# treangenlab/bronko

Hardware: AMD Instinct MI355X
Metric: reads/sec through call k-mer->pileup, SARS-CoV-2 k=21 (higher is better)
Workload: dtype u64

## Files before the change

bronko_amd/csrc/bk_engine.cpp:

```cpp
#include <hip/hip_runtime.h>

#include <algorithm>
#include <cstdarg>
#include <cstdio>
#include <cstdlib>
#include <cstring>
#include <memory>
#include <string>
#include <vector>

#include "bk_engine.h"

thread_local std::string g_err;

int fail(int code, const char* fmt, ...) {
    char buf[1024];
    va_list ap;
    va_start(ap, fmt);
    vsnprintf(buf, sizeof buf, fmt, ap);
    va_end(ap);
    g_err = buf;
    return code;
}

static int alloc_sample_state(bk_engine* e) {
    const bk_params* prm = &e->params;
    const IndexTables& ix = *e->ix;
    for (MatePlane& p : e->mate) BK_HIP(p.counters.alloc(ix.plane_len));
    e->sparse = ix.W > 0 && (ix.plane_len >= (16ull << 20) || test_env("BK_SPARSE_FINALIZE") != nullptr);
    if (e->sparse) {
        const uint64_t n_rows = bk::v_real_rows(ix.n_full, ix.v_span);
        for (MatePlane& p : e->mate) {
            BK_HIP(hipMemset(p.counters.p, 0, p.counters.n * sizeof(unsigned long long)));
            BK_HIP(p.touch_v.alloc(n_rows / 32 + 1)); BK_HIP(p.touch_p.alloc(ix.n_prows / 32 + 1)); BK_HIP(p.touch_e.alloc((size_t)ix.n_u / 32 + 1));
            BK_HIP(hipMemset(p.touch_v.p, 0, p.touch_v.n * 4)); BK_HIP(hipMemset(p.touch_p.p, 0, p.touch_p.n * 4));
            BK_HIP(hipMemset(p.touch_e.p, 0, p.touch_e.n * 4));
            BK_HIP(p.touch_b.alloc((size_t)ix.total_cells / 64 / 32 + 2)); BK_HIP(hipMemset(p.touch_b.p, 0, p.touch_b.n * 4));
            BK_HIP(p.v_list.alloc(n_rows)); BK_HIP(p.p_list.alloc(ix.n_prows)); BK_HIP(p.e_list.alloc(ix.n_u));
            BK_HIP(p.n_list.alloc(8));
        }
    }
    BK_HIP(e->shard_sums.alloc((size_t)2 * ix.n_files * 5 + 9));
    BK_HIP(e->xport_flag.alloc(4));
    BK_HIP(hipMemset(e->xport_flag.p, 0, 4 * sizeof(unsigned long long)));
    if (prm->full_kmer_stats) {
        if (prm->kmer_table_log2 < 10 || prm->kmer_table_log2 > 31) return fail(BK_ERR_INVALID, "kmer_table_log2 out of range");
        BK_HIP(e->ktab.keys.alloc((size_t)1 << prm->kmer_table_log2));
        BK_HIP(e->ktab.cnt.alloc((size_t)1 << prm->kmer_table_log2));
        e->ktab.log2 = prm->kmer_table_log2;
        BK_HIP(e->ktab.h_fill.grow(bk::ktab_fill_words())); BK_HIP(e->ktab.fill_ev.create());
    }
    BK_HIP(e->ktab_out.alloc(8 + bk::ktab_fill_words()));
    if (ix.n_files <= 2048) BK_HIP(e->fin_partials.alloc(bk::finalize_partial_rows() * ((size_t)ix.n_files * 3 + 2)));
    BK_HIP(e->deferred.alloc(bk::v_plane_len(ix.n_full, ix.v_span, ix.n_prows) * (prm->pileup_selected_only ? 2 : 1)));
    BK_HIP(e->n_deferred.alloc(2));
    if (prm->pileup_selected_only && ix.ent_files.p) BK_HIP(e->deferred_mask.alloc(e->deferred.n));
    if (!e->sparse) {
        BK_HIP(e->deferred_n.alloc(e->deferred.n));
        for (MatePlane& p : e->mate) BK_HIP(hipMemset(p.counters.p, 0, std::max<size_t>(p.counters.n, 1) * sizeof(unsigned long long)));
    }
    if (ix.n_files == 1 && !e->sparse && ix.n_full > 0) { BK_HIP(e->lean_e_list.alloc((size_t)ix.n_full)); BK_HIP(e->lean_n_list.alloc(8)); BK_HIP(hipMemset(e->lean_n_list.p, 0, 8 * sizeof(unsigned int))); }
    BK_HIP(e->pileup.alloc(ix.total_cells * 4 * 4));
    e->gather_mode = ix.gather_ok && e->sparse && ix.cell_file.p && ix.dirty_ans.p && ix.W > 1 && ix.file_cell_lo_d.p && !test_env("BK_NO_GATHER");
    if (e->gather_mode) {
        for (MatePlane& p : e->mate) BK_HIP(p.alias_hits.alloc((size_t)bk_engine::kAliasCap * 3));
        BK_HIP(e->n_alias_hits.alloc(2));
        BK_HIP(e->last_sel.upload(std::vector<int>(1, -1)));
        BK_HIP(hipMemset(e->pileup.p, 0, std::max<size_t>(e->pileup.n, 1) * sizeof(unsigned long long)));
        const bool two_pass = prm->pileup_selected_only != 0 && ix.n_files > 1;
        if (!two_pass && prm->cs < (1ull << 28) && ix.total_cells >= 2 * (uint64_t)ix.n_full && !test_env("BK_NO_VOTE_TABLE")) {
            BK_HIP(e->row_bits.alloc((size_t)((bk::v_real_rows(ix.n_full, ix.v_span) + 31) / 32) + 1));
            BK_HIP(e->vote_tab.alloc(bk::vote_table_words(ix.view())));
        }
    }
    BK_HIP(e->stats.alloc((size_t)2 * ix.n_files * 3));
    BK_HIP(e->present.alloc((size_t)2 * ix.n_files));
    if (prm->pileup_selected_only != 0 && ix.n_files > 1) BK_HIP(e->sel_out.alloc(1));
    BK_HIP(e->l2_plan.alloc(4));
    BK_HIP(e->kstats.alloc(8));
    e->use_items = !e->sparse && ix.ref_in_lds && ix.W > 0 && ix.n_lds_bins > 0 && !test_env("BK_NO_ITEMS") && ix.seed_tab2.p && ix.rc_words.p &&
                   bk::item_geometry(std::min<uint32_t>(ix.n_lds_bins, (uint32_t)ix.total_cells), ix.n_full, ix.v_span, &e->ig) &&
                   bk::items_lds_bytes(e->ig, std::min<uint32_t>(ix.n_lds_bins, (uint32_t)ix.total_cells)) <= 128u * 1024u;
    if (e->use_items) {
        if (const char* cp = test_env("BK_ITEM_CAPS")) {
            unsigned ce = 0, cv = 0;
            if (sscanf(cp, "%u,%u", &ce, &cv) == 2 && ce >= 8 && cv >= 8 && ce <= 64 && cv <= 64 && ce % 8 == 0 && cv % 8 == 0) {
                bk::ItemGeom g2 = e->ig;
                g2.cap_e = ce; g2.cap_v = cv; g2.wg_items = g2.n_ebins * ce + g2.n_vbins * cv; g2.wg_stride = g2.wg_items;
                if (bk::items_lds_bytes(g2, std::min<uint32_t>(ix.n_lds_bins, (uint32_t)ix.total_cells)) <= 118u * 1024u) e->ig = g2;
            }
        }
        const size_t g = bk::items_max_grid(ix.n_cus);
        e->ig.grid_max = (uint32_t)g;
        BK_HIP(e->items.alloc(g * e->ig.wg_stride + 64));
        BK_HIP(e->item_tab.alloc(g * ((size_t)e->ig.n_ebins + e->ig.n_vbins)));
        BK_HIP(e->item_gext.alloc(g * ((size_t)e->ig.n_ebins + e->ig.n_vbins) * bk::kItemGCap));
        BK_HIP(e->ov.alloc((size_t)1 << 20));
        BK_HIP(e->ov_n.alloc(4));
        BK_HIP(hipMemset(e->ov_n.p, 0, 4 * sizeof(unsigned long long)));
    } else {
        BK_HIP(e->slabs.alloc((size_t)ix.n_cus * std::max<uint32_t>(ix.n_lds_bins, 1)));
    }
    if (ix.n_files > 1) { BK_HIP(e->win_votes.alloc((size_t)ix.n_files)); BK_HIP(e->win_sel.upload(std::vector<uint32_t>(2, 0u))); }
    e->fuse_ok = e->use_items && ix.n_files == 1 && ix.max_seqs_per_file == 1 && (uint64_t)ix.n_lds_bins >= ix.total_cells && !e->ktab.keys.p && ix.n_prows == 0 &&
                 ix.n_u == ix.n_full && ix.n_full > 0 && ix.dirty_ans.p && ix.W > 1 && ix.v_span > 0 && ix.v_span <= 32 && e->fin_partials.p && e->lean_e_list.p &&
                 prm->cs < (1ull << 32) && e->ig.vq_log2 == 6 && !test_env("BK_NO_LEAN_FINALIZE") && !test_env("BK_NO_FUSE") && !test_env("BK_NO_N_DIRECT");
    if (e->fuse_ok)
        for (MatePlane& p : e->mate) { BK_HIP(p.fuse_touch.alloc(((size_t)ix.n_full + (size_t)ix.v_span + 63) / 64 * 12 + 16)); BK_HIP(hipMemset(p.fuse_touch.p, 0, p.fuse_touch.n * sizeof(unsigned int))); }
    BK_HIP(hipStreamCreateWithFlags(&e->own_stream, hipStreamNonBlocking));
    e->stream = e->own_stream;
    return BK_OK;
}

extern "C" {

int bk_abi_version(void) { return BK_ABI_VERSION; }
int bk_device_count(void) {
    int n = 0;
    return hipGetDeviceCount(&n) == hipSuccess && n > 0 ? n : 0;
}
int bk_device_memory(int device, uint64_t* free_bytes, uint64_t* total_bytes) {
    if (!free_bytes || !total_bytes) return fail(BK_ERR_INVALID, "null argument");
    BK_HIP(hipSetDevice(device));
    size_t f = 0, t = 0;
    BK_HIP(hipMemGetInfo(&f, &t));
    *free_bytes = f; *total_bytes = t;
    return BK_OK;
}
const char* bk_last_error(void) { return g_err.c_str(); }

void bk_params_default(bk_params* p) {
    if (!p) return;
    p->n_fixed = 2;
    p->use_full_kmer = 0;
    p->ci = 3;
    p->cs = 1000000;
    p->cx = 1000000000ull;
    p->device = 0;
    p->full_kmer_stats = 0;
    p->kmer_table_log2 = 26;
    p->pileup_selected_only = 0;
}


int bk_engine_create(const bk_index_desc* ix, const bk_params* prm, bk_engine** out) {
    if (!ix || !prm || !out) return fail(BK_ERR_INVALID, "null argument");
    *out = nullptr;
    const int k = ix->k;
    if (k < 3 || k > bk::kMaxK || (k & 1) == 0) return fail(BK_ERR_INVALID, "Invalid kmer size %d, must be odd and <= %d", k, bk::kMaxK);
    if (prm->n_fixed < 0) return fail(BK_ERR_INVALID, "n_fixed must be >= 0");
    if (ix->n_files <= 0 || ix->n_files > 65536) return fail(BK_ERR_INVALID, "n_files out of range");
    if (ix->n_buckets && (!ix->bucket_ids || !ix->bucket_off || !ix->entries)) return fail(BK_ERR_INVALID, "null index arrays");

    int ndev = 0;
    if (hipGetDeviceCount(&ndev) != hipSuccess || ndev <= 0) return fail(BK_ERR_NO_DEVICE, "no HIP device visible (this library has no CPU fallback)");
    if (prm->device < 0 || prm->device >= ndev) return fail(BK_ERR_NO_DEVICE, "device %d not present (%d visible)", prm->device, ndev);
    BK_HIP(hipSetDevice(prm->device));
    {
        hipDeviceProp_t prop;
        BK_HIP(hipGetDeviceProperties(&prop, prm->device));
        if (std::strncmp(prop.gcnArchName, "gfx950", 6) != 0)
            return fail(BK_ERR_NO_DEVICE, "device %d is %s, not gfx950 (MI355X); this library has no other code path", prm->device, prop.gcnArchName);
    }

    auto tab = std::make_shared<IndexTables>();
    PhaseClock pc;
    if (int rc = build_index_tables(ix, prm, *tab, pc)) return rc;
    std::unique_ptr<bk_engine> e(new bk_engine());
    e->params = *prm;
    e->device = prm->device;
    e->ix = tab;
    if (int rc = alloc_sample_state(e.get())) return rc;
    BK_HIP(tab->d_view.upload(std::vector<bk::IndexView>(1, tab->view())));
    pc.lap("uploads + buffers");
    *out = e.release();
    return BK_OK;
}

int bk_engine_fork(const bk_engine* parent, bk_engine** out) { return bk_engine_fork_params(parent, nullptr, out); }

int bk_engine_fork_params(const bk_engine* parent, const bk_params* prm, bk_engine** out) {
    if (!parent || !out) return fail(BK_ERR_INVALID, "null argument");
    if (prm && (prm->n_fixed != parent->params.n_fixed || (prm->use_full_kmer != 0) != (parent->params.use_full_kmer != 0) ||
                prm->device != parent->params.device || (prm->full_kmer_stats != 0) != (parent->params.full_kmer_stats != 0)))
        return fail(BK_ERR_INVALID, "bk_engine_fork_params: n_fixed, use_full_kmer, full_kmer_stats and device shape the shared tables and must equal the parent's");
    if (prm && prm->cs == 0) return fail(BK_ERR_INVALID, "cs must be >= 1");
    BK_HIP(hipSetDevice(parent->device));
    std::unique_ptr<bk_engine> e(new bk_engine());
    e->params = prm ? *prm : parent->params;
    e->device = parent->device;
    e->ix = parent->ix;
    e->ix->family.fetch_add(1);
    if (int rc = alloc_sample_state(e.get())) return rc;
    *out = e.release();
    return BK_OK;
}

void bk_engine_destroy(bk_engine* e) {
    if (!e) return;
    e->ix->family.fetch_sub(1);
    (void)hipSetDevice(e->device);
    (void)hipStreamSynchronize(e->stream);
    for (auto& s : e->spans) { (void)hipEventDestroy(s.a); (void)hipEventDestroy(s.b); }
    for (auto ev : e->free_events) (void)hipEventDestroy(ev);
    if (e->copy_stream) (void)hipStreamDestroy(e->copy_stream);
    if (e->own_stream) (void)hipStreamDestroy(e->own_stream);
    delete e;
}

int bk_engine_set_stream(bk_engine* e, void* hip_stream) {
    if (!e) return fail(BK_ERR_INVALID, "null engine");
    BK_HIP(hipStreamSynchronize(e->stream));
    e->stream = hip_stream ? reinterpret_cast<hipStream_t>(hip_stream) : e->own_stream;
    return BK_OK;
}

void* bk_engine_get_stream(const bk_engine* e) { return e ? reinterpret_cast<void*>(e->stream) : nullptr; }

uint64_t bk_total_cells(const bk_engine* e) { return e ? e->ix->total_cells : 0; }
int32_t bk_n_files(const bk_engine* e) { return e ? e->ix->n_files : 0; }
uint64_t bk_n_slots(const bk_engine* e) { return e ? e->ix->n_slots : 0; }
uint64_t bk_counter_len(const bk_engine* e) { return e ? e->ix->plane_len : 0; }
int bk_can_shard(const bk_engine* e) { return e && !e->sparse ? 1 : 0; }

int GrowTable::clear(bk_engine* e) {
    if (!old.empty()) {
        BK_HIP(hipStreamSynchronize(e->stream));
        for (auto& o : old) { (void)hipFree(o.first); (void)hipFree(o.second); }
        old.clear();
    }
    BK_HIP(hipMemsetAsync(keys.p, 0xff, keys.n * sizeof(unsigned long long), e->stream));
    BK_HIP(hipMemsetAsync(cnt.p, 0, cnt.n * sizeof(unsigned int), e->stream));
    fill_known = 0; fill_unknown_upper = 0; fill_pending = false;
    return BK_OK;
}

int bk_sample_begin(bk_engine* e) {
    if (!e) return fail(BK_ERR_INVALID, "null engine");
    BK_HIP(hipSetDevice(e->device));
    bk_engine::Span sp(e, 2);
    e->win_chosen = false;
    const bool sel_rows = e->gather_mode && e->params.pileup_selected_only != 0 && e->ix->n_files > 1;
    bk::launch_zero_small(e->stats.p, e->stats.n, e->kstats.p, e->kstats.n, e->ktab_out.p, e->ktab_out.n, e->present.p, e->present.n,
                          e->n_deferred.p, e->n_deferred.n, e->pileup.p, e->gather_mode ? 0 : e->pileup.n, e->stream);
    if (sel_rows) bk::launch_zero_genome_rows(e->pileup.p, (size_t)e->ix->total_cells * 4, e->ix->file_cell_lo_d.p, e->ix->n_files, (uint32_t)e->ix->total_cells, e->last_sel.p, e->stream);
    if (e->ktab.keys.p) { if (int rc = e->ktab.clear(e)) return rc; }
    if (e->dump) { if (int rc = e->dump->begin_sample(e)) return rc; }
    for (EventPass* p : e->event_passes()) if (p) { if (int rc = p->begin_sample(e)) return rc; }
    if (e->linkage) { if (int rc = e->linkage->begin_sample(e)) return rc; }
    if (e->primers) { if (int rc = e->primers->begin_sample(e)) return rc; }
    if (e->adapters) { if (int rc = e->adapters->begin_sample(e)) return rc; }
    e->ktab_exchanged = false; e->in_sample = true; e->finalized_mates = 0; e->called = false; e->cons_made = false; e->ci_made = false; e->regions_made = false;
    e->pending.on = false;
    for (MatePlane& p : e->mate) { if (int rc = p.begin_sample(e)) return rc; }
    return BK_OK;
}

int MatePlane::begin_sample(bk_engine* e) {
    stale = true; fuse_off = false; reduced_shards = 0; pushed_records = 0;
    if (touch_used) { BK_HIP(hipMemsetAsync(fuse_touch.p, 0, fuse_touch.n * sizeof(unsigned int), e->stream)); touch_used = false; }
    return BK_OK;
}

static int flush_pending_items(bk_engine* e) {
    if (!e->pending.on) return BK_OK;
    bk_engine::Span sp(e, 3);
    bk::BinArgs b = e->pending.b;
    b.part = 2; b.v_mode = e->ix->item_v_mode >= 0 && e->ix->item_v_mode != 2 ? e->ix->item_v_mode : 1;
    e->pending.on = false; e->mate[e->pending.mate].no_more_waiting();
    BK_HIP(bk::launch_bin_count(b, e->stream));
    return BK_OK;
}

int MatePlane::zero_if_stale(bk_engine* e) {
    if (!stale) return BK_OK;
    if (used) {
        bk_engine::Span sp(e, 2);
        BK_HIP(hipMemsetAsync(counters.p, 0, std::max<size_t>(counters.n, 1) * sizeof(unsigned long long), e->stream));
        if (e->sparse) for (DevBuf<unsigned int>* t : {&touch_v, &touch_p, &touch_b, &touch_e}) BK_HIP(hipMemsetAsync(t->p, 0, t->n * 4, e->stream));
        used = false;
    }
    stale = false;
    v_clean = true;
    return BK_OK;
}

int GrowTable::ensure_room(bk_engine* e, unsigned long long* out, uint64_t upper) {
    if (!keys.p) return BK_OK;
    const uint64_t cap = 1ull << log2;
    if (fill_known + fill_unknown_upper + upper > cap / 2) {
        if (fill_pending) { BK_HIP(hipEventSynchronize(fill_ev)); read_fill(); }
        uint32_t nl = log2;
        while (nl < 31 && fill_known + fill_unknown_upper + upper > (1ull << nl) / 2) nl += 2;
        if (nl > 31) nl = 31;
        if (nl != log2) {
            unsigned long long* nk = nullptr; unsigned int* nc = nullptr;
            BK_HIP(hipMalloc(reinterpret_cast<void**>(&nk), ((size_t)1 << nl) * sizeof(unsigned long long)));
            BK_HIP(hipMalloc(reinterpret_cast<void**>(&nc), ((size_t)1 << nl) * sizeof(unsigned int)));
            BK_HIP(hipMemsetAsync(nk, 0xff, ((size_t)1 << nl) * sizeof(unsigned long long), e->stream));
            BK_HIP(hipMemsetAsync(nc, 0, ((size_t)1 << nl) * sizeof(unsigned int), e->stream));
            bk::launch_ktab_rehash(keys.p, cnt.p, log2, nk, nc, nl, out + 4, e->stream);
            old.emplace_back(keys.p, cnt.p);
            keys.p = nk; keys.n = (size_t)1 << nl;
            cnt.p = nc; cnt.n = (size_t)1 << nl;
            log2 = nl;
        }
    }
    fill_unknown_upper += upper;
    return BK_OK;
}
int GrowTable::note_fill(bk_engine* e, const unsigned long long* out) {
    if (!keys.p) return BK_OK;
    BK_HIP(hipMemcpyAsync(h_fill.p, out + 8, bk::ktab_fill_words() * sizeof(unsigned long long), hipMemcpyDeviceToHost, e->stream));
    BK_HIP(hipEventRecord(fill_ev, e->stream));
    fill_pending = true;
    return BK_OK;
}

#ifdef BK_TESTING
static int l2_count_report(bk_engine* e, const bk::ScanArgs& a) {
    if (!test_env("BK_L2_COUNT")) return BK_OK;
    const uint64_t take = a.n_records;
    std::vector<unsigned int> hb((size_t)take * a.l2_words), ha((size_t)(take + 31) / 32);
    BK_HIP(hipMemcpyAsync(hb.data(), e->n_bits.p, hb.size() * sizeof(unsigned int), hipMemcpyDeviceToHost, e->stream));
    BK_HIP(hipMemcpyAsync(ha.data(), e->n_any.p, ha.size() * sizeof(unsigned int), hipMemcpyDeviceToHost, e->stream));
    BK_HIP(hipStreamSynchronize(e->stream));
    uint64_t nk = 0, nr = 0, runs = 0;
    for (size_t i = 0; i < hb.size(); i++) { nk += (uint64_t)__builtin_popcount(hb[i]); runs += (uint64_t)__builtin_popcount(hb[i] & ~(hb[i] << 1)); }
    for (unsigned int w : ha) nr += (uint64_t)__builtin_popcount(w);
    fprintf(stderr, "[bk] left to level 2 by the scan: %llu of %llu records marked, %llu k-mers in %llu N runs (per 32-bit word)\n", (unsigned long long)nr,
            (unsigned long long)take, (unsigned long long)nk, (unsigned long long)runs);
    return BK_OK;
}
static int l2_stats_arm(bk_engine* e) {
    if (test_env("BK_L2_STATS") && !e->dbg.p) { BK_HIP(e->dbg.alloc(32 + 4 * 1024)); BK_HIP(hipMemsetAsync(e->dbg.p, 0, (32 + 4 * 1024) * sizeof(unsigned long long), e->stream)); }
    return BK_OK;
}
static int l2_stats_report(bk_engine* e) {
    if (!e->dbg.p) return BK_OK;
    const IndexTables& ix = *e->ix;
    unsigned long long h[32]; unsigned int nd[2] = {0, 0};
    BK_HIP(hipMemcpyAsync(nd, e->n_deferred.p, sizeof nd, hipMemcpyDeviceToHost, e->stream));
    std::vector<unsigned long long> clk(4 * 1024);
    BK_HIP(hipMemcpyAsync(h, e->dbg.p, sizeof h, hipMemcpyDeviceToHost, e->stream));
    BK_HIP(hipMemcpyAsync(clk.data(), e->dbg.p + 32, clk.size() * sizeof(unsigned long long), hipMemcpyDeviceToHost, e->stream));
    BK_HIP(hipMemsetAsync(e->dbg.p, 0, (32 + 4 * 1024) * sizeof(unsigned long long), e->stream));
    BK_HIP(hipStreamSynchronize(e->stream));
    unsigned long long t0 = ~0ull;
    int n_wg = 0;
    for (int b = 0; b < 512; b++) if (clk[4 * b]) { t0 = std::min(t0, clk[4 * b]); n_wg = b + 1; }
    if (n_wg) {
        double mx[4] = {0, 0, 0, 0}, mean[4] = {0, 0, 0, 0}, mn[4] = {1e30, 1e30, 1e30, 1e30};
        for (int b = 0; b < n_wg; b++)
            for (int j = 0; j < 4; j++) {
                const double us = (double)(clk[4 * b + j] - t0) * 0.01;
                mx[j] = std::max(mx[j], us); mn[j] = std::min(mn[j], us); mean[j] += us / n_wg;
            }
        fprintf(stderr, "[bk] scan workgroups (%d), us after the first start, min / mean / max: start %.1f / %.1f / %.1f, reference staged %.1f / %.1f / %.1f, "
                "tiles done %.1f / %.1f / %.1f, end %.1f / %.1f / %.1f\n", n_wg, mn[0], mean[0], mx[0], mn[1], mean[1], mx[1], mn[2], mean[2], mx[2], mn[3], mean[3], mx[3]);
        double m2[4] = {0, 0, 0, 0};
        int n2 = 0;
        for (int b = 0; b < std::min(n_wg, 512); b++) if (clk[2048 + 4 * b]) { n2++; for (int j = 0; j < 4; j++) m2[j] += (double)(clk[2048 + 4 * b + j] - t0) * 0.01; }
        if (n2) fprintf(stderr, "[bk]   ... mean: first tile's copy sent %.1f, window's loads stored %.1f, wave 0 has its first tile %.1f, buckets written out %.1f\n",
                        m2[0] / n2, m2[1] / n2, m2[2] / n2, m2[3] / n2);
        if (test_env("BK_L2_STATS")[0] == '2')
            for (int b = 0; b < n_wg; b++) fprintf(stderr, "[bk]   wg %d: %.1f %.1f %.1f %.1f\n", b, (clk[4 * b] - t0) * 0.01, (clk[4 * b + 1] - t0) * 0.01, (clk[4 * b + 2] - t0) * 0.01, (clk[4 * b + 3] - t0) * 0.01);
    }
    fprintf(stderr, "[bk] finalize: %u + %u k-mers deferred to the general kernel\n", nd[0], nd[1]);
    if (e->gather_mode) {
        unsigned int ah[2] = {0u, 0u};
        BK_HIP(hipMemcpy(ah, e->n_alias_hits.p, sizeof ah, hipMemcpyDeviceToHost));
        fprintf(stderr, "[bk] votes gathered cell by cell (bk_gather.hip); alias hits among the deferred k-mers: %u + %u\n", ah[0], ah[1]);
    }
    if (e->sparse) {
        unsigned int nl[8];
        BK_HIP(hipMemcpy(nl, e->mate[0].n_list.p, sizeof nl, hipMemcpyDeviceToHost));
        fprintf(stderr, "[bk] sparse finalize (mate file 0): %u V rows of %llu, %u pseudo rows of %llu, %u reference k-mers of %u and %u pseudo k-mers of %u touched\n",
                nl[0], (unsigned long long)bk::v_real_rows(ix.n_full, ix.v_span), nl[4], (unsigned long long)ix.n_prows, nl[2], ix.n_full, nl[3], ix.n_u - ix.n_full);
    }
    fprintf(stderr, "[bk] scan: %llu mismatches counted, %llu items processed, %llu E gaps before a mismatch, %llu behind the last\n", h[23], h[24], h[25], h[26]);
    fprintf(stderr, "[bk] scan N batches: %llu with %llu pieces (%.1f per batch), %llu of them forced by a tile's end\n", h[20], h[21], h[20] ? (double)h[21] / (double)h[20] : 0.0, h[22]);
    fprintf(stderr, "[bk] level 2 discovery: %llu records newly marked by the scan, %llu records queued, g_work %llu\n", h[27], h[28], h[29]);
    fprintf(stderr, "[bk] scan marked: no-diagonal %llu, dirty-head %llu, clean-head %llu, pairs %llu | level 2: k-mers %llu in %llu chunks, simple %llu, dead %llu, "
            "dirty answers %llu (one difference but id unknown: %llu), neither half present %llu, slow %llu (diffs 0/1/2/3+ with a diagonal: %llu/%llu/%llu/%llu) -> member %llu, neighbour %llu, nothing %llu\n",
            h[0], h[1], h[2], h[3], h[4], h[11], h[5], h[6], h[16], h[17], h[18], h[7], h[12], h[13], h[14], h[15], h[8], h[9], h[10]);
    return BK_OK;
}
#else
static int l2_count_report(bk_engine*, const bk::ScanArgs&) { return BK_OK; }
static int l2_stats_arm(bk_engine*) { return BK_OK; }
static int l2_stats_report(bk_engine*) { return BK_OK; }
#endif

static bk::ScanArgs scan_args(const bk_engine* e, int mate, const Records& r) {
    const IndexTables& ix = *e->ix;
    const MatePlane& pl = e->mate[mate];
    bk::ScanArgs a{};
    a.n_records_dev = r.n_dev; a.ixp = ix.d_view.p;
    a.k = ix.k; a.wstart = ix.wstart; a.W = ix.W; a.v_omin = ix.v_omin; a.v_span = ix.v_span; a.v_off = ix.v_off; a.total_cells = (uint32_t)ix.total_cells; a.n_u = ix.n_u;
    a.ref_words = ix.ref_words.p; a.cell_codes = ix.cell_codes.p; a.cell_has = ix.cell_has.p; a.cell_clean = ix.cell_clean.p; a.cell_clean3 = ix.cell_clean3.p; a.cell_yf = ix.cell_yf.p; a.cell_yr = ix.cell_yr.p; a.id_at = ix.id_at.p; a.cell_fast = ix.cell_fast.p; a.cell_nat = ix.cell_nat.p; a.cell_natrow = ix.cell_natrow.p; a.cell_blk = ix.cell_blk.p; a.seed_tab = ix.seed_tab.p; a.seed_log2 = ix.seed_log2;
    a.seed_tab2 = ix.seed_tab2.p; a.seed2_log2 = ix.seed2_log2; a.rc_words = ix.rc_words.p;
    a.n_direct = e->use_items && ix.n_files == 1 && ix.max_seqs_per_file == 1 && (uint64_t)ix.n_lds_bins >= ix.total_cells && !test_env("BK_NO_N_DIRECT");
    a.words = r.words; a.lens = r.lens; a.n_records = r.n; a.stride_words = r.stride_words;
    a.counters = pl.counters.p; a.kmer_total = e->kstats.p + mate * 4 + 1;
    a.ablate = ix.ablate; a.slabs = e->slabs.p; a.n_lds_bins = ix.n_lds_bins; a.ref_in_lds = ix.ref_in_lds ? 1 : 0;
    a.ktab_keys = e->ktab.keys.p; a.ktab_cnt = e->ktab.cnt.p; a.ktab_log2 = e->ktab.log2;
    a.ktab_overflow = e->ktab_out.p + 4; a.mate = (uint32_t)mate;
    a.occ = ix.occ.p; a.n_files = ix.n_files;
    if (e->sparse) {
        a.touch_v = pl.touch_v.p; a.touch_b = pl.touch_b.p; a.touch_p = pl.touch_p.p; a.touch_e = pl.touch_e.p;
        a.rl_recip = ~0ull / (unsigned long long)(ix.v_span + 1) + 1ull;
    }
    a.dbg = e->dbg.p; a.l2_words = bk::scan_l2_words(r.stride_words, ix.k); a.l2_min_grid = (uint32_t)std::max(1, ix.n_cus / 2);
    if (const char* mg = test_env("BK_L2_MIN_GRID")) a.l2_min_grid = (uint32_t)std::max(1, atoi(mg));
    if (e->use_items) { a.ig = e->ig; a.items = e->items.p; a.tab = e->item_tab.p; a.gext = e->item_gext.p; a.ov = e->ov.p; a.ov_n = e->ov_n.p; a.ov_cap = (uint32_t)e->ov.n; }
    return a;
}
static int choose_window(bk_engine* e, bk::ScanArgs& a, uint64_t n) {
    const IndexTables& ix = *e->ix;
    if (ix.occ.p && !e->win_chosen && n > 0) {
        BK_HIP(hipMemsetAsync(e->win_votes.p, 0, e->win_votes.n * sizeof(unsigned int), e->stream));
        const char* wf = test_env("BK_WINDOW_FILE");
        const int forced = wf ? std::max(0, atoi(wf)) : -1;
        bk::launch_pick_window(a, 16384, e->win_votes.p, ix.file_cell_lo_d.p, forced, e->win_sel.p, e->stream);
        e->win_chosen = true;
    }
    a.win_dev = ix.occ.p ? e->win_sel.p : nullptr;
    return BK_OK;
}
static uint64_t next_launch(const bk_engine* e, uint64_t left, uint64_t l2_cap, uint32_t& grid) {
    const IndexTables& ix = *e->ix;
    grid = bk::scan_grid(left, ix.n_cus);
    uint64_t take = e->use_items ? std::min<uint64_t>(left, l2_cap) : std::min<uint64_t>(std::min<uint64_t>(left, bk::scan_max_records(grid)), l2_cap);
    if (ix.max_launch_records) take = std::min<uint64_t>(take, ix.max_launch_records);
    if (e->use_items) {
        int share = ix.n_cus - ix.n_cus / 4;
        if (const char* fr = test_env("BK_ITEM_SHARE")) share = std::max(1, std::min(ix.n_cus, ix.n_cus * atoi(fr) / 16));
        grid = bk::items_grid(take, ix.family.load() > 1 ? share : ix.n_cus);
        if (const char* gr = test_env("BK_ITEM_GRID")) grid = std::max<uint32_t>(1, std::min<uint32_t>(grid, (uint32_t)atoi(gr)));
    }
    return take;
}
static int make_l2_room(bk_engine* e, bk::ScanArgs& a, uint64_t l2_cap) {
    if (e->l2_bits.n < a.n_records * a.l2_words || e->l2_diag.n < a.n_records) {
        BK_HIP(hipStreamSynchronize(e->stream));
        const uint64_t recs = std::min<uint64_t>(std::max<uint64_t>(a.n_records + a.n_records / 4, 1 << 16), l2_cap);
        BK_HIP(e->l2_bits.alloc((size_t)recs * a.l2_words)); BK_HIP(e->n_bits.alloc((size_t)recs * a.l2_words)); BK_HIP(e->l2_diag.alloc((size_t)recs));
        BK_HIP(e->l2_any.alloc((size_t)(recs + 31) / 32)); BK_HIP(e->n_any.alloc((size_t)(recs + 31) / 32));
        for (DevBuf<unsigned int>* b : {&e->l2_bits, &e->l2_any, &e->n_bits, &e->n_any}) BK_HIP(hipMemsetAsync(b->p, 0, b->n * sizeof(unsigned int), e->stream));
    }
    a.l2_bits = e->l2_bits.p; a.l2_diag = e->l2_diag.p; a.l2_any = e->l2_any.p; a.n_bits = e->n_bits.p; a.n_any = e->n_any.p;
    return BK_OK;
}
static int bin_items(bk_engine* e, bk::ScanArgs& a, int mate, uint32_t grid, bool wait_v, bk::BinArgs* ride) {
    const IndexTables& ix = *e->ix;
    MatePlane& pl = e->mate[mate];
    bk_engine::Span sp(e, 3);
    bk::BinArgs b{};
    b.ig = e->ig; b.items = e->items.p; b.tab = e->item_tab.p; b.gext = e->item_gext.p; b.n_wg = grid; b.ov = e->ov.p; b.ov_n = e->ov_n.p; b.ov_cap = (uint32_t)e->ov.n;
    b.ov_par = e->ov_par; e->ov_par ^= 1u;
    b.id_at = ix.id_at.p; b.cell_codes = ix.cell_codes.p + bk::scan_ref_pad_words(); b.win_lo = a.win_lo; b.win_dev = a.win_dev; b.total_cells = (uint32_t)ix.total_cells;
    b.counters = pl.counters.p; b.v_off = ix.v_off; b.v_real_len = bk::v_real_len(ix.n_full, ix.v_span); b.rl = (uint32_t)ix.v_span + 1u;
    const bool v_clean = pl.take_v_clean();
    b.v_mode = ix.item_v_mode >= 0 ? ix.item_v_mode : (v_clean ? 2 : 1);
    if (const char* ba = test_env("BK_BIN_ABLATE")) b.ablate = atoi(ba);
    if (wait_v) {
        e->pending.on = true; e->pending.mate = mate; e->pending.b = b;
        b.part = 1;
        a.touch_v = pl.fuse_touch.p; a.rl_recip = ~0ull / (unsigned long long)(ix.v_span + 1) + 1ull;
        pl.items_wait();
    } else {
        pl.no_more_waiting();
        if (e->fuse_ok) a.touch_v = nullptr;
    }
    if (ride) {
        *ride = b; ride->part = 1;
        if (wait_v) return BK_OK;
        b.part = 2;
    }
    BK_HIP(bk::launch_bin_count(b, e->stream));
    return BK_OK;
}
static bool level2_runs(const bk_engine* e, const bk::ScanArgs& a) { return e->ix->ablate != 1 && e->ix->ablate != 4 && bk::level2_launches(a); }
static int level2_and_fold(bk_engine* e, const bk::ScanArgs& a, int mate, uint32_t grid, const bk::BinArgs* ride) {
    const IndexTables& ix = *e->ix;
    bk_engine::Span sp(e, 3);
    if (int rc = l2_count_report(e, a)) return rc;
    if (ix.ablate == 1 || ix.ablate == 4) {
        BK_HIP(hipMemsetAsync(e->n_bits.p, 0, (size_t)a.n_records * a.l2_words * sizeof(unsigned int), e->stream));
        BK_HIP(hipMemsetAsync(e->n_any.p, 0, e->n_any.n * sizeof(unsigned int), e->stream));
    }
    else BK_HIP(bk::launch_level2(a, ix.n_cus, e->stream, ride));
    if (!e->use_items) {
        bk::FoldArgs f{};
        f.slabs = e->slabs.p; f.n_slabs = grid; f.n_lds_bins = ix.n_lds_bins; f.id_at = ix.id_at.p; f.cell_codes = ix.cell_codes.p + bk::scan_ref_pad_words(); f.win_lo = a.win_lo; f.win_dev = a.win_dev; f.touch_e = a.touch_e;
        f.counters = e->mate[mate].counters.p;
        bk::launch_fold(f, e->stream);
    }
    return BK_OK;
}
}
int push_device(bk_engine* e, int mate, const Records& r) {
    MatePlane& pl = e->mate[mate];
    if (int rc = pl.zero_if_stale(e)) return rc;
    const uint64_t n = r.n, upper = r.kmers_upper ? r.kmers_upper : n * (uint64_t)r.stride_words * 16;
    if (int rc = e->ktab.ensure_room(e, e->ktab_out.p, upper)) return rc;
    if (e->dump) { if (int rc = e->dump->push(e, mate, r, upper)) return rc; }
    pl.written();
    if (int rc = l2_stats_arm(e)) return rc;
    bk::ScanArgs a = scan_args(e, mate, r);
    if (e->ix->W <= 0) {
        bk::launch_count_kmers(a, e->stream);
    } else {
        if (int rc = choose_window(e, a, n)) return rc;
        const uint64_t l2_cap = std::max<uint64_t>(64, ((1ull << 30) / sizeof(unsigned int)) / a.l2_words);
        for (uint64_t base = 0; base < n; base += a.n_records) {
            uint32_t grid = 0;
            a.rec_base = base; a.n_records = next_launch(e, n - base, l2_cap, grid);
            if (int rc = make_l2_room(e, a, l2_cap)) return rc;
            if (int rc = flush_pending_items(e)) return rc;
            const bool wait_v = e->fuse_ok && a.n_direct && !pl.fuse_off && e->ix->item_v_mode < 0;
            a.l2_plan = e->use_items && e->ix->n_files == 1 && e->ix->family.load() >= 4 && !test_env("BK_NO_L2_PLAN") ? e->l2_plan.p : nullptr;
            {
                bk_engine::Span sp(e, 0);
                if (e->use_items) { a.ov_par = e->ov_par; BK_HIP(bk::launch_scan_items(a, grid, e->stream)); }
                else BK_HIP(bk::launch_scan_count(a, grid, e->stream));
            }
            bk::BinArgs ride_b{};
            const bool ride = e->use_items && level2_runs(e, a) && !test_env("BK_NO_E_RIDE");
            if (e->use_items) { if (int rc = bin_items(e, a, mate, grid, wait_v, ride ? &ride_b : nullptr)) return rc; }
            if (int rc = level2_and_fold(e, a, mate, grid, ride ? &ride_b : nullptr)) return rc;
        }
    }
    for (EventPass* p : e->event_passes()) if (p) { if (int rc = p->push(e, r)) return rc; }
    if (e->linkage) { if (int rc = e->linkage->push(e, r)) return rc; }
    BK_HIP(hipGetLastError());
    if (!r.n_dev) pl.pushed_records += n;
    return e->ktab.note_fill(e, e->ktab_out.p);
}
extern "C" {

int bk_counters_device_ptr(bk_engine* e, int mate, void** d_ptr) {
    if (!e || !d_ptr || mate < 0 || mate > 1) return fail(BK_ERR_INVALID, "bad argument");
    if (e->sparse) return fail(BK_ERR_UNSUPPORTED, "an index this large keeps its counter planes sparse: shard whole samples over GPUs, not one sample's reads");
    if (e->pending.on) { BK_HIP(hipSetDevice(e->device)); if (int rc = flush_pending_items(e)) return rc; }
    if (e->in_sample) {
        BK_HIP(hipSetDevice(e->device));
        if (int rc = e->mate[mate].zero_if_stale(e)) return rc;
    }
    e->mate[mate].handed_out();
    *d_ptr = e->mate[mate].counters.p;
    return BK_OK;
}

int bk_pileup_device_ptr(bk_engine* e, void** d_ptr) {
    if (!e || !d_ptr) return fail(BK_ERR_INVALID, "bad argument");
    *d_ptr = e->pileup.p;
    return BK_OK;
}

struct FinalizeCall { int n_mates; uint64_t elem_lo, elem_hi; bool two_pass = false, gather = false, clean_dense = false; };
static int compact_sparse_lists(bk_engine* e, int n_mates) {
    const IndexTables& ix = *e->ix;
    for (int m = 0; m < n_mates; m++) {
        MatePlane& pl = e->mate[m];
        bk_engine::Span sp(e, 1);
        BK_HIP(hipMemsetAsync(pl.n_list.p, 0, 8 * sizeof(unsigned int), e->stream));
#ifdef BK_TESTING
        if (ix.ablate == 15) BK_HIP(hipMemsetAsync(pl.touch_b.p, 0xff, pl.touch_b.n * 4, e->stream));
#endif
        bk::launch_expand_touched_blocks(pl.touch_b.p, (uint32_t)((ix.total_cells + 63) / 64), ix.cell_blk.p, pl.touch_v.p, (uint32_t)ix.k,
                                         (uint64_t)ix.n_full + (uint64_t)ix.v_span, e->stream);
        bk::launch_compact_touched(pl.touch_v.p, bk::v_real_rows(ix.n_full, ix.v_span), pl.touch_p.p, ix.n_prows, pl.touch_e.p, ix.n_u,
                                   ix.n_full, pl.v_list.p, pl.p_list.p, pl.e_list.p, pl.n_list.p, e->stream);
    }
    return BK_OK;
}
static bk::FinalizeArgs finalize_args(const bk_engine* e, const FinalizeCall& c, int m, int pass) {
    const IndexTables& ix = *e->ix;
    const MatePlane& pl = e->mate[m];
    bk::FinalizeArgs a{};
    a.ix = ix.view();
    a.counters = pl.reduced_shards > 0 ? pl.reduced.p - c.elem_lo : pl.counters.p;
    a.elem_lo = c.elem_lo; a.elem_hi = c.elem_hi; a.ci = e->params.ci; a.cs = e->params.cs; a.cx = e->params.cx; a.pileup = e->pileup.p; a.plane = (size_t)ix.total_cells * 4;
    a.stats = e->stats.p + (size_t)m * ix.n_files * 3; a.present = e->present.p + (size_t)m * ix.n_files; a.kept_total = e->kstats.p + m * 4 + 3; a.distinct_total = e->kstats.p + m * 4 + 2;
    a.partials = e->fin_partials.p; a.n_deferred = e->n_deferred.p + m;
    a.deferred = e->deferred.p + (c.two_pass ? (size_t)m * (e->deferred.n / 2) : 0);
    a.file_cell_lo = ix.file_cell_lo_d.p; a.max_file_cells = (uint32_t)ix.max_file_cells_idx;
    a.deferred_mask = c.two_pass && e->deferred_mask.p ? e->deferred_mask.p + (size_t)m * (e->deferred_mask.n / 2) : nullptr;
    a.ktab_keys = e->ktab.keys.p; a.ktab_cnt = e->ktab.cnt.p; a.ktab_log2 = e->ktab.log2; a.ktab_overflow = e->ktab_out.p + 4; a.mate = (uint32_t)m;
    if (e->sparse) { a.v_list = pl.v_list.p; a.p_list = pl.p_list.p; a.e_list = pl.e_list.p; a.n_list = pl.n_list.p; }
    a.deferred_n = e->deferred_n.p ? e->deferred_n.p + (c.two_pass ? (size_t)m * (e->deferred_n.n / 2) : 0) : nullptr;
    a.clear_v = c.clean_dense && pass == (c.two_pass ? 1 : 0);
    a.mode = c.two_pass ? pass + 1 : c.gather ? (pass == 0 ? 1 : 3) : 0;
    if (c.gather) {
        if (const char* ga = test_env("BK_GATHER_ABLATE")) a.gather_ablate = atoi(ga);
        a.merged_slots = ix.merged_slots.p; a.n_merged_slots = ix.n_merged_slots;
        a.gather = pass == 1 ? 1 : 0; a.alias_hits = pl.alias_hits.p; a.n_alias_hits = e->n_alias_hits.p + m; a.alias_cap = bk_engine::kAliasCap;
    }
    a.sel = c.two_pass ? &e->sel_out.p->file_id : nullptr; a.sel_file = -1;
    const bool ride = c.clean_dense && !c.two_pass && e->fin_partials.p && pl.used;
    a.no_lean = test_env("BK_NO_LEAN_FINALIZE") != nullptr; a.lean_e_list = e->lean_e_list.p; a.lean_n_list = e->lean_n_list.p;
    a.zero_e = ride ? pl.counters.p : nullptr; a.zero_e_n = ride ? (size_t)std::min<uint64_t>(ix.v_off, ix.plane_len) : 0;
    return a;
}
static int clean_planes(bk_engine* e, const FinalizeCall& c) {
    const IndexTables& ix = *e->ix;
    for (int m = 0; m < c.n_mates && c.clean_dense; m++) {
        MatePlane& pl = e->mate[m];
        if (pl.used) {
            bk_engine::Span sp(e, 2);
            BK_HIP(hipMemsetAsync(pl.counters.p, 0, (size_t)std::min<uint64_t>(ix.v_off, ix.plane_len) * sizeof(unsigned long long), e->stream));
        }
        pl.finalized_clean();
    }
    for (int m = 0; m < c.n_mates && e->sparse; m++) {
        MatePlane& pl = e->mate[m];
        bk_engine::Span sp(e, 1);
        bk::launch_clear_touched(pl.counters.p, ix.v_off, bk::v_real_len(ix.n_full, ix.v_span), (uint32_t)ix.v_span + 1u, pl.v_list.p, pl.p_list.p,
                                 pl.e_list.p, pl.n_list.p, ix.n_u, e->stream);
        pl.finalized_clean();
    }
    if (e->ktab.keys.p) { bk_engine::Span sp(e, 1); bk::launch_ktab_stats(e->ktab.keys.p, e->ktab.cnt.p, e->ktab.log2, e->params.ci, e->params.cx, e->ktab_out.p, e->stream); }
    return BK_OK;
}
static int finalize_part(bk_engine* e, int n_mates, uint64_t elem_lo, uint64_t elem_hi) {
    const IndexTables& ix = *e->ix;
    if (!e->in_sample) return fail(BK_ERR_STATE, "bk_sample_finalize called before bk_sample_begin");
    if (n_mates < 1 || n_mates > 2) return fail(BK_ERR_INVALID, "n_mates must be 1 or 2");
    BK_HIP(hipSetDevice(e->device));
    const bool whole = elem_lo == 0 && elem_hi == ix.plane_len;
    const bool via_reduced = e->mate[0].reduced_shards > 0 || e->mate[1].reduced_shards > 0;
    FinalizeCall c{n_mates, elem_lo, elem_hi};
    c.two_pass = e->params.pileup_selected_only != 0 && ix.n_files > 1;
    c.gather = e->gather_mode && whole && !via_reduced;
    c.clean_dense = !e->sparse && whole && !via_reduced;
    if (c.two_pass && !whole) return fail(BK_ERR_UNSUPPORTED, "pileup_selected_only cannot be combined with a sharded finalize");
    if (e->sparse && !whole) return fail(BK_ERR_UNSUPPORTED, "an index this large cannot be finalized in shards");
    if (e->sparse) { if (int rc = compact_sparse_lists(e, n_mates)) return rc; }
    if (c.gather) BK_HIP(hipMemsetAsync(e->n_alias_hits.p, 0, 2 * sizeof(unsigned int), e->stream));
    auto sync_debug = [e](const char* what) -> int {
        if (test_env("BK_SYNC_DEBUG")) { fprintf(stderr, "[bk] %s ...", what); BK_HIP(hipStreamSynchronize(e->stream)); fprintf(stderr, " ok\n"); }
        return BK_OK;
    };
    for (int pass = 0; pass < ((c.two_pass || c.gather) ? 2 : 1); pass++) {
        const bool votes = c.gather && pass == 1;
        if (votes) {
            bk_engine::Span sp(e, 1);
            if (int rc = sync_debug("statistics pass")) return rc;
            if (e->row_bits.p) BK_HIP(hipMemsetAsync(e->row_bits.p, 0, e->row_bits.n * sizeof(unsigned int), e->stream));
            for (int m = 0; m < n_mates; m++) bk::launch_prefix_rows(e->mate[m].counters.p, ix.view(), e->mate[m].v_list.p, e->mate[m].n_list.p, e->row_bits.p, e->stream);
            if (int rc = sync_debug("prefix_rows")) return rc;
        }
        for (int m = 0; m < n_mates; m++) {
            bk::FinalizeArgs a = finalize_args(e, c, m, pass);
            if (a.zero_e) e->mate[m].finalized_clean();
            if (pass == 0) { if (int rc = e->mate[m].zero_if_stale(e)) return rc; }
            if (e->pending.on && e->pending.mate == m) {
                const bk::BinArgs& pb = e->pending.b;
                a.f_items = pb.items; a.f_tab = pb.tab; a.f_gext = pb.gext; a.f_ov = pb.ov; a.f_ov_n = pb.ov_n; a.f_ov_cap = pb.ov_cap; a.f_ov_par = pb.ov_par;
                a.f_n_wg = pb.n_wg; a.f_ig = pb.ig; a.f_touch = e->mate[m].fuse_touch.p;
                if (c.clean_dense && !c.two_pass && bk::finalize_runs_by_region(a)) { e->pending.on = false; e->mate[m].items_taken(); }
                else { a.f_items = nullptr; if (int rc = flush_pending_items(e)) return rc; }
            }
            bk_engine::Span sp(e, 1);
            if (votes && m == 0) {
                const unsigned long long* c1 = n_mates == 2 ? e->mate[1].counters.p : nullptr;
                if (bk::vote_table_fits(a) && e->row_bits.p && e->vote_tab.n >= bk::vote_table_words(a.ix)) bk::launch_gather_votes_table(a, c1, e->vote_tab.p, e->row_bits.p, e->stream);
                else bk::launch_gather_votes(a, c1, e->stream);
                if (int rc = sync_debug("gather_votes")) return rc;
            }
            if (votes && ix.n_merged_slots) { bk::launch_merged_votes(a, e->stream); if (int rc = sync_debug("merged_votes")) return rc; }
            bk::launch_finalize(a, e->stream);
            if (votes) if (int rc = sync_debug("alias-only general kernels")) return rc;
        }
        if (c.two_pass && pass == 0) {
            bk::CallArgs s{};
            s.n_files = ix.n_files; s.n_mates = n_mates; s.stats = e->stats.p; s.present = e->present.p; s.genome_len = ix.genome_len.p; s.out = e->sel_out.p;
            bk_engine::Span sp(e, 1);
            bk::launch_select_genome(s, e->stream);
            if (c.gather) bk::launch_copy_int(e->last_sel.p, &e->sel_out.p->file_id, e->stream);
        }
    }
    if (int rc = clean_planes(e, c)) return rc;
    BK_HIP(hipGetLastError());
    e->in_sample = false; e->finalized_mates = n_mates;
    return l2_stats_report(e);
}

int bk_sample_finalize(bk_engine* e, int n_mates) {
    if (!e) return fail(BK_ERR_INVALID, "null engine");
    if (e->mate[0].reduced_shards > 1 || e->mate[1].reduced_shards > 1) return fail(BK_ERR_STATE, "this sample's planes went through bk_shard_transport: finalize it with bk_sample_finalize_shard");
    int rc = finalize_part(e, n_mates, 0, e->ix->plane_len);
    if (rc == BK_OK && e->dump) rc = e->dump->finalize(e, n_mates);
    return rc;
}

int bk_sample_finalize_shard(bk_engine* e, int n_mates, int shard, int n_shards) {
    if (!e) return fail(BK_ERR_INVALID, "null engine");
    if (n_shards < 1 || (int)bk::kMaxShards % n_shards != 0 || shard < 0 || shard >= n_shards)
        return fail(BK_ERR_INVALID, "n_shards must divide %u and 0 <= shard < n_shards", bk::kMaxShards);
    if (e->ktab.keys.p && n_shards > 1 && !e->ktab_exchanged)
        return fail(BK_ERR_STATE, "full_kmer_stats with a sharded finalize: exchange the ranks' k-mer statistics tables first "
                                  "(bk_kmer_table_partition, all-to-all, bk_kmer_table_replace)");
    const uint64_t part = e->ix->plane_len / (uint64_t)n_shards;
    for (int m = 0; m < n_mates; m++)
        if (e->mate[m].reduced_shards > 0 && (e->mate[m].reduced_shards != n_shards || e->mate[m].reduced_shard != shard))
            return fail(BK_ERR_STATE, "bk_sample_finalize_shard(%d of %d): mate file %d received part %d of %d (bk_shard_received)", shard, n_shards, m,
                        e->mate[m].reduced_shard, e->mate[m].reduced_shards);
    int rc = finalize_part(e, n_mates, part * shard, part * (shard + 1));
    if (rc != BK_OK) return rc;
    if (e->ktab.keys.p) bk::launch_ktab_totals_to_kstats(e->ktab_out.p, e->kstats.p, n_mates, e->stream);
    for (int m = 0; m < n_mates; m++) {
        if (e->mate[m].pushed_records) bk::launch_add_const_u64(e->kstats.p + m * 4 + 0, e->mate[m].pushed_records, e->stream);
        e->mate[m].pushed_records = 0;
    }
    bk::launch_pack_sums(e->shard_sums.p, e->stats.p, e->present.p, e->kstats.p, e->ix->n_files, e->xport_flag.p, e->stream);
    BK_HIP(hipGetLastError());
    return BK_OK;
}

int bk_kmer_table_partition(bk_engine* e, int n_parts, void** d_keys, void** d_counts, uint64_t* part_off) {
    if (!e || !d_keys || !d_counts || !part_off) return fail(BK_ERR_INVALID, "null argument");
    if (n_parts < 1 || n_parts > (int)bk::kMaxShards) return fail(BK_ERR_INVALID, "1 <= n_parts <= %u", bk::kMaxShards);
    if (!e->ktab.keys.p) return fail(BK_ERR_STATE, "the engine was created without full_kmer_stats");
    if (!e->in_sample) return fail(BK_ERR_STATE, "bk_kmer_table_partition comes between the pushes and the finalize of a sample");
    BK_HIP(hipSetDevice(e->device));
    if (!e->xchg_cursors.p) BK_HIP(e->xchg_cursors.alloc(bk::kMaxShards));
    BK_HIP(hipMemsetAsync(e->xchg_cursors.p, 0, bk::kMaxShards * sizeof(unsigned long long), e->stream));
    bk::launch_ktab_count_parts(e->ktab.keys.p, e->ktab.log2, (uint32_t)n_parts, e->xchg_cursors.p, e->stream);
    unsigned long long counts[bk::kMaxShards];
    if (int rc = download(e, counts, e->xchg_cursors.p, (size_t)n_parts)) return rc;
    unsigned long long first[bk::kMaxShards];
    part_off[0] = 0;
    for (int r = 0; r < n_parts; r++) { first[r] = part_off[r]; part_off[r + 1] = part_off[r] + counts[r]; }
    const uint64_t total = part_off[n_parts];
    if (e->xchg_keys.n < total || !e->xchg_keys.p) {
        BK_HIP(e->xchg_keys.alloc(std::max<uint64_t>(total + total / 4, 1024)));
        BK_HIP(e->xchg_cnt.alloc(e->xchg_keys.n));
    }
    BK_HIP(hipMemcpyAsync(e->xchg_cursors.p, first, (size_t)n_parts * sizeof(unsigned long long), hipMemcpyHostToDevice, e->stream));
    bk::launch_ktab_scatter_parts(e->ktab.keys.p, e->ktab.cnt.p, e->ktab.log2, (uint32_t)n_parts, e->xchg_cursors.p, e->xchg_keys.p, e->xchg_cnt.p, e->stream);
    BK_HIP(hipGetLastError());
    BK_HIP(hipStreamSynchronize(e->stream));
    *d_keys = e->xchg_keys.p; *d_counts = e->xchg_cnt.p;
    return BK_OK;
}

int bk_kmer_table_replace(bk_engine* e, const void* d_keys, const void* d_counts, uint64_t n) {
    if (!e || (n && (!d_keys || !d_counts))) return fail(BK_ERR_INVALID, "null argument");
    if (!e->ktab.keys.p) return fail(BK_ERR_STATE, "the engine was created without full_kmer_stats");
    if (!e->in_sample) return fail(BK_ERR_STATE, "bk_kmer_table_replace comes between the pushes and the finalize of a sample");
    BK_HIP(hipSetDevice(e->device));
    BK_HIP(hipMemsetAsync(e->ktab.keys.p, 0xff, e->ktab.keys.n * sizeof(unsigned long long), e->stream));
    BK_HIP(hipMemsetAsync(e->ktab.cnt.p, 0, e->ktab.cnt.n * sizeof(unsigned int), e->stream));
// ... 198 lines not shown
```

bronko_amd/csrc/bk_engine.h:

```cpp
#pragma once
#include <hip/hip_runtime.h>

#include <algorithm>
#include <array>
#include <atomic>
#include <chrono>
#include <cstdio>
#include <cstdlib>
#include <memory>
#include <string>
#include <thread>
#include <vector>

#include "../../include/bronko_hip.h"
#include "bk_device.h"
#include "bk_kernels.h"

#pragma GCC visibility push(hidden)

extern thread_local std::string g_err;

int fail(int code, const char* fmt, ...);
struct bk_engine;

// ... 263 lines not shown
    bool in_sample = false;
    bool summed = false;
    bool made = false;
    virtual ~EventPass() = default;
    int begin_sample(bk_engine* e);
    virtual int push(bk_engine* e, const Records& r) = 0;
    virtual int clear_table(bk_engine* e);
};
template <class Cfg, class Row>
struct EventPassOf : EventPass {
    Cfg cfg{};
    DevBuf<Row> rows;
};
struct Indels : EventPassOf<bk_indel_config, bk_indel_record> {
    DevBuf<unsigned long long> key0, key1;
    int push(bk_engine* e, const Records& r) override;
    int clear_table(bk_engine* e) override;
};
struct Junctions : EventPassOf<bk_junction_config, bk_junction_record> { int push(bk_engine* e, const Records& r) override; };
struct Copybacks : EventPassOf<bk_copyback_config, bk_copyback_record> { int push(bk_engine* e, const Records& r) override; };
struct Chimeras : EventPassOf<bk_chimera_config, bk_chimera_record> { int push(bk_engine* e, const Records& r) override; };
struct Breakends : EventPassOf<bk_breakend_config, bk_breakend_record> {
    DevBuf<unsigned int> site;
    int push(bk_engine* e, const Records& r) override;
    int clear_table(bk_engine* e) override;
};
struct Duplications : EventPassOf<bk_duplication_config, bk_duplication_record> { int push(bk_engine* e, const Records& r) override; };

struct IndexTables {
    mutable std::atomic<int> family{1};
    int k = 0, wstart = 0, W = 0, n_files = 0;
    uint64_t total_cells = 0, n_slots = 0;
    uint32_t log2s = 4, log2nb = 0, log2p = 0, m = 1, n_u = 0, n_full = 0, n_lds_bins = 0;
    uint64_t n_prows = 0;
    int v_omin = 0, v_span = 0;
    uint64_t v_off = 0, plane_len = 0;
    DevBuf<uint32_t> prow_id;
    DevBuf<uint8_t> prow_t;
    bool ref_in_lds = false;
    int lo_bases = 0, n_cus = 256;

    DevBuf<bk::KmerPos> kmer_pos;
    DevBuf<bk::IndexView> d_view;
    DevBuf<uint64_t> kmer_of;
    DevBuf<bk::IdRec> id_rec;
    DevBuf<bk::DirtyAns> dirty_ans;
    DevBuf<uint8_t> cell_flags;
    DevBuf<uint32_t> ref_words, cell_codes, cell_has, cell_clean, cell_clean3, cell_yf, cell_yr, id_at, cell_fast, cell_nat, cell_natrow;
    DevBuf<uint2> cell_blk, seed_tab, seed_tab2;
    uint32_t seed_log2 = 0, seed2_log2 = 0;
    DevBuf<uint32_t> rc_words;
    struct HalfBufs { DevBuf<uint16_t> pilots; DevBuf<bk::HalfDir> dir; DevBuf<bk::NbEntry> cand; uint32_t m = 1, log2nb = 0, log2p = 0; DevBuf<uint32_t> bits; uint32_t bits_log2 = 0, bits_exact = 0; } half_lo, half_hi;
    DevBuf<uint32_t> slot_of, estat_off, estat;
    DevBuf<bk::SlotRec> slot_rec;
    DevBuf<uint4> ent_files, slot_files, id_own_files, estat_files;
    DevBuf<uint16_t> cell_file;
    DevBuf<uint32_t> slot_alias;
    DevBuf<uint64_t> merged_slots;
    uint32_t n_merged_slots = 0;
    bool gather_ok = false;
    DevBuf<uint32_t> id_rest_off, id_rest;
    DevBuf<uint8_t> amb;
    DevBuf<uint16_t> pilots;
    DevBuf<bk::TableSlot> table;
    DevBuf<uint32_t> ent_off, ent_len;
    DevBuf<bk::DevEntry> entries;
    DevBuf<uint32_t> occ;
    DevBuf<uint32_t> file_cell_lo_d;
    std::vector<uint32_t> file_cell_lo;
    DevBuf<uint64_t> genome_len, seq_cell, seq_len_d;
    DevBuf<int32_t> seq_first, n_seqs_d;
    std::vector<uint64_t> h_seq_cell, h_seq_len;
    std::vector<int32_t> h_seq_first, h_n_seqs;
    std::vector<uint2> h_nonacgt;
    int max_seqs_per_file = 0;
    uint64_t max_file_cells = 0;
    uint64_t max_file_cells_idx = 0;
    int ablate = 0;
    int item_v_mode = -1;
    uint64_t max_launch_records = 0;

    bk::IndexView view() const {
        bk::IndexView v{};
        v.kmer_pos = kmer_pos.p; v.pilots = pilots.p; v.m = m; v.log2nb = log2nb; v.log2p = log2p;
        v.kmer_of = kmer_of.p; v.id_rec = id_rec.p; v.dirty_ans = dirty_ans.p; v.cell_flags = cell_flags.p; v.ref_words = ref_words.p; v.cell_codes = cell_codes.p; v.cell_has = cell_has.p; v.cell_clean = cell_clean.p; v.cell_clean3 = cell_clean3.p; v.cell_yf = cell_yf.p; v.cell_yr = cell_yr.p; v.id_at = id_at.p; v.cell_fast = cell_fast.p; v.cell_nat = cell_nat.p; v.cell_natrow = cell_natrow.p; v.cell_blk = cell_blk.p; v.seed_tab = seed_tab.p; v.seed_log2 = seed_log2; v.total_cells = (uint32_t)total_cells; v.n_u = n_u;
        v.n_full = n_full; v.n_prows = n_prows; v.prow_id = prow_id.p; v.prow_t = prow_t.p; v.v_omin = v_omin; v.v_span = v_span; v.v_off = v_off;
        v.lo = bk::HalfView{half_lo.pilots.p, half_lo.dir.p, half_lo.cand.p, half_lo.m, half_lo.log2nb, half_lo.log2p, half_lo.bits.p, half_lo.bits_log2, half_lo.bits_exact};
        v.hi = bk::HalfView{half_hi.pilots.p, half_hi.dir.p, half_hi.cand.p, half_hi.m, half_hi.log2nb, half_hi.log2p, half_hi.bits.p, half_hi.bits_log2, half_hi.bits_exact};
        v.lo_bases = lo_bases; v.slot_of = slot_of.p; v.slot_rec = slot_rec.p; v.ent_files = ent_files.p; v.slot_files = slot_files.p; v.slot_alias = slot_alias.p; v.gather_ok = gather_ok ? 1u : 0u; v.id_own_files = id_own_files.p; v.cell_file = cell_file.p; v.id_rest_off = id_rest_off.p; v.id_rest = id_rest.p; v.estat_files = estat_files.p; v.amb = amb.p; v.estat_off = estat_off.p; v.estat = estat.p;
        v.table = table.p; v.ent_off = ent_off.p; v.ent_len = ent_len.p;
        v.entries = entries.p; v.n_slots = n_slots; v.log2s = log2s; v.k = k; v.wstart = wstart; v.W = W; v.n_files = n_files;
        return v;
    }
};

int build_index_tables(const bk_index_desc* ix, const bk_params* prm, IndexTables& tab, PhaseClock& pc);

struct MatePlane {
    DevBuf<unsigned long long> counters;
    DevBuf<unsigned int> touch_v, touch_b, touch_p, touch_e, v_list, p_list, e_list, n_list;
    DevBuf<unsigned int> fuse_touch;
    DevBuf<unsigned long long> alias_hits;
    DevBuf<unsigned long long> reduced;
    int reduced_shards = 0, reduced_shard = 0;
    uint64_t pushed_records = 0;
    bool stale = true, used = false, v_clean = false, fuse_off = false, touch_used = false;
    int begin_sample(bk_engine* e);
    int zero_if_stale(bk_engine* e);
    void written() { used = true; }
    void handed_out() { used = true; v_clean = false; }
    void finalized_clean() { used = false; }
    bool take_v_clean() { const bool c = v_clean; v_clean = false; return c; }
    void items_wait() { touch_used = true; }
    void no_more_waiting() { fuse_off = true; }
    void items_taken() { touch_used = false; }
};

struct bk_engine {
    bk_params params{};
    std::shared_ptr<const IndexTables> ix;
    DevBuf<unsigned long long> shard_sums;
    MatePlane mate[2];
    DevBuf<unsigned char> xport_send, xport_recv;
    DevBuf<unsigned long long> xport_flag;
    bool xport_ever = false;
    int device = 0;

    DevBuf<unsigned int> deferred, n_deferred, deferred_mask;
    DevBuf<unsigned long long> deferred_n;
    DevBuf<unsigned int> fin_partials;
    GrowTable ktab;
    DevBuf<unsigned long long> ktab_out;
    DevBuf<unsigned long long> xchg_keys, xchg_cursors;
    DevBuf<unsigned int> xchg_cnt;
    bool ktab_exchanged = false;
    std::unique_ptr<Primers> primers;
    std::unique_ptr<Adapters> adapters;
    bool trims() const { return primers || adapters; }
    std::unique_ptr<KmerDump> dump;
    bool gather_mode = false;
    DevBuf<unsigned int> row_bits;
    DevBuf<uint32_t> vote_tab;
    DevBuf<unsigned int> n_alias_hits;
    static constexpr unsigned int kAliasCap = 1u << 20;
    DevBuf<int> last_sel;
    DevBuf<unsigned int> slabs;
    bool use_items = false;
    bk::ItemGeom ig{};
    DevBuf<unsigned short> items, item_tab;
    DevBuf<unsigned short> item_gext;
    DevBuf<unsigned int> ov;
    DevBuf<unsigned long long> ov_n;
    uint32_t ov_par = 0;
    DevBuf<unsigned int> lean_e_list, lean_n_list;
    bool fuse_ok = false;
    struct PendingItems { bool on = false; int mate = 0; bk::BinArgs b{}; } pending;
    DevBuf<unsigned int> n_bits, n_any;
    DevBuf<unsigned int> l2_bits;
    DevBuf<unsigned int> l2_any;
    DevBuf<unsigned int> l2_plan;
    DevBuf<uint2> l2_diag;
    bool sparse = false;
    DevBuf<unsigned long long> pileup;
    DevBuf<unsigned long long> stats;
    DevBuf<unsigned char> present;
    DevBuf<unsigned long long> kstats;
    struct StageSlot {
        RecordBufs rec;
        PinnedBuf<uint8_t> h;
        Event done; bool busy = false;
    } stage[2];
    int next_stage = 0;

    struct IngestSlot {
        PinnedBuf<uint8_t> h_bases, h_quals;
        PinnedBuf<unsigned long long> h_off;
        DevBuf<uint8_t> d_bases, d_quals;
        DevBuf<unsigned long long> d_off, d_nrec;
        DevBuf<uint32_t> d_work;
        RecordBufs rec;
        Event uploaded, done;
        bool busy = false;
    };
    IngestSlot slots[3];
    IngestSlot dev_ascii;
    int next_slot = 0;
    hipStream_t copy_stream = nullptr;

    hipStream_t own_stream = nullptr, stream = nullptr;
    bool in_sample = false;
    int finalized_mates = 0;
    DevBuf<unsigned int> win_votes;
    DevBuf<uint32_t> win_sel;
    bool win_chosen = false;

    DevBuf<double> call_noise, noise_maf, noise_tbl, noise_sums;
    DevBuf<unsigned int> noise_cnt, noise_state;
    DevBuf<bk_call_record> call_records;
    DevBuf<bk_call_summary> call_out;
    DevBuf<bk_call_summary> sel_out;
    bool called = false;
    DevBuf<uint8_t> cons_letters;
    DevBuf<bk_consensus_summary> cons_out;
    bool cons_made = false;
    bk_consensus_params cons_prm{};
    DevBuf<unsigned int> ci_bounds;
    DevBuf<bk_consensus_indel_record> ci_rows;
    DevBuf<bk_consensus_indel_summary> ci_out;
    bool ci_made = false;
    std::unique_ptr<Regions> regions;
    bool regions_made = false;
    std::unique_ptr<Indels> indels;
    std::unique_ptr<Junctions> junctions;
    std::unique_ptr<Copybacks> copybacks;
    std::unique_ptr<Chimeras> chimeras;
    std::unique_ptr<Breakends> breakends;
    std::unique_ptr<Duplications> duplications;
    std::array<EventPass*, 6> event_passes() const { return {indels.get(), junctions.get(), copybacks.get(), chimeras.get(), breakends.get(), duplications.get()}; }
    std::unique_ptr<Linkage> linkage;
    std::weak_ptr<AnchorTables> anchors;
    DevBuf<unsigned long long> dbg;
    bool timing = false;
    unsigned timing_kinds = 0xfu, timing_every = 1, timing_seen[4] = {0, 0, 0, 0};
    std::vector<TimedSpan> spans;
    std::vector<hipEvent_t> free_events;

    hipEvent_t get_event() {
        if (!free_events.empty()) { hipEvent_t e = free_events.back(); free_events.pop_back(); return e; }
        hipEvent_t e = nullptr;
        (void)hipEventCreate(&e);
        return e;
    }
    struct Span {
        bk_engine* e; int kind; hipEvent_t a = nullptr;
        Span(bk_engine* eng, int k) : e(eng), kind(k) {
            if (e->timing && (e->timing_kinds >> k) & 1 && e->timing_seen[k]++ % e->timing_every == 0) { a = e->get_event(); (void)hipEventRecord(a, e->stream); }
        }
        ~Span() {
            if (a) { hipEvent_t b = e->get_event(); (void)hipEventRecord(b, e->stream); e->spans.push_back({a, b, kind}); }
        }
    };
};

int push_device(bk_engine* e, int mate, const Records& r);

template <class T>
int download(bk_engine* e, T* host_dst, const void* dev_src, size_t count) {
    BK_HIP(hipMemcpyAsync(host_dst, dev_src, count * sizeof(T), hipMemcpyDeviceToHost, e->stream));
    BK_HIP(hipStreamSynchronize(e->stream));
    return BK_OK;
}

#pragma GCC visibility pop
```

bronko_amd/csrc/bk_finalize_common.h:

```cpp
#pragma once
#include <hip/hip_runtime.h>

#include "bk_device.h"
#include "bk_kernels.h"
#include "bk_scan_common.h"

namespace bk {

__device__ __forceinline__ void vote(const FinalizeArgs& a, const DevEntry& e, uint64_t c, uint32_t isrc, int k, unsigned long long v) {
    if (a.mode == 1 || (a.mode == 2 && (int)e.file != a.sel_file)) return;
    uint32_t bit_idx;
    bool forward;
    if (e.canonical) {
        bit_idx = ((uint32_t)(c >> (2 * e.idx)) & 3u) ^ 3u;
        forward = isrc != 0;
    } else {
        bit_idx = (uint32_t)(c >> (2 * (k - 1 - e.idx))) & 3u;
        forward = isrc == 0;
    }
    const size_t cell = (size_t)e.cell * 4 + bit_idx;
    atomicAdd(a.pileup + (forward ? 2 : 3) * a.plane + cell, 1ull);
    atomicMax(a.pileup + (forward ? 0 : 1) * a.plane + cell, v);
}


__device__ __forceinline__ void tally(uint32_t* lstats, uint32_t idx) {
    const unsigned long long active = __ballot(true);
    const int leader = __builtin_ctzll(active);
    const uint32_t lidx = (uint32_t)__shfl((int)idx, leader);
    const bool same = idx == lidx;
    const unsigned long long sm = __ballot(same);
    if (!same) atomicAdd(&lstats[idx], 1u);
    else if ((int)(threadIdx.x & 63u) == leader) atomicAdd(&lstats[idx], (uint32_t)__popcll(sm));
}

__device__ __forceinline__ void finalize_epilogue(const FinalizeArgs& a, const uint32_t* lstats, unsigned int kept, unsigned int distinct,
                                                  uint32_t* scratch2 , int row) {
    const int n3 = a.ix.n_files * 3;
#pragma unroll
    for (int off = 32; off; off >>= 1) { kept += (unsigned int)__shfl_xor((int)kept, off); distinct += (unsigned int)__shfl_xor((int)distinct, off); }
    if ((threadIdx.x & 63) == 0) { if (kept) atomicAdd(&scratch2[0], kept); if (distinct) atomicAdd(&scratch2[1], distinct); }
    __syncthreads();
    if (a.partials) {
        uint32_t* out = a.partials + (size_t)row * (n3 + 2);
        for (int g = threadIdx.x; g < n3; g += blockDim.x) out[g] = lstats[g];
        if (threadIdx.x == 0) { out[n3] = scratch2[0]; out[n3 + 1] = scratch2[1]; }
    } else {
        for (int g = threadIdx.x; g < a.ix.n_files; g += blockDim.x) {
            const uint32_t pf = lstats[g * 3], vr = lstats[g * 3 + 1], un = lstats[g * 3 + 2];
            if (pf) atomicAdd(a.stats + (size_t)g * 3 + 0, (unsigned long long)pf);
            if (vr) atomicAdd(a.stats + (size_t)g * 3 + 1, (unsigned long long)vr);
            if (un) atomicAdd(a.stats + (size_t)g * 3 + 2, (unsigned long long)un);
            if (pf | vr) a.present[g] = 1;
        }
        if (threadIdx.x == 0) {
            if (scratch2[0] && a.kept_total) atomicAdd(a.kept_total, (unsigned long long)scratch2[0]);
            if (scratch2[1] && a.distinct_total) atomicAdd(a.distinct_total, (unsigned long long)scratch2[1]);
        }
    }
}


__device__ __forceinline__ uint64_t revcomp_kmer(uint64_t c, int k) {
    const uint64_t t = ~c;
    const uint64_t r = ((uint64_t)rev2_32((uint32_t)t) << 32) | rev2_32((uint32_t)(t >> 32));
    return r >> (64 - 2 * k);
}


}
```

bronko_amd/csrc/bk_finalize_lean.hip:

```cpp
#include <hip/hip_runtime.h>

#include "bk_device.h"
#include "bk_kernels.h"
#include "bk_scan_common.h"
#include "bk_finalize_common.h"

namespace bk {

constexpr int kLeanVBlock = 1024;
constexpr uint32_t kLeanVq = 64;
constexpr uint32_t kLeanWin = 256;
constexpr uint32_t kLeanMaxSpan = 32;
constexpr uint32_t kLeanTouchWords = kLeanVq * kVRowsPerPos / 32;
constexpr size_t kLeanStaticLds = (2u * 8u * kLeanWin + 5u + kLeanTouchWords + 1u) * sizeof(unsigned int);
constexpr size_t lean_dynamic_lds(uint32_t v_span) { return (size_t)kLeanVq * kVRowsPerPos * ((size_t)v_span + 1u) * sizeof(unsigned int); }
static_assert(kLeanStaticLds + 64u + lean_dynamic_lds(kLeanMaxSpan) <= 80u * 1024u, "two finalize_vbin workgroups no longer fit one CU's LDS");

__device__ __forceinline__ void lean_vote(unsigned int* cnt, unsigned int* mxv, uint32_t span, uint32_t p0, const FinalizeArgs& a, uint32_t cell,
                                          uint32_t idx, bool canonical, uint64_t c, uint32_t isrc, int k, uint32_t v) {
    uint32_t bit_idx;
    bool forward;
    if (canonical) { bit_idx = ((uint32_t)(c >> (2 * idx)) & 3u) ^ 3u; forward = isrc != 0; }
    else { bit_idx = (uint32_t)(c >> (2 * (k - 1 - (int)idx))) & 3u; forward = isrc == 0; }
    const uint32_t pos = cell - p0;
    if (cell >= p0 && pos < span) {
        const uint32_t at = ((forward ? 0u : 4u) + bit_idx) * span + pos;
        __hip_atomic_fetch_add(cnt + at, 1u, __ATOMIC_RELAXED, __HIP_MEMORY_SCOPE_WORKGROUP);
        __hip_atomic_fetch_max(mxv + at, v, __ATOMIC_RELAXED, __HIP_MEMORY_SCOPE_WORKGROUP);
    } else {
        const size_t pc = (size_t)cell * 4 + bit_idx;
        atomicAdd(a.pileup + (forward ? 2 : 3) * a.plane + pc, 1ull);
        atomicMax(a.pileup + (forward ? 0 : 1) * a.plane + pc, (unsigned long long)v);
    }
}
__device__ __forceinline__ void lean_flush(const unsigned int* cnt, const unsigned int* mxv, uint32_t span, uint32_t p0, const FinalizeArgs& a) {
    for (uint32_t i = threadIdx.x; i < 8u * span; i += blockDim.x) {
        const unsigned int nv = cnt[i];
        if (!nv) continue;
        const uint32_t row = i / span, pos = i - row * span;
        const size_t pc = ((size_t)p0 + pos) * 4 + (row & 3u);
        atomicAdd(a.pileup + (row < 4u ? 2 : 3) * a.plane + pc, (unsigned long long)nv);
        atomicMax(a.pileup + (row < 4u ? 0 : 1) * a.plane + pc, (unsigned long long)mxv[i]);
    }
}

template <bool FUSED>
__global__ __launch_bounds__(kLeanVBlock) __attribute__((amdgpu_waves_per_eu(8, 8))) void finalize_vbin_kernel(FinalizeArgs a) {
    __shared__ unsigned int cnt[8 * kLeanWin], mxv[8 * kLeanWin];
    __shared__ uint32_t lstats[3 + 2];
    __shared__ unsigned int tmask[kLeanTouchWords + 1];
    extern __shared__ __attribute__((aligned(16))) unsigned int acc[];
    const IndexView& ix = a.ix;
    const int k = ix.k;
    const uint32_t span = (uint32_t)ix.v_span, rl = span + 1u;
    const uint32_t q0 = blockIdx.x * kLeanVq;
    const uint32_t nq = ix.n_full + span;
    const uint32_t id_lo = min(q0 >= span - 1u ? q0 - (span - 1u) : 0u, ix.n_full - 1u);
    const uint32_t p0 = ix.id_rec[id_lo].cell;
    for (uint32_t i = threadIdx.x; i < 8u * kLeanWin; i += kLeanVBlock) { cnt[i] = 0u; mxv[i] = 0u; }
    if (threadIdx.x < 5) lstats[threadIdx.x] = 0u;
    if constexpr (FUSED) {
        const uint32_t n_eb = a.f_ig.n_ebins, n_bins = n_eb + a.f_ig.n_vbins, bin = n_eb + blockIdx.x, cap = a.f_ig.cap_v, G = a.f_ig.grid_max;
        const uint32_t upb = cap / 8u;
        const uint32_t vsize = kLeanVq * kVRowsPerPos * rl;
        const uint32_t n_units = a.f_n_wg * upb;
        const unsigned short* const bin_items = a.f_items + (size_t)n_eb * G * a.f_ig.cap_e + (size_t)blockIdx.x * G * cap;
        const bool mine = threadIdx.x < n_units;
        const uint32_t wg0 = mine ? threadIdx.x / upb : 0u, un0 = threadIdx.x - wg0 * upb;
        uint32_t hdr0 = 0u;
        uint4 v0 = make_uint4(0u, 0u, 0u, 0u);
        if (mine) { hdr0 = a.f_tab[(size_t)bin * G + wg0]; v0 = reinterpret_cast<const uint4*>(bin_items + (size_t)wg0 * cap)[un0]; }
        const unsigned long long ov_all = a.f_ov_n[a.f_ov_par];
        if (threadIdx.x <= kLeanTouchWords) {
            unsigned int* tw = a.f_touch + (size_t)blockIdx.x * kLeanTouchWords + threadIdx.x;
            unsigned int m = 0u;
            if (threadIdx.x < kLeanTouchWords) { m = *tw; if (m) *tw = 0u; }
            else m = ov_all > (unsigned long long)a.f_ov_cap ? 1u : 0u;
            tmask[threadIdx.x] = m;
        }
        for (uint32_t i = threadIdx.x; i < vsize; i += kLeanVBlock) acc[i] = 0u;
        __syncthreads();
        auto take = [&](uint32_t it) __attribute__((always_inline)) {
            __hip_atomic_fetch_add(acc + (it & 0x7fffu), (it & 0x8000u) ? 0u - 1u : 1u, __ATOMIC_RELAXED, __HIP_MEMORY_SCOPE_WORKGROUP);
        };
        auto take8 = [&](const uint4& v, uint32_t left) __attribute__((always_inline)) {
            if (left > 0u) take(v.x & 0xffffu);
            if (left > 1u) take(v.x >> 16);
            if (left > 2u) take(v.y & 0xffffu);
            if (left > 3u) take(v.y >> 16);
            if (left > 4u) take(v.z & 0xffffu);
            if (left > 5u) take(v.z >> 16);
            if (left > 6u) take(v.w & 0xffffu);
            if (left > 7u) take(v.w >> 16);
        };
        for (uint32_t u = threadIdx.x; u < n_units; u += kLeanVBlock) {
            const uint32_t wg = u / upb, un = u - wg * upb;
            uint32_t n_all; uint4 v;
            if (u == threadIdx.x) { n_all = hdr0; v = v0; }
            else { n_all = a.f_tab[(size_t)bin * G + wg]; v = reinterpret_cast<const uint4*>(bin_items + (size_t)wg * cap)[un]; }
            const uint32_t n = min(n_all, cap);
            take8(v, n > 8u * un ? n - 8u * un : 0u);
            const uint32_t g = min(n_all - n, kItemGCap);
            if (g) {
                const uint4* q = reinterpret_cast<const uint4*>(a.f_gext + ((size_t)wg * n_bins + bin) * kItemGCap);
                for (uint32_t i0 = 8u * un; i0 < g; i0 += 8u * upb * 4u) {
                    uint4 e[4];
#pragma unroll
                    for (uint32_t j = 0; j < 4u; ++j) e[j] = i0 + 8u * upb * j < g ? q[(i0 >> 3) + upb * j] : make_uint4(0u, 0u, 0u, 0u);
#pragma unroll
                    for (uint32_t j = 0; j < 4u; ++j) take8(e[j], g > i0 + 8u * upb * j ? g - i0 - 8u * upb * j : 0u);
                }
            }
        }
        {
            const uint32_t n_ov = (uint32_t)(ov_all < (unsigned long long)a.f_ov_cap ? ov_all : (unsigned long long)a.f_ov_cap);
            for (uint32_t i = threadIdx.x; i < n_ov; i += kLeanVBlock) {
                const uint32_t e = a.f_ov[i];
                if ((e >> 16) == bin) take(e & 0xffffu);
            }
        }
    }
    __syncthreads();
    unsigned long long* __restrict__ vc = const_cast<unsigned long long*>(a.counters) + ix.v_off;
    const uint32_t lpr = span, gpw = 64u / lpr;
    const uint32_t lane64 = threadIdx.x & 63u, wave = threadIdx.x >> 6;
    const uint32_t grp = lane64 / lpr, oo = lane64 - grp * lpr;
    const bool lane_on = grp < gpw;
    unsigned int kept = 0, distinct = 0, variant = 0;
    for (uint32_t g0 = 0; g0 < kLeanVq * kVRowsPerPos; g0 += (kLeanVBlock / 64) * gpw) {
        const uint32_t g = g0 + wave * gpw + grp;
        const uint32_t q = q0 + g / kVRowsPerPos, r6 = g % kVRowsPerPos;
        const bool in_row = lane_on && g < kLeanVq * kVRowsPerPos && q < nq;
        const size_t at = ((size_t)q * kVRowsPerPos + r6) * rl + oo;
        unsigned long long n;
        if constexpr (FUSED) {
            const uint32_t gg = in_row ? g : 0u;
            n = in_row ? (unsigned long long)(long long)(int32_t)acc[gg * rl + oo] : 0ull;
            if (in_row && (tmask[kLeanTouchWords] || ((tmask[gg >> 5] >> (gg & 31u)) & 1u))) {
                const unsigned long long pv = vc[at];
                if (pv) { n += pv; vc[at] = 0ull; }
            }
        } else {
            n = in_row ? vc[at] : 0ull;
            if (a.clear_v && n) vc[at] = 0ull;
        }
        const uint32_t d = r6 & 1u, alt = r6 >> 1;
        const bool inq = in_row && q >= oo && q - oo < ix.n_full;
        const uint32_t p = inq ? q - oo : 0u;
        const uint4 idr = *reinterpret_cast<const uint4*>(ix.id_rec + p);
        const uint64_t kmer_p = (uint64_t)idr.x | ((uint64_t)idr.y << 32);
        const uint32_t ambp = idr.w;
        const int o = (int)oo + ix.v_omin;
        if (!__ballot(n + (1ull << 26) >= (1ull << 27))) {
            int m = (int)(unsigned int)n;
#pragma unroll
            for (int off = 1; off < 32; off <<= 1) {
                const int t = __shfl_up(m, off, 64);
                if (oo >= (uint32_t)off) m += t;
            }
            n = (unsigned long long)(long long)m;
        } else {
#pragma unroll
            for (int off = 1; off < 32; off <<= 1) {
                const unsigned long long t = __shfl_up(n, off, 64);
                if (oo >= (uint32_t)off) n += t;
            }
        }
        bool act = inq && n != 0;
        const uint32_t rcid = (ambp >> 1) & 1u;
        const int j = rcid ? k - 1 - o : o;
        const int sh = 2 * (k - 1 - (act ? j : 0));
        const uint32_t bb = ((uint32_t)(kmer_p >> sh) & 3u) ^ (alt + 1u);
        const uint32_t isrc = d ^ rcid;
        const uint64_t c = (kmer_p & ~(3ull << sh)) | ((uint64_t)bb << sh);
        const uint64_t rc = revcomp_kmer(c, k);
        if (act && !(j >= ix.wstart && j < ix.wstart + ix.W && c < rc)) act = false;
        if (act) { distinct += 1; if (n < a.ci || n > a.cx) act = false; else kept += 1; }
        const uint32_t v = (uint32_t)(n > a.cs ? a.cs : n);
        bool defer = false;
        if (act) {
            bool plain = (ambp & kIdSimple) != 0u;
            if (plain && (ambp & 1u)) {
                const uint2 ans = *reinterpret_cast<const uint2*>(ix.dirty_ans + ans_index(p, (uint32_t)o, rcid ? 3u - bb : bb, k));
                plain = !(ans.y & (kAnsNone | kAnsMulti));
            }
            if (!plain) { defer = true; act = false; }
        }
        {
            const unsigned long long dm = __ballot(defer);
            if (dm) {
                unsigned int base = 0;
                if (lane64 == (uint32_t)__builtin_ctzll(dm)) base = atomicAdd(a.n_deferred, (unsigned int)__popcll(dm));
                base = (unsigned int)__shfl((int)base, __builtin_ctzll(dm));
                if (defer) {
                    const unsigned int slot = base + (unsigned int)__popcll(dm & ((1ull << lane64) - 1ull));
                    a.deferred[slot] = (uint32_t)at;
                    if (a.deferred_n) a.deferred_n[slot] = n;
                }
            }
        }
        if (act) lean_vote(cnt, mxv, kLeanWin, p0, a, idr.z + (uint32_t)j, (uint32_t)j, rcid != 0u, c, isrc, k, v);
        variant += act ? 1u : 0u;
    }
#pragma unroll
    for (int off = 32; off; off >>= 1) variant += (unsigned int)__shfl_xor((int)variant, off);
    if (lane64 == 0 && variant) atomicAdd(&lstats[1], variant);
    {
        const uint32_t W = (uint32_t)ix.W;
        const uint32_t sub = threadIdx.x & 15u, id = q0 + (threadIdx.x >> 4);
        unsigned int perfect = 0;
        if (id < ix.n_full) {
            const uint4 idr = *reinterpret_cast<const uint4*>(ix.id_rec + id);
            const unsigned long long n0 = a.counters[2 * (size_t)id], n1 = a.counters[2 * (size_t)id + 1];
            if (!(idr.w & kIdSimple)) {
                if (sub == 0u && (n0 | n1)) a.lean_e_list[atomicAdd(a.lean_n_list + 2, 1u)] = id;
            } else {
                const uint64_t km = (uint64_t)idr.x | ((uint64_t)idr.y << 32);
                const uint32_t rcid = (idr.w >> 1) & 1u;
#pragma unroll
                for (uint32_t isrc = 0; isrc < 2u; ++isrc) {
                    const unsigned long long n = isrc ? n1 : n0;
                    if (sub == 0u) distinct += n != 0;
                    if (n == 0 || n < a.ci || n > a.cx) continue;
                    if (sub == 0u) { kept += 1; perfect += 1; }
                    const uint32_t v = (uint32_t)(n > a.cs ? a.cs : n);
                    for (uint32_t t = sub; t < W; t += 16u) {
                        const uint32_t j = (uint32_t)ix.wstart + t;
                        lean_vote(cnt, mxv, kLeanWin, p0, a, idr.z + j, j, rcid != 0u, km, isrc, k, v);
                    }
                }
            }
        }
#pragma unroll
        for (int off = 32; off; off >>= 1) perfect += (unsigned int)__shfl_xor((int)perfect, off);
        if (lane64 == 0 && perfect) { atomicAdd(&lstats[0], perfect); atomicAdd(&lstats[2], perfect); }
    }
    __syncthreads();
    lean_flush(cnt, mxv, kLeanWin, p0, a);
    finalize_epilogue(a, lstats, kept, distinct, lstats + 3, (int)blockIdx.x);
}

bool finalize_lean_ok(const FinalizeArgs& a) {
    return !a.no_lean && a.lean_e_list && a.lean_n_list && !a.ix.slot_files && a.mode == 0 && !a.v_list && !a.p_list && !a.e_list && !a.ktab_keys && a.ix.n_prows == 0 && a.ix.n_u == a.ix.n_full &&
           a.ix.n_full > 0 && a.ix.n_files == 1 && a.ix.dirty_ans && a.ix.W > 1 && a.ix.v_span > 0 && a.ix.v_span <= (int)kLeanMaxSpan && a.partials && a.cs < (1ull << 32) &&
           a.elem_lo == 0 && a.elem_hi >= a.ix.v_off + v_plane_len(a.ix.n_full, a.ix.v_span, 0);
}
unsigned launch_finalize_lean_variant(const FinalizeArgs& a, hipStream_t stream) {
    const unsigned grid = (unsigned)((a.ix.n_full + (uint32_t)a.ix.v_span + kLeanVq - 1) / kLeanVq);
    if (a.f_items) {
        const size_t lds = lean_dynamic_lds((uint32_t)a.ix.v_span);
        (void)raise_lds_limit(reinterpret_cast<const void*>(finalize_vbin_kernel<true>), lds + 20u * 1024u);
        hipLaunchKernelGGL(finalize_vbin_kernel<true>, dim3(grid), dim3(kLeanVBlock), lds, stream, a);
    } else {
        hipLaunchKernelGGL(finalize_vbin_kernel<false>, dim3(grid), dim3(kLeanVBlock), 0, stream, a);
    }
    return grid;
}
}
```

bronko_amd/csrc/bk_kernels.h:

```cpp
#pragma once
#include <hip/hip_runtime.h>

#include <cstddef>

#include "../../include/bronko_hip.h"
#include "bk_device.h"
#include "bk_link_row.h"

namespace bk {

struct ItemGeom {
    uint32_t n_ebins, n_vbins;
    uint32_t cap_e, cap_v;
    uint32_t vq_log2;
    uint32_t wg_items;
    uint32_t wg_stride;
    uint32_t grid_max;
};
constexpr uint32_t kEBinLog2 = 7;
constexpr uint32_t kERunMax = 255;
constexpr uint32_t kEBinSpan = (1u << kEBinLog2) + kERunMax;
constexpr uint32_t kItemGCap = 256;

struct ScanArgs {
    const IndexView* ixp;
    int32_t k, wstart, W, v_omin, v_span;
    uint64_t v_off;
    uint32_t total_cells, n_u;
    const uint32_t* ref_words;
    const uint32_t* cell_codes;
    const uint32_t* cell_has;
    const uint32_t* cell_clean;
    const uint32_t* cell_clean3;
    const uint32_t* cell_yf;
    const uint32_t* cell_yr;
    const uint32_t* id_at;
    const uint32_t* cell_fast;
    const uint2* cell_blk;
    const uint32_t* cell_nat;
    const uint32_t* cell_natrow;
    const uint2* seed_tab;
    uint32_t seed_log2;
    const uint2* seed_tab2;
    uint32_t seed2_log2;
    const uint32_t* rc_words;
    const uint32_t* words;
    const uint16_t* lens;
    uint64_t rec_base;
    uint64_t n_records;
    const unsigned long long* n_records_dev;
    uint32_t stride_words;
    unsigned long long* counters;
    unsigned int* slabs;
    unsigned int* n_bits;
    unsigned int* n_any;
    unsigned int* l2_bits;
    unsigned int* l2_any;
    unsigned int* l2_plan;
    uint32_t l2_min_grid;
    uint2* l2_diag;
    uint32_t l2_words;
    uint32_t n_lds_bins;
    uint32_t win_lo;
    const uint32_t* win_dev;
    const uint32_t* occ;
    int32_t win_file, n_files;
    int ref_in_lds;
    unsigned long long* kmer_total;
    unsigned long long* ktab_keys;
    unsigned int* ktab_cnt;
    uint32_t ktab_log2;
    unsigned long long* ktab_overflow;
    uint32_t mate;
    unsigned int* touch_v;
    unsigned int* touch_b;
    unsigned int* touch_p;
    unsigned int* touch_e;
    unsigned long long rl_recip;
    ItemGeom ig;
    unsigned short* items;
    unsigned short* tab;
    unsigned short* gext;
    unsigned int* ov;
    unsigned long long* ov_n;
    uint32_t ov_cap;
    uint32_t ov_par;
    int n_direct;
    uint32_t stage_off;
    int ablate;
    unsigned long long* dbg;
};

struct FinalizeArgs {
    IndexView ix;
    const unsigned long long* counters;
    uint64_t elem_lo, elem_hi;
    unsigned long long ci, cs, cx;
    unsigned long long* pileup;
    size_t plane;
    unsigned long long* stats;
    unsigned char* present;
    unsigned long long* kept_total;
    unsigned long long* distinct_total;
    unsigned int* partials;
    int row_exact, row_general;
    const uint32_t* file_cell_lo;
    uint32_t max_file_cells;
    unsigned int* deferred;
    unsigned long long* deferred_n;
    int clear_v;
    unsigned int* deferred_mask;
    unsigned int* n_deferred;
    unsigned long long* ktab_keys;
    unsigned int* ktab_cnt;
    uint32_t ktab_log2;
    unsigned long long* ktab_overflow;
    uint32_t mate;
    const unsigned int* v_list;
    const unsigned int* p_list;
    const unsigned int* e_list;
    const unsigned int* n_list;
    int mode;
    const int* sel;
    int sel_file;
    unsigned int* lean_e_list;
    unsigned int* lean_n_list;
    int no_lean;
    const unsigned int* tail_e_list;
    const unsigned int* tail_n_list;
    unsigned long long* zero_e;
    size_t zero_e_n;
    int gather;
    int gather_ablate;
    unsigned long long* alias_hits;
    unsigned int* n_alias_hits;
    unsigned int alias_cap;
    const uint64_t* merged_slots;
    uint32_t n_merged_slots;
    const unsigned short* f_items;
    const unsigned short* f_tab;
    const unsigned short* f_gext;
    const unsigned int* f_ov;
    const unsigned long long* f_ov_n;
    uint32_t f_ov_cap, f_ov_par, f_n_wg;
    ItemGeom f_ig;
    unsigned int* f_touch;
};

struct FoldArgs {
    const unsigned int* slabs;
    uint32_t n_slabs;
    uint32_t n_lds_bins;
    const uint32_t* id_at;
    uint32_t win_lo;
    const uint32_t* win_dev;
    unsigned int* touch_e;
    const uint32_t* cell_codes;
    unsigned long long* counters;
};

struct PackArgs {
    const uint8_t* bases;
    uint32_t shift;
    const unsigned long long* offsets;
    uint64_t n_reads;
    int32_t k;
    uint32_t stride_words;
    uint32_t* words;
    uint16_t* lens;
    uint64_t cap;
    unsigned long long* n_records;
    unsigned long long* n_real;
    uint32_t* work;
};
struct QualArgs {
    const uint8_t* quals;
    uint32_t shift;
    uint32_t thr;
};
void launch_pack_reads(const PackArgs& a, unsigned long long* tally, hipStream_t stream, const QualArgs* q = nullptr, uint8_t* ends = nullptr);

constexpr uint32_t kEndFirst = 1u, kEndLast = 2u;
constexpr uint32_t kPrimerMinLen = BK_PRIMER_MIN_LEN, kPrimerMaxLen = BK_PRIMER_MAX_LEN, kMaxPrimers = BK_MAX_PRIMERS, kMaxPrimerMismatches = BK_PRIMER_MAX_MISMATCHES;
constexpr uint32_t kPrimerEntryWords = 9;
struct TrimArgs {
    uint32_t* words;
    uint16_t* lens;
    const uint8_t* ends;
    uint64_t n_records;
    const unsigned long long* n_records_dev;
    uint32_t stride_words;
    int32_t k;
    const uint32_t* table;
    uint32_t n_primers;
    uint32_t max_mismatches;
    unsigned long long* stats;
    unsigned long long* n_real;
};
void launch_primer_trim(const TrimArgs& a, int n_cus, hipStream_t stream);

constexpr uint32_t kAdapterMinLen = BK_ADAPTER_MIN_LEN, kAdapterMaxLen = BK_ADAPTER_MAX_LEN, kMaxAdapters = BK_MAX_ADAPTERS,
                   kAdapterMinOverlap = BK_ADAPTER_MIN_OVERLAP;
constexpr double kAdapterMaxErrorRate = BK_ADAPTER_MAX_ERROR_RATE;
static_assert(kAdapterMaxLen == 64 && kMaxAdapters <= 8, "AdapterEntry holds 64 bases, AdapterArgs eight entries");
constexpr uint32_t kNoCut = 0xFFFFFFFFu;
struct AdapterEntry {
    uint32_t code[4];
    uint32_t mask[4];
    uint32_t len;
    uint32_t allowed;
};
struct AdapterArgs {
    uint32_t* words;
    uint16_t* lens;
    const uint8_t* ends;
    uint32_t* cut;
    uint64_t n_records;
    const unsigned long long* n_records_dev;
    uint32_t stride_words;
    int32_t k;
    uint32_t n_adapters;
    uint32_t min_overlap;
    uint64_t allowed_steps;
    unsigned long long* stats;
    unsigned long long* n_real;
    AdapterEntry adapters[kMaxAdapters];
};
void launch_adapter_trim(const AdapterArgs& a, int n_cus, hipStream_t stream);
void launch_pick_window(const ScanArgs& a, uint64_t n_probe, unsigned int* votes, const uint32_t* file_cell_lo, int forced, uint32_t* win,
                        hipStream_t stream);
void launch_count_kmers(const ScanArgs& a, hipStream_t stream);
void launch_add_u64(unsigned long long* dst, const unsigned long long* src, hipStream_t stream);
void launch_add_const_u64(unsigned long long* dst, unsigned long long v, hipStream_t stream);
uint32_t scan_grid(uint64_t n_records, int n_cus);
uint32_t scan_l2_words(uint32_t stride_words, int k);
uint64_t scan_max_records(uint32_t grid);
int scan_ref_pad_words();
int scan_ref_back_words();
int scan_bit_pad_words();
int scan_bit_back_words();
size_t scan_lds_budget();
size_t scan_ref_lds_bytes(uint32_t total_cells);
size_t scan_lds_bytes(uint32_t n_lds_bins, bool ref_in_lds, uint32_t total_cells);
hipError_t launch_scan_count(const ScanArgs& a, uint32_t grid, hipStream_t stream);
void launch_fold(const FoldArgs& f, hipStream_t stream);
struct BinArgs {
    ItemGeom ig;
    const unsigned short* items;
    const unsigned short* tab;
    const unsigned short* gext;
    uint32_t n_wg;
    const unsigned int* ov;
    unsigned long long* ov_n;
    uint32_t ov_cap, ov_par;
    const uint32_t* id_at;
    const uint32_t* cell_codes;
    uint32_t win_lo;
    const uint32_t* win_dev;
    uint32_t total_cells;
    unsigned long long* counters;
    uint64_t v_off, v_real_len;
    uint32_t rl;
    int v_mode;
    int part;
    int ablate;
};
bool item_geometry(uint32_t win_cells, uint32_t n_full, int v_span, ItemGeom* g);
uint32_t items_grid(uint64_t n_records, int n_cus);
uint32_t items_max_grid(int n_cus);
size_t items_lds_bytes(const ItemGeom& g, uint32_t win_cells);
hipError_t launch_scan_items(const ScanArgs& a, uint32_t grid, hipStream_t stream);
hipError_t launch_bin_count(const BinArgs& b, hipStream_t stream);
inline bool level2_launches(const ScanArgs& a) { return a.n_records != 0 && a.W > 0; }
hipError_t launch_level2(const ScanArgs& a, int n_cus, hipStream_t stream, const BinArgs* ride = nullptr);
void launch_ktab_stats(const unsigned long long* keys, const unsigned int* cnt, uint32_t log2n, unsigned long long ci,
                       unsigned long long cx, unsigned long long* out, hipStream_t stream);
void launch_ktab_rehash(const unsigned long long* okeys, const unsigned int* ocnt, uint32_t olog2, unsigned long long* nkeys, unsigned int* ncnt,
                        uint32_t nlog2, unsigned long long* overflow, hipStream_t stream);
void launch_ktab_count_parts(const unsigned long long* keys, uint32_t log2n, uint32_t n_parts, unsigned long long* counts, hipStream_t stream);
void launch_ktab_scatter_parts(const unsigned long long* keys, const unsigned int* cnt, uint32_t log2n, uint32_t n_parts, unsigned long long* cursors,
                               unsigned long long* out_keys, unsigned int* out_cnt, hipStream_t stream);
void launch_ktab_import(const unsigned long long* in_keys, const unsigned int* in_cnt, uint64_t n, unsigned long long* keys, unsigned int* cnt, uint32_t log2n,
// ... 274 lines not shown
```

bronko_amd/csrc/bk_kernels.hip:

```cpp
#include <hip/hip_runtime.h>

#include <algorithm>
#include <cstdlib>
#include <mutex>
#include <utility>
#include <vector>

#include "bk_bin_count.h"
#include "bk_device.h"
#include "bk_kernels.h"
#include "bk_scan_common.h"
#include "bk_finalize_common.h"

namespace bk {


__device__ __forceinline__ int probe_table(const TableSlot* __restrict__ sub, uint32_t log2s, uint64_t key) {
    const uint32_t smask = (1u << log2s) - 1u;
    uint32_t h = hash_key(key, log2s);
    for (;;) {
        const uint4 e = *reinterpret_cast<const uint4*>(sub + h);
        const uint64_t kk = (uint64_t)e.x | ((uint64_t)e.y << 32);
        if (kk == key) return (int)e.z;
        if (kk == kEmptyKey) return -1;
        h = (h + 1) & smask;
    }
}

__device__ __forceinline__ int single_diff_pos(uint64_t a, uint64_t b, int k) {
    const uint64_t x = a ^ b;
    const uint64_t y = (x | (x >> 1)) & 0x5555555555555555ull;
    if (y == 0 || (y & (y - 1)) != 0) return -1;
    return k - 1 - (__builtin_ctzll(y) >> 1);
}


__device__ __forceinline__ HalfDir half_lookup(const HalfView& hv, uint64_t half) {
    const uint32_t pilot = hv.pilots[phf_bucket(half, hv.log2nb)];
    const uint4 e = *reinterpret_cast<const uint4*>(hv.dir + phf_pos(half, pilot, hv.m, hv.log2nb, hv.log2p));
    HalfDir d;
    d.key = e.x; d.off = e.y; d.cnt = (e.x == (uint32_t)half) ? e.z : 0u; d.pad = 0u;
    return d;
}

template <typename F>
__device__ __forceinline__ void for_each_neighbour(const IndexView& ix, uint64_t c, F&& f) {
    const int k = ix.k;
    const int lo_bits = 2 * ix.lo_bases;
    const uint64_t lo = c & ((1ull << lo_bits) - 1ull), hi = c >> lo_bits;
    const int wlo = ix.wstart, whi = ix.wstart + ix.W;
    const HalfDir dl = half_lookup(ix.lo, lo);
    const HalfDir dh = half_lookup(ix.hi, hi);
    for (uint32_t i = 0; i < dl.cnt; ++i) {
        const uint4 e = *reinterpret_cast<const uint4*>(ix.lo.cand + dl.off + i);
        const int j = single_diff_pos((uint64_t)e.x | ((uint64_t)e.y << 32), c, k);
        if (j >= wlo && j < whi && ((e.w >> (j - wlo)) & 1u)) f(j, e.z, e.w);
    }
    for (uint32_t i = 0; i < dh.cnt; ++i) {
        const uint4 e = *reinterpret_cast<const uint4*>(ix.hi.cand + dh.off + i);
        const int j = single_diff_pos((uint64_t)e.x | ((uint64_t)e.y << 32), c, k);
        if (j >= wlo && j < whi && ((e.w >> (j - wlo)) & 1u)) f(j, e.z, e.w);
    }
}

__device__ __forceinline__ int acgt_code(unsigned char c) {
    switch (c | 0x20) {
        case 'a': return 0;
        case 'c': return 1;
        case 'g': return 2;
        case 't': return 3;
        default: return -1;
    }
}

template <bool kQual, bool kEnds, typename NextSlot>
__device__ __forceinline__ unsigned long long pack_runs(const PackArgs& a, const QualArgs& q, uint8_t* ends, uint64_t r, NextSlot&& next_slot) {
    const uint64_t maxb = min((uint64_t)a.stride_words * 16, (uint64_t)65535);
    const uint64_t o0 = a.offsets[r], len = a.offsets[r + 1] - o0;
    const uint8_t* s = a.bases + a.shift + o0;
    const uint8_t* qs = kQual ? q.quals + q.shift + o0 : nullptr;
    unsigned long long real = 0;
    uint64_t start = 0;
    for (uint64_t p = 0; p <= len; ++p) {
        if (p < len && acgt_code(s[p]) >= 0 && (!kQual || qs[p] >= q.thr)) continue;
        const uint64_t run = p - start;
        if (run >= (uint64_t)a.k) {
            uint64_t pos = 0;
            for (;;) {
                const uint64_t take = min(maxb, run - pos);
                const unsigned long long rec = next_slot();
                if (rec < a.cap) {
                    uint32_t* w = a.words + rec * a.stride_words;
                    uint32_t acc = 0;
                    for (uint64_t j = 0; j < take; ++j) {
                        acc |= (uint32_t)acgt_code(s[start + pos + j]) << (2 * (j & 15));
                        if ((j & 15) == 15) { w[j >> 4] = acc; acc = 0; }
                    }
                    if (take & 15) w[take >> 4] = acc;
                    for (uint64_t j = (take + 15) >> 4; j < a.stride_words; ++j) w[j] = 0;
                    a.lens[rec] = (uint16_t)take;
                    if constexpr (kEnds) ends[rec] = run <= maxb ? (uint8_t)((start == 0 ? kEndFirst : 0u) | (p == len ? kEndLast : 0u)) : (uint8_t)0;
                    ++real;
                }
                if (pos + take >= run) break;
                pos += take - (uint64_t)(a.k - 1);
            }
        }
        start = p + 1;
    }
    return real;
}
template <bool kQual, bool kEnds>
__device__ __forceinline__ unsigned long long pack_read_slow(const PackArgs& a, const QualArgs& q, uint8_t* ends, uint64_t r) {
    return pack_runs<kQual, kEnds>(a, q, ends, r, [&] { return atomicAdd(a.n_records, 1ull); });
}

constexpr int kPackBlock = 256;
constexpr uint32_t kPackMaxWords = 16;
constexpr uint32_t kPackWpt = 2;
constexpr uint32_t kPackLdsBytes = kPackBlock * kPackWpt * 16u + 96u;

template <bool kQual = false>
__device__ __forceinline__ uint32_t pack16(uint32_t x0, uint32_t x1, uint32_t x2, uint32_t x3, uint32_t nb, bool& ok,
                                           const uint32_t* qx = nullptr, uint32_t thr4 = 0u) {
    uint32_t out = 0u;
    const uint32_t x4[4] = {x0, x1, x2, x3};
#pragma unroll
    for (uint32_t j = 0; j < 4u; ++j) {
        const uint32_t x = x4[j];
        const uint32_t c = ((x >> 1) ^ (x >> 2)) & 0x03030303u;
        bool good = (x & 0xdfdfdfdfu) == __builtin_amdgcn_perm(0x54474341u, 0x54474341u, c);
        if constexpr (kQual) good = good && ((((qx[j] | 0x80808080u) - thr4) | qx[j]) & 0x80808080u) == 0x80808080u;
        ok &= good || nb <= 4u * j;
        const uint32_t c2 = c | (c >> 6);
        out |= ((c2 | (c2 >> 12)) & 0xffu) << (8u * j);
    }
    return nb < 16u ? out & ((1u << (2u * nb)) - 1u) : out;
}

__device__ __forceinline__ uint32_t valid16(const uint32_t* x4, const uint32_t* qx, uint32_t thr4) {
    uint32_t v = 0u;
#pragma unroll
    for (uint32_t j = 0; j < 4u; ++j) {
        const uint32_t x = x4[j];
        const uint32_t c = ((x >> 1) ^ (x >> 2)) & 0x03030303u;
        const uint32_t d = (x & 0xdfdfdfdfu) ^ __builtin_amdgcn_perm(0x54474341u, 0x54474341u, c);
        const uint32_t eq = ~(((d & 0x7f7f7f7fu) + 0x7f7f7f7fu) | d) & 0x80808080u;
        const uint32_t ge = (((qx[j] | 0x80808080u) - thr4) | qx[j]) & 0x80808080u;
        v |= ((((eq & ge) >> 7) * 0x00204081u) >> 21 & 0xfu) << (4u * j);
    }
    return v;
}

template <bool kQual, bool kEnds>
__device__ __forceinline__ void pack_words(const PackArgs& a, const QualArgs& qa, uint8_t* ends, uint32_t rpb, uint32_t tpr, uint32_t tpr_recip,
                                           unsigned char* lines, unsigned char* qlines, unsigned long long* off_s, unsigned int* bad_s,
                                           unsigned long long* blk_s, uint32_t* vm_s, uint32_t* pw_s) {
    const uint32_t sw = a.stride_words;
    const uint64_t r0 = (uint64_t)blockIdx.x * rpb, r1 = min(r0 + (uint64_t)rpb, a.n_reads);
    const uint32_t nr = (uint32_t)(r1 - r0);
    for (uint32_t i = threadIdx.x; i <= nr; i += kPackBlock) off_s[i] = a.offsets[r0 + i] + a.shift;
    if (threadIdx.x < rpb) bad_s[threadIdx.x] = 0u;
    if (kQual && threadIdx.x < 3u) blk_s[threadIdx.x] = 0ull;
    __syncthreads();
    const uint64_t b0 = off_s[0], b1 = off_s[nr], end = a.offsets[a.n_reads] + a.shift;
    const uint64_t a0 = b0 & ~15ull;
    const uint64_t span = b1 - a0;
    const uint64_t qd = kQual ? (uint64_t)qa.shift - (uint64_t)a.shift : 0ull;
    const uint64_t qa0 = kQual ? (b0 + qd) & ~15ull : 0ull, qspan = kQual ? b1 + qd - qa0 : 0ull, qend = kQual ? end + qd : 0ull;
    const bool fits = (kQual ? max(span, qspan) : span) + 48u <= kPackLdsBytes;
    if (fits) {
        const uint64_t n16 = (span + 15) / 16 + 2, full16 = (end - a0) / 16;
        for (uint64_t i = threadIdx.x; i < min(n16, full16); i += kPackBlock) reinterpret_cast<uint4*>(lines)[i] = reinterpret_cast<const uint4*>(a.bases + a0)[i];
        if (n16 > full16) for (uint64_t i = full16 * 16 + threadIdx.x; i < min(end - a0, n16 * 16); i += kPackBlock) lines[i] = a.bases[a0 + i];
        if constexpr (kQual) {
            const uint64_t m16 = (qspan + 15) / 16 + 2, qfull16 = (qend - qa0) / 16;
            for (uint64_t i = threadIdx.x; i < min(m16, qfull16); i += kPackBlock) reinterpret_cast<uint4*>(qlines)[i] = reinterpret_cast<const uint4*>(qa.quals + qa0)[i];
            if (m16 > qfull16) for (uint64_t i = qfull16 * 16 + threadIdx.x; i < min(qend - qa0, m16 * 16); i += kPackBlock) qlines[i] = qa.quals[qa0 + i];
        }
    }
// ... 1515 lines not shown
}
size_t scan_lds_bytes(uint32_t n_lds_bins, bool ref_in_lds, uint32_t total_cells) {
    return kScanLdsFixed + ((size_t)n_lds_bins + 1) * sizeof(unsigned int) +
           (ref_in_lds ? scan_ref_lds_bytes(std::min(n_lds_bins, total_cells)) : 0);
}
int scan_ref_pad_words() { return kRefPadWords; }
int scan_ref_back_words() { return kRefBackWords; }
int scan_bit_pad_words() { return kBitPadWords; }
int scan_bit_back_words() { return kBitBackWords; }

uint32_t scan_grid(uint64_t n_records, int n_cus) {
    const uint64_t want = (n_records + kScanBlock - 1) / kScanBlock;
    return (uint32_t)std::max<uint64_t>(1, std::min<uint64_t>(want, (uint64_t)n_cus));
}
uint32_t scan_l2_words(uint32_t stride_words, int k) { const uint32_t b = stride_words * 16u; return b >= (uint32_t)k ? (b - (uint32_t)k + 1u + 31u) / 32u : 1u; }
uint64_t scan_max_records(uint32_t grid) { return (uint64_t)grid * (kMaxRecordsPerGroup - kScanBlock - 64); }

hipError_t launch_scan_count(const ScanArgs& a, uint32_t grid, hipStream_t stream) {
    if (a.n_records == 0 || a.W <= 0) return hipSuccess;
    if (a.n_records > scan_max_records(grid)) return hipErrorInvalidValue;
    const size_t lds = scan_lds_bytes(a.n_lds_bins, a.ref_in_lds != 0, a.total_cells);
    void (*kern)(ScanArgs);
#define BK_PICK(KT) (!a.touch_v ? (a.ref_in_lds ? scan_count_kernel<true, KT, false> : scan_count_kernel<false, KT, false>) \
                                : (a.ref_in_lds ? scan_count_kernel<true, KT, true> : scan_count_kernel<false, KT, true>))
    kern = a.k == 21 ? BK_PICK(21) : a.k == 31 ? BK_PICK(31) : BK_PICK(0);
#undef BK_PICK
    {
        static std::mutex mu;
        static std::vector<std::pair<std::pair<const void*, int>, size_t>> have;
        int dev = 0;
        (void)hipGetDevice(&dev);
        const void* fn = reinterpret_cast<const void*>(kern);
        std::lock_guard<std::mutex> lock(mu);
        size_t* cur = nullptr;
        for (auto& h : have) if (h.first.first == fn && h.first.second == dev) cur = &h.second;
        if (!cur || *cur < lds) {
            hipError_t e = hipFuncSetAttribute(fn, hipFuncAttributeMaxDynamicSharedMemorySize, (int)lds);
            if (e != hipSuccess) return e;
            if (cur) *cur = lds; else have.push_back({{fn, dev}, lds});
        }
    }
    hipLaunchKernelGGL(kern, dim3(grid), dim3(kScanBlock), lds, stream, a);
    return hipGetLastError();
}

__global__ __launch_bounds__(1024) void l2_plan_kernel(const unsigned int* __restrict__ l2_any, uint64_t n_words, unsigned int* __restrict__ plan, uint32_t g_min) {
    __shared__ unsigned int part[16];
    unsigned int n = 0;
    for (uint64_t i = threadIdx.x; i < n_words; i += 1024u) n += (unsigned int)__popc(l2_any[i]);
#pragma unroll
    for (int off = 32; off; off >>= 1) n += (unsigned int)__shfl_xor((int)n, off);
    if ((threadIdx.x & 63u) == 0u) part[threadIdx.x >> 6] = n;
    __syncthreads();
    if (threadIdx.x == 0) {
        unsigned int t = 0;
        for (int w = 0; w < 16; ++w) t += part[w];
        plan[0] = max(g_min, (t + 255u) / 256u);
    }
}

hipError_t launch_level2(const ScanArgs& a, int n_cus, hipStream_t stream, const BinArgs* ride) {
    if (!level2_launches(a)) return ride ? hipErrorInvalidValue : hipSuccess;
    const bool stats = a.ktab_keys != nullptr;
    if (!a.n_direct) {
        void (*kern)(ScanArgs);
#define BK_PICKN(KT) (!a.touch_v ? (stats ? nbatch_kernel<true, KT, false> : nbatch_kernel<false, KT, false>) \
                                 : (stats ? nbatch_kernel<true, KT, true> : nbatch_kernel<false, KT, true>))
        kern = a.k == 21 ? BK_PICKN(21) : a.k == 31 ? BK_PICKN(31) : BK_PICKN(0);
#undef BK_PICKN
        const uint64_t turns = (a.n_records + 32 * kAnyWords * kNbBlocksPerWave - 1) / (32 * kAnyWords * kNbBlocksPerWave);
        const unsigned grid = (unsigned)std::max<uint64_t>(1, std::min<uint64_t>((turns + kL2Waves - 1) / kL2Waves, (uint64_t)n_cus * 8));
        hipLaunchKernelGGL(kern, dim3(grid), dim3(kL2Block), 0, stream, a);
    }
#define BK_PICK(KT) (!a.touch_v ? (stats ? level2_kernel<true, KT, false> : level2_kernel<false, KT, false>) \
                                : (stats ? level2_kernel<true, KT, true> : level2_kernel<false, KT, true>))
    void (*kern)(ScanArgs, uint32_t, BinArgs) = a.k == 21 ? BK_PICK(21) : a.k == 31 ? BK_PICK(31) : BK_PICK(0);
#undef BK_PICK
    const uint64_t blks = (a.n_records + 32 * kAnyWords - 1) / (32 * kAnyWords);
    const unsigned grid = (unsigned)std::max<uint64_t>(1, std::min<uint64_t>((blks + kL2Waves - 1) / kL2Waves, (uint64_t)n_cus * (a.n_files == 1 ? 2 : 8)));
    if (a.l2_plan) hipLaunchKernelGGL(l2_plan_kernel, dim3(1), dim3(1024), 0, stream, (const unsigned int*)a.l2_any, (a.n_records + 31) / 32, a.l2_plan, a.l2_min_grid);
    const BinArgs rb = ride ? *ride : BinArgs{};
    const unsigned n_ride = ride && ride->n_wg ? ride->ig.n_ebins : 0u;
    hipLaunchKernelGGL(kern, dim3(grid + n_ride), dim3(kL2Block), 0, stream, a, (uint32_t)grid, rb);
    return hipGetLastError();
}

__global__ __launch_bounds__(256) void fold_kernel(FoldArgs f) {
    const uint64_t tid = (uint64_t)blockIdx.x * 256 + threadIdx.x;
    const uint64_t nthreads = (uint64_t)gridDim.x * 256;
    const uint32_t per = (f.n_slabs + gridDim.y - 1) / gridDim.y;
    const uint32_t b0 = blockIdx.y * per, b1 = min(f.n_slabs, b0 + per);
    for (uint64_t i = tid; i < f.n_lds_bins && b0 < b1; i += nthreads) {
        unsigned long long s0 = 0, s1 = 0;
        for (uint32_t b = b0; b < b1; ++b) {
            const unsigned int v = f.slabs[(size_t)b * f.n_lds_bins + i];
            s0 += v & 0xffffu;
            s1 += v >> 16;
        }
        if (s0 | s1) {
            const uint64_t cell = (f.win_dev ? f.win_dev[1] : f.win_lo) + i;
            const uint32_t id = f.id_at[cell];
            const uint32_t rc = ((f.cell_codes[cell >> 4] >> (2 * (cell & 15))) & 3u) == 2u ? 1u : 0u;
            touch(f.touch_e, id);
            if (s0) atomicAdd(f.counters + 2 * (size_t)id + rc, s0);
            if (s1) atomicAdd(f.counters + 2 * (size_t)id + (1u - rc), s1);
        }
    }
}

void launch_fold(const FoldArgs& f, hipStream_t stream) {
    const uint64_t work = f.n_lds_bins;
    if (work == 0) return;
    uint64_t blocks = (work + 255) / 256;
    if (blocks > 1024) blocks = 1024;
    const unsigned groups = std::max(1u, std::min(8u, f.n_slabs / 8));
    hipLaunchKernelGGL(fold_kernel, dim3((unsigned)blocks, groups), dim3(256), 0, stream, f);
}

__device__ __forceinline__ uint32_t first_of_file(const DevEntry* __restrict__ ent, uint32_t cnt, int file) {
    uint32_t lo = 0, hi = cnt;
    while (lo < hi) {
        const uint32_t mid = (lo + hi) >> 1;
        if ((int)ent[mid].file < file) lo = mid + 1; else hi = mid;
    }
    return lo;
}

template <int B>
__device__ __forceinline__ void write_lane(int& acc, int nb) { asm("v_writelane_b32 %0, %1, %2" : "+v"(acc) : "s"(nb), "n"(B)); }
template <int... B>
__device__ __forceinline__ void tally_word(uint32_t wd, int& acc, std::integer_sequence<int, B...>) {
    (write_lane<B>(acc, __popcll(__ballot((wd & (1u << B)) != 0u))), ...);
}
template <bool ATOMIC, uint32_t COL = 1u>
__device__ __forceinline__ void tally_files(const uint4& fb, uint32_t* lstats, uint32_t lane, uint32_t n_files) {
    if (!__ballot(files_any(fb))) return;
#pragma unroll
    for (uint32_t w = 0; w < 4u; ++w) {
        const uint32_t wd = w == 0u ? fb.x : w == 1u ? fb.y : w == 2u ? fb.z : fb.w;
        if (w * 32u >= n_files || !__ballot(wd != 0u)) continue;
        int acc = 0;
        tally_word(wd, acc, std::make_integer_sequence<int, 32>{});
        const uint32_t f = w * 32u + lane;
        if (lane < 32u && acc && f < n_files) {
            if (ATOMIC) atomicAdd(&lstats[f * 3u + COL], (uint32_t)acc); else lstats[f * 3u + COL] += (uint32_t)acc;
        }
    }
}

__global__ __launch_bounds__(256) void finalize_reduce_kernel(FinalizeArgs a, int n_rows, unsigned long long* zero_p, size_t zero_n) {
    __shared__ unsigned long long wave_sums[4];
    const int n3 = a.ix.n_files * 3, cols = n3 + 2;
    for (size_t i = (size_t)blockIdx.x * 256 + threadIdx.x; i < zero_n; i += (size_t)gridDim.x * 256) zero_p[i] = 0ull;
    if (a.lean_n_list && blockIdx.x == 0 && threadIdx.x < 8) a.lean_n_list[threadIdx.x] = 0u;
    const int col = blockIdx.x;
    unsigned long long s = 0;
    for (int r = threadIdx.x; r < n_rows; r += 256) s += a.partials[(size_t)r * cols + col];
#pragma unroll
    for (int off = 32; off; off >>= 1) s += __shfl_xor(s, off);
    if ((threadIdx.x & 63) == 0) wave_sums[threadIdx.x >> 6] = s;
    __syncthreads();
    if (threadIdx.x != 0) return;
    s = wave_sums[0] + wave_sums[1] + wave_sums[2] + wave_sums[3];
    if (!s) return;
    if (col < n3) { a.stats[col] += s; if (col % 3 != 2) a.present[col / 3] = 1; }
    else if (col == n3) { if (a.kept_total) *a.kept_total += s; }
    else if (a.distinct_total) *a.distinct_total += s;
}

constexpr int kVoteSlots = 512;
constexpr uint32_t kVoteMaxEntries = 4;
constexpr size_t kVoteLdsBytes = (size_t)kVoteSlots * (8 + 8 + 4 + 2) + 16;
struct VoteTable {
    unsigned long long* keys;
    unsigned long long* mx;
    unsigned int* cnt;
    unsigned int* n_used;
    unsigned short* used;
};
__device__ __forceinline__ VoteTable vt_make(unsigned char* lds) {
    VoteTable vt;
    vt.keys = reinterpret_cast<unsigned long long*>(lds);
    vt.mx = vt.keys + kVoteSlots;
    vt.cnt = reinterpret_cast<unsigned int*>(vt.mx + kVoteSlots);
    vt.n_used = vt.cnt + kVoteSlots;
    vt.used = reinterpret_cast<unsigned short*>(vt.n_used + 4);
    return vt;
}
__device__ __forceinline__ void vt_clear(const VoteTable& vt) {
    for (int i = threadIdx.x; i < kVoteSlots; i += blockDim.x) { vt.keys[i] = ~0ull; vt.mx[i] = 0ull; vt.cnt[i] = 0u; }
    if (threadIdx.x == 0) { vt.n_used[0] = 0u; vt.n_used[1] = 0u; }
}
__device__ __forceinline__ void vt_vote(const VoteTable& vt, uint32_t par, const FinalizeArgs& a, const DevEntry& e, uint64_t c, uint32_t isrc,
                                        int k, unsigned long long v) {
    if (a.mode == 1 || (a.mode == 2 && (int)e.file != a.sel_file)) return;
    uint32_t bit_idx;
    bool forward;
    if (e.canonical) { bit_idx = ((uint32_t)(c >> (2 * e.idx)) & 3u) ^ 3u; forward = isrc != 0; }
    else { bit_idx = (uint32_t)(c >> (2 * (k - 1 - e.idx))) & 3u; forward = isrc == 0; }
    const unsigned long long key = (((unsigned long long)e.cell * 4 + bit_idx) << 1) | (forward ? 0ull : 1ull);
    uint32_t h = (uint32_t)((key * 0x9E3779B97F4A7C15ull) >> 55) & (kVoteSlots - 1);
    for (int probe = 0; probe < 8; ++probe) {
        const unsigned long long old = atomicCAS(&vt.keys[h], ~0ull, key);
        if (old == ~0ull) vt.used[atomicAdd(vt.n_used + par, 1u)] = (unsigned short)h;
        if (old == ~0ull || old == key) { atomicAdd(&vt.cnt[h], 1u); atomicMax(&vt.mx[h], v); return; }
        h = (h + 1) & (kVoteSlots - 1);
    }
    vote(a, e, c, isrc, k, v);
}
__device__ __forceinline__ void vt_flush(const VoteTable& vt, uint32_t par, const FinalizeArgs& a) {
    __syncthreads();
    const unsigned int nu = vt.n_used[par];
    if (threadIdx.x == 0) vt.n_used[par ^ 1u] = 0u;
    for (unsigned int u = threadIdx.x; u < nu; u += blockDim.x) {
        const int i = vt.used[u];
        const unsigned long long key = vt.keys[i];
        const size_t cell = (size_t)(key >> 1);
        atomicAdd(a.pileup + ((key & 1ull) ? 3 : 2) * a.plane + cell, (unsigned long long)vt.cnt[i]);
        atomicMax(a.pileup + ((key & 1ull) ? 1 : 0) * a.plane + cell, vt.mx[i]);
        vt.keys[i] = ~0ull; vt.mx[i] = 0ull; vt.cnt[i] = 0u;
    }
    __syncthreads();
    if (threadIdx.x == 0) { vt.n_used[0] = 0u; vt.n_used[1] = 0u; }
}

__device__ __forceinline__ void v_kmer_of_counter(const IndexView& ix, const unsigned long long* __restrict__ vc, uint64_t vi,
                                                  uint32_t& p, uint32_t& t, uint64_t& c, uint32_t& isrc, unsigned long long& n) {
    const int k = ix.k;
    const uint64_t real_len = v_real_len(ix.n_full, ix.v_span);
    uint32_t bb;
    if (vi < real_len) {
        const uint32_t rl = (uint32_t)ix.v_span + 1u;
        const uint64_t row = vi / rl;
        const uint32_t oo = (uint32_t)(vi % rl);
        n = 0;
        if (vc) for (uint32_t x = 0; x <= oo; ++x) n += vc[row * rl + x];
        const uint32_t r6 = (uint32_t)(row % kVRowsPerPos);
        p = (uint32_t)(row / kVRowsPerPos) - oo;
        const uint32_t rcid = (ix.amb[p] >> 1) & 1u;
        const int o = (int)oo + ix.v_omin;
        const int j = rcid ? k - 1 - o : o;
        const uint32_t own = (uint32_t)(ix.kmer_of[p] >> (2 * (k - 1 - j))) & 3u;
        bb = own ^ ((r6 >> 1) + 1u);
        isrc = (r6 & 1u) ^ rcid;
        t = (uint32_t)(j - ix.wstart);
    } else {
        const uint64_t x = vi - real_len;
        isrc = (uint32_t)x & 1u;
        bb = (uint32_t)(x >> 1) & 3u;
        p = ix.prow_id[x >> 3];
        t = ix.prow_t[x >> 3];
        n = vc ? vc[vi] : 0ull;
    }
    const int sh = 2 * (k - 1 - (ix.wstart + (int)t));
    c = (ix.kmer_of[p] & ~(3ull << sh)) | ((uint64_t)bb << sh);
}

template <bool MANY>
__global__ __launch_bounds__(256) __attribute__((amdgpu_waves_per_eu(8, 8))) void finalize_variant_kernel(FinalizeArgs a) {
    extern __shared__ __attribute__((aligned(16))) unsigned char smem[];
    if (a.mode == 2) { a.sel_file = *a.sel; if (a.sel_file < 0 && !a.clear_v) return; }
    const bool do_stats = a.mode < 2;
    const IndexView& ix = a.ix;
    uint32_t* lstats = reinterpret_cast<uint32_t*>(smem);
    const VoteTable vt = vt_make(smem + (((size_t)ix.n_files * 3 + 2) * sizeof(uint32_t) + 15) / 16 * 16);
    for (int g = threadIdx.x; g < ix.n_files * 3 + 2; g += 256) lstats[g] = 0;
    vt_clear(vt);
    __syncthreads();

    const int k = ix.k;
    const uint64_t n_rows = v_real_rows(ix.n_full, ix.v_span);
    const uint64_t real_len = v_real_len(ix.n_full, ix.v_span);
    const uint32_t rl = (uint32_t)ix.v_span + 1u;
    unsigned long long* __restrict__ vc = const_cast<unsigned long long*>(a.counters) + ix.v_off;
    const KmerTable kt{a.ktab_keys, a.ktab_cnt, a.ktab_log2, a.ktab_overflow, a.mate};
    unsigned int kept = 0, distinct = 0;
    const uint64_t vlo = a.elem_lo > ix.v_off ? a.elem_lo - ix.v_off : 0ull, vhi = a.elem_hi > ix.v_off ? a.elem_hi - ix.v_off : 0ull;
    const uint64_t row_lo = min(vlo / rl, n_rows), row_hi = min(vhi / rl, n_rows);
    const uint64_t px_lo = min(vlo > real_len ? vlo - real_len : 0ull, ix.n_prows * 8ull), px_hi = min(vhi > real_len ? vhi - real_len : 0ull, ix.n_prows * 8ull);

    size_t acc_at[2] = {~(size_t)0, ~(size_t)0};
    unsigned long long acc_n[2] = {0, 0}, acc_max[2] = {0, 0};
    auto flush = [&](int f) {
        if (acc_at[f] != ~(size_t)0) {
            atomicAdd(a.pileup + (f ? 3 : 2) * a.plane + acc_at[f], acc_n[f]);
            atomicMax(a.pileup + (f ? 1 : 0) * a.plane + acc_at[f], acc_max[f]);
        }
        acc_at[f] = ~(size_t)0; acc_n[f] = 0; acc_max[f] = 0;
    };
    auto vote_acc = [&](const DevEntry& e, uint64_t c, uint32_t isrc, unsigned long long v) {
        if (a.mode == 1 || (a.mode == 2 && (int)e.file != a.sel_file)) return;
        uint32_t bit_idx;
        bool forward;
        if (e.canonical) { bit_idx = ((uint32_t)(c >> (2 * e.idx)) & 3u) ^ 3u; forward = isrc != 0; }
        else { bit_idx = (uint32_t)(c >> (2 * (k - 1 - e.idx))) & 3u; forward = isrc == 0; }
        const size_t cell = (size_t)e.cell * 4 + bit_idx;
        const int f = forward ? 0 : 1;
        if (acc_at[f] != cell) { flush(f); acc_at[f] = cell; }
        acc_n[f] += 1;
        acc_max[f] = acc_max[f] > v ? acc_max[f] : v;
    };

    auto map_one = [&](uint32_t p, uint32_t t, uint64_t c, uint32_t isrc, unsigned long long n, uint64_t vi) {
        if (do_stats) distinct += 1;
        if (n < a.ci || n > a.cx) return;
        if (do_stats) ++kept;
        const unsigned long long v = n > a.cs ? a.cs : n;
// ... 399 lines not shown
          const uint32_t t = (uint32_t)(g & 7ull);
          distinct += (n != 0 && t == 0);
          if (n == 0 || n < a.ci || n > a.cx) continue;
          kept += (t == 0);
          const uint32_t id = (uint32_t)(cidx >> 1);
          uint32_t n_perfect = 0, perfect_file = 0;
          for (uint32_t q = ix.estat_off[id] + t, qe = ix.estat_off[id + 1]; q < qe; q += 8u) {
              const uint32_t e = ix.estat[q];
              tally(lstats, (e >> 1) * 3 + ((e & 1u) ? 0u : 1u));
              if (e & 1u) { ++n_perfect; perfect_file = e >> 1; }
          }
          uint32_t tot = n_perfect;
          tot += (uint32_t)__shfl_xor((int)tot, 1); tot += (uint32_t)__shfl_xor((int)tot, 2); tot += (uint32_t)__shfl_xor((int)tot, 4);
          if (tot == 1 && n_perfect == 1) atomicAdd(&lstats[perfect_file * 3 + 2], 1u);
          continue;
      }
      if (ix.n_files > 1 && !a.e_list && !__syncthreads_or(mine && a.counters[cidx] != 0ull)) continue;
      if (mine) pair_body(cidx, (uint32_t)(g % W));
      vt_flush(vt, par, a);
      par ^= 1u;
    }
    const uint64_t pc_n = a.e_list ? n_pseudo_listed * 2ull : c_hi;
    const uint32_t pl = a.e_list ? 8u : 1u;
    const uint64_t pw_n = a.e_list ? pc_n * W * pl : pc_n;
    for (uint64_t wi = (a.e_list ? 0ull : max(c_lo, 2ull * ix.n_full)) + (uint64_t)blockIdx.x * 256 + threadIdx.x; wi < pw_n; wi += (uint64_t)gridDim.x * 256) {
        const uint64_t ci = a.e_list ? wi / (W * pl) : wi;
        const uint32_t rem = a.e_list ? (uint32_t)(wi - ci * (W * pl)) : 0u, t0 = rem / pl, sub = rem - t0 * pl;
        const bool head = t0 == 0u && sub == 0u;
        const uint64_t cidx = a.e_list ? 2ull * a.e_list[ix.n_u - 1u - (uint32_t)(ci >> 1)] + (ci & 1ull) : ci;
        const unsigned long long n = a.counters[cidx];
        if (n == 0) continue;
        distinct += do_stats && head;
        if (n < a.ci || n > a.cx) continue;
        kept += do_stats && head;
        const unsigned long long v = n > a.cs ? a.cs : n;
        const uint32_t id = (uint32_t)(cidx >> 1), isrc = (uint32_t)cidx & 1u;
        const uint64_t c = ix.kmer_of[id];
        if (a.mode != 1) for (uint32_t t = a.e_list ? t0 : 0u; t < (a.e_list ? t0 + 1u : W); ++t) {
            const uint32_t s = ix.slot_of[(size_t)id * W + t];
            if (a.gather && !(ix.slot_alias && ((ix.slot_alias[s >> 5] >> (s & 31u)) & 1u))) continue;
            const uint32_t off = ix.ent_off[s], cnt = ix.ent_len[s];
            if (a.mode == 2 && ix.ent_files) {
                const uint4 fb = ix.ent_files[s];
                if (files_any(fb)) {
                    if (sub == 0u && files_has(fb, (uint32_t)a.sel_file)) vote(a, ix.entries[off + files_rank(fb, (uint32_t)a.sel_file)], c, isrc, k, v);
                    continue;
                }
            }
            if (a.mode == 2) {
                if (sub != 0u) continue;
                for (uint32_t q = first_of_file(ix.entries + off, cnt, a.sel_file); q < cnt; ++q) {
                    const DevEntry en = ix.entries[off + q];
                    if ((int)en.file != a.sel_file) break;
                    vote(a, en, c, isrc, k, v);
                }
            } else {
                for (uint32_t q = sub; q < cnt; q += pl) vote(a, ix.entries[off + q], c, isrc, k, v);
            }
        }
        if (!do_stats || !head) continue;
        uint32_t n_perfect = 0, perfect_file = 0;
        for (uint32_t q = ix.estat_off[id]; q < ix.estat_off[id + 1]; ++q) {
            const uint32_t e = ix.estat[q];
            atomicAdd(&lstats[(e >> 1) * 3 + ((e & 1u) ? 0 : 1)], 1u);
            if (e & 1u) { ++n_perfect; perfect_file = e >> 1; }
        }
        if (n_perfect == 1) atomicAdd(&lstats[perfect_file * 3 + 2], 1u);
    }
    __syncthreads();
    if (do_stats) finalize_epilogue(a, lstats, kept, distinct, lstats + ix.n_files * 3, a.row_exact + (int)blockIdx.x);
}

constexpr uint32_t kOwnCells = 256, kOwnSpan = kOwnCells + 32;
__global__ __launch_bounds__(256) void finalize_exact_own_kernel(FinalizeArgs a) {
    __shared__ unsigned long long mx[8][kOwnSpan];
    __shared__ unsigned int cnt[8][kOwnSpan];
    const IndexView& ix = a.ix;
    const int sel = a.mode == 2 ? *a.sel : 0;
    if (sel < 0) return;
    const uint32_t c_lo = a.mode == 2 ? a.file_cell_lo[sel] : 0u;
    const uint32_t c_hi = a.mode == 2 ? (sel + 1 < ix.n_files ? a.file_cell_lo[sel + 1] : ix.total_cells) : ix.total_cells;
    const uint32_t c0 = c_lo + blockIdx.x * kOwnCells;
    if (c0 >= c_hi) return;
    for (uint32_t i = threadIdx.x; i < 8u * kOwnSpan; i += 256u) { (&mx[0][0])[i] = 0ull; (&cnt[0][0])[i] = 0u; }
    __syncthreads();
    const int k = ix.k;
    const uint32_t W = (uint32_t)ix.W;
    const uint32_t c = c0 + threadIdx.x;
    const uint32_t id = c < c_hi ? ix.id_at[c] : 0xffffffffu;
    const uint32_t fsel = a.mode == 2 ? (uint32_t)sel : (c < c_hi ? (uint32_t)ix.cell_file[c] : 0u);
    unsigned long long n2[2] = {0ull, 0ull};
    if (id < ix.n_full) {
#pragma unroll
        for (int isrc = 0; isrc < 2; ++isrc) { const unsigned long long n = a.counters[2 * (size_t)id + isrc]; n2[isrc] = (n >= a.ci && n <= a.cx) ? n : 0ull; }
    }
    if ((n2[0] | n2[1]) != 0ull && files_has(ix.id_own_files[id], fsel)) {
        const uint4 fb = ix.slot_files[(size_t)id * W];
        const DevEntry e0 = ix.entries[ix.slot_rec[(size_t)id * W].off + files_rank(fb, fsel)];
        const uint4 idr = *reinterpret_cast<const uint4*>(ix.id_rec + id);
        const uint64_t km = (uint64_t)idr.x | ((uint64_t)idr.y << 32);
        const int dir = (idr.w & kIdOwnMirror) ? -1 : 1;
        const uint32_t q0 = e0.cell - c0;
        for (uint32_t isrc = 0; isrc < 2u && e0.cell == c + (uint32_t)e0.idx; ++isrc) {
            const unsigned long long n = n2[isrc];
            if (n == 0) continue;
            const unsigned long long v = n > a.cs ? a.cs : n;
            for (uint32_t t = 0; t < W; ++t) {
                const uint32_t idx = (uint32_t)((int)e0.idx + dir * (int)t);
                uint32_t bit_idx;
                bool forward;
                if (e0.canonical) { bit_idx = ((uint32_t)(km >> (2 * idx)) & 3u) ^ 3u; forward = isrc != 0; }
                else { bit_idx = (uint32_t)(km >> (2 * (k - 1 - (int)idx))) & 3u; forward = isrc == 0; }
                const uint32_t row = (forward ? 0u : 4u) + bit_idx;
                const uint32_t q = (uint32_t)((int)q0 + dir * (int)t);
                atomicAdd(&cnt[row][q], 1u);
                atomicMax(&mx[row][q], v);
            }
        }
    }
    __syncthreads();
    for (uint32_t i = threadIdx.x; i < 8u * kOwnSpan; i += 256u) {
        const uint32_t row = i / kOwnSpan, q = i - row * kOwnSpan;
        const unsigned int nv = cnt[row][q];
        if (!nv) continue;
        const size_t cell = ((size_t)c0 + q) * 4 + (row & 3u);
        atomicAdd(a.pileup + (row < 4u ? 2 : 3) * a.plane + cell, (unsigned long long)nv);
        atomicMax(a.pileup + (row < 4u ? 0 : 1) * a.plane + cell, mx[row][q]);
    }
}

__global__ __launch_bounds__(64) void finalize_general_kernel(FinalizeArgs a) {
    extern __shared__ __attribute__((aligned(16))) unsigned char smem[];
    if (a.mode == 2) { a.sel_file = *a.sel; if (a.sel_file < 0) return; }
    const bool do_stats = a.mode < 2;
    const IndexView& ix = a.ix;
    auto note_alias = [&](int sb, uint64_t c, uint32_t isrc, unsigned long long n) {
        if (a.alias_hits && ix.slot_alias && sb >= 0 && ((ix.slot_alias[(uint32_t)sb >> 5] >> ((uint32_t)sb & 31u)) & 1u)) {
            const unsigned int at = atomicAdd(a.n_alias_hits, 1u);
            if (at < a.alias_cap) { a.alias_hits[3ull * at] = c | ((unsigned long long)isrc << 62); a.alias_hits[3ull * at + 1ull] = n; a.alias_hits[3ull * at + 2ull] = (unsigned long long)(uint32_t)sb; }
        }
    };
    uint32_t* hits = reinterpret_cast<uint32_t*>(smem);
    uint32_t* touched = hits + ix.n_files;
    uint32_t* lstats = touched + ix.n_files;
    uint32_t* ntouched = lstats + (size_t)ix.n_files * 3;
    const int lane = threadIdx.x;
    for (int g = lane; g < ix.n_files; g += 64) hits[g] = 0;
    for (int g = lane; g < ix.n_files * 3; g += 64) lstats[g] = 0;
    if (lane == 0) *ntouched = 0;
    __syncthreads();

    const int k = ix.k;
    const size_t S = (size_t)1 << ix.log2s;
    const uint64_t n_e = e_plane_len(ix.n_u);
    const uint64_t n_items = *a.n_deferred;

    if (a.mode == 2) {
        for (uint64_t item = (uint64_t)blockIdx.x * 64 + (uint32_t)lane; item < n_items; item += (uint64_t)gridDim.x * 64) {
            unsigned long long v;
            uint64_t c;
            uint32_t isrc, p_, t_;
            v_kmer_of_counter(ix, a.deferred_n ? nullptr : a.counters + ix.v_off, a.deferred[item], p_, t_, c, isrc, v);
            if (a.deferred_n) v = a.deferred_n[item];
            v = v > a.cs ? a.cs : v;
            for (uint32_t tm = a.deferred_mask ? a.deferred_mask[item] : 0xffffffffu >> (32 - ix.W); tm; tm &= tm - 1u) {
                const int t = __builtin_ctz(tm);
                const int sh = 2 * (k - 1 - (ix.wstart + t));
                const int sb = probe_table(ix.table + (size_t)t * S, ix.log2s, c & ~(3ull << sh));
                if (sb < 0) continue;
                const uint32_t off = ix.ent_off[sb];
                const uint4 fb = ix.ent_files ? ix.ent_files[sb] : make_uint4(0u, 0u, 0u, 0u);
                if (files_any(fb)) {
                    if (files_has(fb, (uint32_t)a.sel_file)) vote(a, ix.entries[off + files_rank(fb, (uint32_t)a.sel_file)], c, isrc, k, v);
                    continue;
                }
                const uint32_t cnt = ix.ent_len[sb];
                for (uint32_t q = first_of_file(ix.entries + off, cnt, a.sel_file); q < cnt; ++q) {
                    const DevEntry e = ix.entries[off + q];
                    if ((int)e.file != a.sel_file) break;
                    vote(a, e, c, isrc, k, v);
                }
            }
        }
        return;
    }
    const uint64_t n_tail = (a.tail_e_list && a.mode == 0) ? 2ull * a.tail_n_list[2] : 0ull;
    unsigned int tail_kept = 0, tail_distinct = 0;
    auto wave_item = [&](uint64_t item) {
        {
            uint64_t ci, c;
            unsigned long long v;
            uint32_t isrc, p_, t_;
            if (item < n_items) {
                ci = n_e + a.deferred[item];
                v_kmer_of_counter(ix, a.deferred_n ? nullptr : a.counters + ix.v_off, ci - n_e, p_, t_, c, isrc, v);
                if (a.deferred_n) v = a.deferred_n[item];
            } else {
                const uint64_t e = item - n_items;
                const uint32_t id = a.tail_e_list[e >> 1];
                isrc = (uint32_t)e & 1u;
                ci = 2ull * id + isrc;
                v = a.counters[ci];
                const uint4 idr = *reinterpret_cast<const uint4*>(ix.id_rec + id);
                c = (uint64_t)idr.x | ((uint64_t)idr.y << 32);
                if (lane == 0) tail_distinct += v != 0;
                if (v == 0 || v < a.ci || v > a.cx) return;
                if (lane == 0) tail_kept += 1;
            }
            v = v > a.cs ? a.cs : v;

            int s = -1;
            if (lane < ix.W) {
                if (ci < n_e) {
                    s = (int)ix.slot_of[(size_t)(ci >> 1) * ix.W + lane];
                } else {
                    const int sh = 2 * (k - 1 - (ix.wstart + lane));
                    s = probe_table(ix.table + (size_t)lane * S, ix.log2s, c & ~(3ull << sh));
                }
            }
            if (a.mode == 1) note_alias(s, c, isrc, v);
            for (unsigned long long bm = __ballot(s >= 0); bm; bm &= bm - 1ull) {
                const int sb = __shfl(s, __builtin_ctzll(bm));
                const uint32_t off = ix.ent_off[sb], cnt = ix.ent_len[sb];
                for (uint32_t q = (uint32_t)lane; q < cnt; q += 64u) {
                    const DevEntry e = ix.entries[off + q];
                    if (atomicAdd(&hits[e.file], 1u) == 0u) touched[atomicAdd(ntouched, 1u)] = e.file;
                    vote(a, e, c, isrc, k, v);
                }
            }
            __syncthreads();
            const uint32_t nt = *ntouched;
            uint32_t n_perfect = 0;
            int my_perfect = -1;
            for (uint32_t q = lane; q < ((nt + 63u) & ~63u); q += 64) {
                bool perfect = false;
                if (q < nt) {
                    const uint32_t g = touched[q];
                    const uint32_t h = hits[g];
                    hits[g] = 0;
                    perfect = h == (uint32_t)ix.W;
                    if (do_stats) lstats[g * 3 + (perfect ? 0 : 1)] += 1;
                    if (perfect) my_perfect = (int)g;
                }
                n_perfect += (uint32_t)__popcll(__ballot(perfect));
            }
            if (do_stats && n_perfect == 1 && my_perfect >= 0) lstats[my_perfect * 3 + 2] += 1;
            __syncthreads();
            if (lane == 0) *ntouched = 0;
            __syncthreads();
        }
    };
    if (a.mode == 1 && ix.ent_files) {
        for (uint64_t item0 = (uint64_t)blockIdx.x * 64; item0 < n_items; item0 += (uint64_t)gridDim.x * 64) {
            const uint64_t item = item0 + (uint32_t)lane;
            const bool on = item < n_items;
            unsigned long long v = 0;
            uint64_t c = 0;
            uint32_t isrc = 0, p_ = 0, t_ = 0;
            if (on) v_kmer_of_counter(ix, nullptr, a.deferred[item], p_, t_, c, isrc, v);
            uint4 acc = make_uint4(0u, 0u, 0u, 0u);
            uint32_t found = 0, alias_n = 0;
            int alias_sb = -1;
            bool generic = false;
            for (int t = 0; t < ix.W; ++t) {
                const int sh = 2 * (k - 1 - (ix.wstart + t));
                const int sb = on ? probe_table(ix.table + (size_t)t * S, ix.log2s, c & ~(3ull << sh)) : -1;
                if (sb < 0) continue;
                const uint4 fb = ix.ent_files[sb];
                generic |= !files_any(fb);
                acc.x |= fb.x; acc.y |= fb.y; acc.z |= fb.z; acc.w |= fb.w;
                found |= 1u << t;
                alias_sb = (a.alias_hits && ix.slot_alias && ((ix.slot_alias[(uint32_t)sb >> 5] >> ((uint32_t)sb & 31u)) & 1u)) ? (alias_n++ ? -2 : sb) : alias_sb;
            }
            generic |= found == 0xffffffffu >> (32 - ix.W);
            generic |= alias_sb == -2;
            if (on && !generic && alias_sb >= 0) {
                unsigned long long n_; uint64_t c2; uint32_t i2, p2, t2;
                v_kmer_of_counter(ix, a.counters + ix.v_off, a.deferred[item], p2, t2, c2, i2, n_);
                note_alias(alias_sb, c, isrc, n_);
            }
            if (on && a.deferred_mask) a.deferred_mask[item] = found;
            if (!on || generic) acc = make_uint4(0u, 0u, 0u, 0u);
            tally_files<false>(acc, lstats, (uint32_t)lane, (uint32_t)ix.n_files);
            for (unsigned long long gm = __ballot(on && generic); gm; gm &= gm - 1ull) wave_item(item0 + (uint64_t)__builtin_ctzll(gm));
        }
    } else
    for (uint64_t item = blockIdx.x; item < n_items + n_tail; item += gridDim.x) wave_item(item);
    __syncthreads();
    if (lane == 0) { ntouched[0] = 0; ntouched[1] = 0; }
    __syncthreads();
    if (do_stats) finalize_epilogue(a, lstats, tail_kept, tail_distinct, ntouched, a.row_general + (int)blockIdx.x);
}

__global__ __launch_bounds__(256) void compact_touched_kernel(unsigned int* bm, uint64_t n_bits, unsigned int* list, unsigned int* n_out,
                                                              uint64_t split, uint64_t cap) {
    const uint64_t n_words = (n_bits + 31) / 32;
    const int lane = threadIdx.x & 63;
    for (uint64_t w0 = (uint64_t)blockIdx.x * 256; w0 < n_words; w0 += (uint64_t)gridDim.x * 256) {
        const uint64_t w = w0 + threadIdx.x;
        const uint32_t bits = w < n_words ? bm[w] : 0u;
        if (!__ballot(bits != 0u)) continue;
        if (bits) bm[w] = 0u;
        const uint32_t lo_mask = w * 32 + 32 <= split ? ~0u : w * 32 >= split ? 0u : (1u << (uint32_t)(split - w * 32)) - 1u;
        uint32_t lo = bits & lo_mask, hi = bits & ~lo_mask;
        const uint32_t n_lo = (uint32_t)__popc(lo), n_hi = (uint32_t)__popc(hi);
        uint32_t inc = n_lo | (n_hi << 16);
#pragma unroll
        for (int d = 1; d < 64; d <<= 1) { const uint32_t up = (uint32_t)__shfl_up((int)inc, d); if (lane >= d) inc += up; }
        uint32_t base_lo = 0, base_hi = 0;
        if (lane == 63) {
            if (inc & 0xffffu) base_lo = atomicAdd(n_out, inc & 0xffffu);
            if (inc >> 16) base_hi = atomicAdd(n_out + 1, inc >> 16);
        }
        base_lo = (uint32_t)__shfl((int)base_lo, 63) + (inc & 0xffffu) - n_lo;
        base_hi = (uint32_t)__shfl((int)base_hi, 63) + (inc >> 16) - n_hi;
        for (; lo; lo &= lo - 1u) list[base_lo++] = (uint32_t)(w * 32) + (uint32_t)__builtin_ctz(lo);
        for (; hi; hi &= hi - 1u) list[cap - 1 - base_hi++] = (uint32_t)(w * 32) + (uint32_t)__builtin_ctz(hi);
    }
}
__global__ __launch_bounds__(256) void expand_touched_blocks_kernel(unsigned int* touch_b, uint32_t n_blocks, const uint2* cell_blk, unsigned int* touch_v,
                                                                    uint32_t span, uint64_t n_q) {
    const uint32_t gb = blockIdx.x * 4u + (threadIdx.x >> 6), lane = threadIdx.x & 63u;
    if (gb >= n_blocks || !((touch_b[gb >> 5] >> (gb & 31u)) & 1u)) return;
    if (lane == 0) atomicAnd(touch_b + (gb >> 5), ~(1u << (gb & 31u)));
    const long long q_0 = (long long)gb * 64 + (long long)(int32_t)cell_blk[gb].x;
    const long long q_lo = max(q_0 - (long long)span, 0ll);
    const long long q_hi = min(q_0 + 64 + (long long)span, (long long)n_q);
    if (q_lo >= q_hi) return;
    const uint64_t r0 = (uint64_t)q_lo * kVRowsPerPos, r1 = (uint64_t)q_hi * kVRowsPerPos;
    for (uint64_t w = (r0 >> 5) + lane; w * 32u < r1; w += 64u) {
        const uint64_t lo = max(w * 32u, r0), hi = min(w * 32u + 32u, r1);
        const uint32_t take = (uint32_t)(hi - lo);
        atomicOr(touch_v + w, (take == 32u ? 0xffffffffu : (1u << take) - 1u) << (uint32_t)(lo & 31u));
    }
}
void launch_expand_touched_blocks(unsigned int* touch_b, uint32_t n_blocks, const uint2* cell_blk, unsigned int* touch_v, uint32_t span, uint64_t n_q, hipStream_t stream) {
    if (!n_blocks) return;
    hipLaunchKernelGGL(expand_touched_blocks_kernel, dim3((n_blocks + 3u) / 4u), dim3(256), 0, stream, touch_b, n_blocks, cell_blk, touch_v, span, n_q);
}
void launch_compact_touched(unsigned int* touch_v, uint64_t n_rows, unsigned int* touch_p, uint64_t n_prows, unsigned int* touch_e, uint64_t n_ids,
                            uint64_t n_full, unsigned int* v_list, unsigned int* p_list, unsigned int* e_list, unsigned int* n_list, hipStream_t stream) {
    auto go = [&](unsigned int* bm, uint64_t n, unsigned int* list, unsigned int* cnt, uint64_t split) {
        if (!n) return;
        const uint64_t blocks = std::max<uint64_t>(1, std::min<uint64_t>(((n + 31) / 32 + 255) / 256, 2048));
        hipLaunchKernelGGL(compact_touched_kernel, dim3((unsigned)blocks), dim3(256), 0, stream, bm, n, list, cnt, split, n);
    };
    go(touch_v, n_rows, v_list, n_list + 0, ~0ull);
    go(touch_p, n_prows, p_list, n_list + 4, ~0ull);
    go(touch_e, n_ids, e_list, n_list + 2, n_full);
}
__global__ __launch_bounds__(256) void clear_touched_kernel(unsigned long long* counters, uint64_t v_off, uint64_t v_real, uint32_t rl,
                                                            const unsigned int* v_list, const unsigned int* p_list, const unsigned int* e_list,
                                                            const unsigned int* n_list, uint64_t n_ids) {
    const uint64_t t = (uint64_t)blockIdx.x * 256 + threadIdx.x, nt = (uint64_t)gridDim.x * 256;
    unsigned long long* vc = counters + v_off;
    for (uint64_t i = t; i < (uint64_t)n_list[0] * rl; i += nt) vc[(uint64_t)v_list[i / rl] * rl + i % rl] = 0ull;
    for (uint64_t i = t; i < (uint64_t)n_list[4] * 8ull; i += nt) vc[v_real + (uint64_t)p_list[i >> 3] * 8ull + (i & 7ull)] = 0ull;
    for (uint64_t i = t; i < (uint64_t)n_list[2] * 2ull; i += nt) counters[2ull * e_list[i >> 1] + (i & 1ull)] = 0ull;
    for (uint64_t i = t; i < (uint64_t)n_list[3] * 2ull; i += nt) counters[2ull * e_list[n_ids - 1 - (i >> 1)] + (i & 1ull)] = 0ull;
}
void launch_clear_touched(unsigned long long* counters, uint64_t v_off, uint64_t v_real_len, uint32_t rl, const unsigned int* v_list,
                          const unsigned int* p_list, const unsigned int* e_list, const unsigned int* n_list, uint64_t n_ids, hipStream_t stream) {
    hipLaunchKernelGGL(clear_touched_kernel, dim3(2048), dim3(256), 0, stream, counters, v_off, v_real_len, rl, v_list, p_list, e_list, n_list, n_ids);
}

size_t finalize_lds_bytes(int n_files) { return ((size_t)n_files * 5 + 4) * sizeof(uint32_t); }
constexpr unsigned kFinVariantBlocks = 256 * 8, kFinExactBlocks = 256 * 8, kFinGeneralBlocks = 256 * 32;
size_t finalize_partial_rows() { return (size_t)kFinVariantBlocks + kFinExactBlocks + kFinGeneralBlocks; }

static unsigned finalize_general_blocks(const FinalizeArgs& a) {
    return (unsigned)std::min<size_t>(a.ix.n_files >= 8 ? kFinGeneralBlocks : kFinGeneralBlocks / 32, 256 * std::max<size_t>(1, (160u * 1024u) / finalize_lds_bytes(a.ix.n_files)));
}
bool finalize_runs_by_region(const FinalizeArgs& a) {
    return finalize_lean_ok(a) && (uint64_t)(a.ix.n_full + (uint32_t)a.ix.v_span) / 64 + (uint64_t)a.ix.total_cells / 256 + 2 + 64 + finalize_general_blocks(a) <= finalize_partial_rows();
}
void launch_finalize(const FinalizeArgs& a0, hipStream_t stream) {
    if (a0.ix.W <= 0) return;
    FinalizeArgs a = a0;
    const size_t lds_stats = ((size_t)a.ix.n_files * 3 + 2) * sizeof(uint32_t);
    const uint64_t rows_per_group = 4ull * (64ull / (uint64_t)std::max(a.ix.v_span, 1));
    const uint64_t n_v = std::max<uint64_t>((v_real_rows(a.ix.n_full, a.ix.v_span) + rows_per_group - 1) / rows_per_group * 256ull, a.ix.n_prows * 8ull);
    const unsigned b_var = (unsigned)std::max<uint64_t>(1, std::min<uint64_t>((n_v + 255) / 256, kFinVariantBlocks));
    const size_t lds_votes = (lds_stats + 15) / 16 * 16 + kVoteLdsBytes;
    const size_t lds = finalize_lds_bytes(a.ix.n_files);
    if (lds_votes > 64 * 1024 || lds > 64 * 1024) {
        (void)hipFuncSetAttribute(reinterpret_cast<const void*>(finalize_variant_kernel<false>), hipFuncAttributeMaxDynamicSharedMemorySize, (int)lds_votes);
        (void)hipFuncSetAttribute(reinterpret_cast<const void*>(finalize_variant_kernel<true>), hipFuncAttributeMaxDynamicSharedMemorySize, (int)lds_votes);
        (void)hipFuncSetAttribute(reinterpret_cast<const void*>(finalize_exact_kernel), hipFuncAttributeMaxDynamicSharedMemorySize, (int)lds_votes);
        (void)hipFuncSetAttribute(reinterpret_cast<const void*>(finalize_general_kernel), hipFuncAttributeMaxDynamicSharedMemorySize, (int)lds);
    }
    const unsigned b_gen = finalize_general_blocks(a);
    if (a.gather && a.mode >= 2) {
        if (a.ix.n_prows) {
            if (a.ix.slot_files) hipLaunchKernelGGL(finalize_variant_kernel<true>, dim3(64), dim3(256), lds_votes, stream, a);
            else hipLaunchKernelGGL(finalize_variant_kernel<false>, dim3(64), dim3(256), lds_votes, stream, a);
        }
        if (a.ix.n_u > a.ix.n_full) hipLaunchKernelGGL(finalize_exact_kernel, dim3(64), dim3(256), lds_votes, stream, a);
        if (a.alias_hits) launch_alias_votes(a, stream);
        return;
    }
    unsigned b_v = b_var, b_e = 0;
    const bool lean = finalize_runs_by_region(a);
    if (lean) {
        b_v = launch_finalize_lean_variant(a, stream);
        a.tail_e_list = a.lean_e_list; a.tail_n_list = a.lean_n_list;
        b_e = 0;
    } else {
    if (a.ix.slot_files) hipLaunchKernelGGL(finalize_variant_kernel<true>, dim3(b_var), dim3(256), lds_votes, stream, a);
    else hipLaunchKernelGGL(finalize_variant_kernel<false>, dim3(b_var), dim3(256), lds_votes, stream, a);
    const uint64_t n_work = e_plane_len(a.ix.n_u) * (uint64_t)a.ix.W;
    const unsigned b_ex = (unsigned)std::max<uint64_t>(1, std::min<uint64_t>((n_work + 255) / 256, kFinExactBlocks));
    a.row_exact = (int)b_var;
    if (a.mode == 2 && a.file_cell_lo && a.ix.id_own_files && a.max_file_cells)
        hipLaunchKernelGGL(finalize_exact_own_kernel, dim3((a.max_file_cells + kOwnCells - 1) / kOwnCells), dim3(256), 0, stream, a);
    else if (a.mode == 0 && a.e_list && a.file_cell_lo && a.ix.id_own_files && a.ix.cell_file && a.ix.estat_files && a.ix.id_rest_off && a.ix.total_cells)
        hipLaunchKernelGGL(finalize_exact_own_kernel, dim3((a.ix.total_cells + kOwnCells - 1) / kOwnCells), dim3(256), 0, stream, a);
    hipLaunchKernelGGL(finalize_exact_kernel, dim3(b_ex), dim3(256), lds_votes, stream, a);
    b_e = b_ex;
    }
    a.row_general = (int)(b_v + b_e);
    hipLaunchKernelGGL(finalize_general_kernel, dim3(b_gen), dim3(64), lds, stream, a);
    if (a.partials && a.mode < 2) {
        const int cols = a.ix.n_files * 3 + 2;
        hipLaunchKernelGGL(finalize_reduce_kernel, dim3((unsigned)cols), dim3(256), 0, stream, a, (int)(b_v + b_e + b_gen), a.zero_e, a.zero_e_n);
    }
}

__global__ __launch_bounds__(256) void zero_small_kernel(unsigned long long* a, size_t na, unsigned long long* b, size_t nb, unsigned long long* c, size_t nc,
                                                         unsigned char* d, size_t nd, unsigned int* e, size_t ne, unsigned long long* big, size_t nbig) {
    const size_t t = (size_t)blockIdx.x * blockDim.x + threadIdx.x, n = (size_t)gridDim.x * blockDim.x;
    for (size_t i = t; i < na; i += n) a[i] = 0;
    for (size_t i = t; i < nb; i += n) b[i] = 0;
    for (size_t i = t; i < nc; i += n) c[i] = 0;
    for (size_t i = t; i < nd; i += n) d[i] = 0;
    for (size_t i = t; i < ne; i += n) e[i] = 0;
    ulonglong2* big2 = reinterpret_cast<ulonglong2*>(big);
    for (size_t i = t; i < nbig / 2; i += n) big2[i] = make_ulonglong2(0ull, 0ull);
    if (t == 0 && (nbig & 1)) big[nbig - 1] = 0;
}
void launch_zero_small(unsigned long long* a, size_t na, unsigned long long* b, size_t nb, unsigned long long* c, size_t nc,
                       unsigned char* d, size_t nd, unsigned int* e, size_t ne, unsigned long long* big, size_t nbig, hipStream_t stream) {
    const unsigned grid = (unsigned)std::max<size_t>(16, std::min<size_t>((nbig / 2 + 255) / 256, 2048));
    hipLaunchKernelGGL(zero_small_kernel, dim3(grid), dim3(256), 0, stream, a, na, b, nb, c, nc, d, nd, e, ne, big, nbig);
}

__global__ void pack_sums_kernel(unsigned long long* sums, const unsigned long long* stats, const unsigned char* present,
                                 const unsigned long long* kstats, int n_files, unsigned long long* xflag) {
    const int n_s = 2 * n_files * 3, n_p = 2 * n_files;
    for (int i = blockIdx.x * blockDim.x + threadIdx.x; i < n_s + n_p + 9; i += gridDim.x * blockDim.x)
        sums[i] = i < n_s ? stats[i] : i < n_s + n_p ? (unsigned long long)present[i - n_s] : i < n_s + n_p + 8 ? kstats[i - n_s - n_p] : xflag[0];
}
__global__ void unpack_sums_kernel(const unsigned long long* sums, unsigned long long* stats, unsigned char* present,
                                   unsigned long long* kstats, int n_files, unsigned long long* xflag) {
    const int n_s = 2 * n_files * 3, n_p = 2 * n_files;
    for (int i = blockIdx.x * blockDim.x + threadIdx.x; i < n_s + n_p + 9; i += gridDim.x * blockDim.x) {
        if (i < n_s) stats[i] = sums[i];
        else if (i < n_s + n_p) present[i - n_s] = sums[i] ? 1 : 0;
        else if (i < n_s + n_p + 8) kstats[i - n_s - n_p] = sums[i];
        else { if (sums[i]) xflag[1] = 1ull; xflag[0] = 0ull; }
    }
}
void launch_pack_sums(unsigned long long* sums, const unsigned long long* stats, const unsigned char* present, const unsigned long long* kstats,
                      int n_files, unsigned long long* xflag, hipStream_t stream) {
    hipLaunchKernelGGL(pack_sums_kernel, dim3(8), dim3(256), 0, stream, sums, stats, present, kstats, n_files, xflag);
}
void launch_unpack_sums(const unsigned long long* sums, unsigned long long* stats, unsigned char* present, unsigned long long* kstats,
                        int n_files, unsigned long long* xflag, hipStream_t stream) {
    hipLaunchKernelGGL(unpack_sums_kernel, dim3(8), dim3(256), 0, stream, sums, stats, present, kstats, n_files, xflag);
}

struct XportGeom {
    uint64_t plane_len, part_len, v_off;
    uint32_t n_parts;
    uint64_t part_elems;
};
BK_HD uint64_t xport_e_in_part(const XportGeom& g, uint64_t p) {
    const uint64_t lo = p * g.part_len;
    return g.v_off > lo ? (g.v_off - lo < g.part_len ? g.v_off - lo : g.part_len) : 0ull;
}
__global__ __launch_bounds__(256) void xport_measure_kernel(const unsigned long long* __restrict__ plane, XportGeom g, unsigned long long* out ) {
    unsigned long long me = 0, mv = 0;
    for (uint64_t i = (uint64_t)blockIdx.x * 256 + threadIdx.x; i < g.plane_len; i += (uint64_t)gridDim.x * 256) {
        const unsigned long long v = plane[i];
        if (i < g.v_off) me = max(me, v);
        else { const long long sv = (long long)v; mv = max(mv, (unsigned long long)(sv < 0 ? -sv : sv)); }
    }
#pragma unroll
    for (int off = 32; off; off >>= 1) { me = max(me, (unsigned long long)__shfl_xor(me, off)); mv = max(mv, (unsigned long long)__shfl_xor(mv, off)); }
    if ((threadIdx.x & 63) == 0) { if (me) atomicMax(out, me); if (mv) atomicMax(out + 1, mv); }
}
template <int WIDTH>
__global__ __launch_bounds__(256) void xport_pack_kernel(const unsigned long long* __restrict__ plane, XportGeom g, void* buf, unsigned long long* flag) {
    bool bad = false;
    for (uint64_t i = (uint64_t)blockIdx.x * 256 + threadIdx.x; i < g.plane_len; i += (uint64_t)gridDim.x * 256) {
        const uint64_t p = i / g.part_len, j = i - p * g.part_len;
        const unsigned long long v = plane[i];
        const long long sv = (long long)v;
        if (WIDTH == 32) {
            bad |= sv > (long long)(0x7fffffffll / g.n_parts) || sv < -(long long)(0x7fffffffll / g.n_parts);
            static_cast<int*>(buf)[p * g.part_elems + j] = (int)sv;
        } else {
            const uint64_t n_e = xport_e_in_part(g, p);
            unsigned short* part = static_cast<unsigned short*>(buf) + p * g.part_elems;
            const long long lim = 32767 / g.n_parts;
            if (j < n_e) {
                bad |= v >> 32 != 0ull;
                *reinterpret_cast<uint2*>(part + 4 * j) = make_uint2((uint32_t)(v & 255u) | ((uint32_t)((v >> 8) & 255u) << 16),
                                                                      (uint32_t)((v >> 16) & 255u) | ((uint32_t)((v >> 24) & 255u) << 16));
            } else {
                bad |= sv > lim || sv < -lim;
                part[4 * n_e + (j - n_e)] = (unsigned short)(sv + lim);
            }
        }
    }
    if (WIDTH == 16) {
        for (uint64_t p = blockIdx.x; p < g.n_parts; p += gridDim.x) {
            const uint64_t used = g.part_len + 3 * xport_e_in_part(g, p);
            unsigned short* part = static_cast<unsigned short*>(buf) + p * g.part_elems;
            for (uint64_t x = used + threadIdx.x; x < g.part_elems; x += 256) part[x] = 0;
        }
    }
    if (__ballot(bad) && (threadIdx.x & 63) == 0) atomicOr(flag, 1ull);
}
template <int WIDTH>
__global__ __launch_bounds__(256) void xport_unpack_kernel(const void* __restrict__ recv, XportGeom g, uint32_t shard, unsigned long long* reduced) {
    const uint64_t n_e = xport_e_in_part(g, shard);
    for (uint64_t j = (uint64_t)blockIdx.x * 256 + threadIdx.x; j < g.part_len; j += (uint64_t)gridDim.x * 256) {
        long long v;
        if (WIDTH == 32) v = static_cast<const int*>(recv)[j];
        else if (j < n_e) {
            const unsigned short* d = static_cast<const unsigned short*>(recv) + 4 * j;
            v = (long long)d[0] + ((long long)d[1] << 8) + ((long long)d[2] << 16) + ((long long)d[3] << 24);
        } else v = (long long)static_cast<const unsigned short*>(recv)[4 * n_e + (j - n_e)] - (long long)(32767 / g.n_parts) * g.n_parts;
        reduced[j] = (unsigned long long)v;
    }
}
static XportGeom xport_geom(uint64_t plane_len, uint64_t v_off, uint32_t n_parts, int width) {
    XportGeom g{plane_len, plane_len / n_parts, v_off, n_parts, 0};
    g.part_elems = width == 16 ? (g.part_len + 3 * xport_e_in_part(g, 0) + 3) / 4 * 4 : g.part_len;
    return g;
}
uint64_t xport_part_bytes(uint64_t plane_len, uint64_t v_off, uint32_t n_parts, int width) {
    return width == 64 ? plane_len / n_parts * 8 : xport_geom(plane_len, v_off, n_parts, width).part_elems * (uint64_t)(width / 8);
}
void launch_xport_measure(const unsigned long long* plane, uint64_t plane_len, uint64_t v_off, unsigned long long* out, hipStream_t stream) {
    hipLaunchKernelGGL(xport_measure_kernel, dim3((unsigned)std::max<uint64_t>(1, std::min<uint64_t>((plane_len + 255) / 256, 2048))), dim3(256), 0, stream, plane,
                       xport_geom(plane_len, v_off, 1, 32), out);
}
void launch_xport_pack(const unsigned long long* plane, uint64_t plane_len, uint64_t v_off, uint32_t n_parts, int width, void* buf, unsigned long long* flag,
                       hipStream_t stream) {
    const XportGeom g = xport_geom(plane_len, v_off, n_parts, width);
    const dim3 grid((unsigned)std::max<uint64_t>(1, std::min<uint64_t>((plane_len + 255) / 256, 4096)));
    if (width == 16) hipLaunchKernelGGL(xport_pack_kernel<16>, grid, dim3(256), 0, stream, plane, g, buf, flag);
    else hipLaunchKernelGGL(xport_pack_kernel<32>, grid, dim3(256), 0, stream, plane, g, buf, flag);
}
void launch_xport_unpack(const void* recv, uint64_t plane_len, uint64_t v_off, uint32_t n_parts, uint32_t shard, int width, unsigned long long* reduced,
                         hipStream_t stream) {
    const XportGeom g = xport_geom(plane_len, v_off, n_parts, width);
    const dim3 grid((unsigned)std::max<uint64_t>(1, std::min<uint64_t>((g.part_len + 255) / 256, 4096)));
    if (width == 16) hipLaunchKernelGGL(xport_unpack_kernel<16>, grid, dim3(256), 0, stream, recv, g, shard, reduced);
    else hipLaunchKernelGGL(xport_unpack_kernel<32>, grid, dim3(256), 0, stream, recv, g, shard, reduced);
}

}
```

Measured before the change: 10.09 billion.

## Settle deferred k-mers inside lean finalize workgroups, dropping the general-kernel launch

```diff
diff --git a/bronko_amd/csrc/bk_engine.cpp b/bronko_amd/csrc/bk_engine.cpp
--- a/bronko_amd/csrc/bk_engine.cpp
+++ b/bronko_amd/csrc/bk_engine.cpp
@@ -59,7 +59,6 @@
         BK_HIP(e->deferred_n.alloc(e->deferred.n));
         for (MatePlane& p : e->mate) BK_HIP(hipMemset(p.counters.p, 0, std::max<size_t>(p.counters.n, 1) * sizeof(unsigned long long)));
     }
-    if (ix.n_files == 1 && !e->sparse && ix.n_full > 0) { BK_HIP(e->lean_e_list.alloc((size_t)ix.n_full)); BK_HIP(e->lean_n_list.alloc(8)); BK_HIP(hipMemset(e->lean_n_list.p, 0, 8 * sizeof(unsigned int))); }
     BK_HIP(e->pileup.alloc(ix.total_cells * 4 * 4));
     e->gather_mode = ix.gather_ok && e->sparse && ix.cell_file.p && ix.dirty_ans.p && ix.W > 1 && ix.file_cell_lo_d.p && !test_env("BK_NO_GATHER");
     if (e->gather_mode) {
@@ -103,7 +102,7 @@
     }
     if (ix.n_files > 1) { BK_HIP(e->win_votes.alloc((size_t)ix.n_files)); BK_HIP(e->win_sel.upload(std::vector<uint32_t>(2, 0u))); }
     e->fuse_ok = e->use_items && ix.n_files == 1 && ix.max_seqs_per_file == 1 && (uint64_t)ix.n_lds_bins >= ix.total_cells && !e->ktab.keys.p && ix.n_prows == 0 &&
-                 ix.n_u == ix.n_full && ix.n_full > 0 && ix.dirty_ans.p && ix.W > 1 && ix.v_span > 0 && ix.v_span <= 32 && e->fin_partials.p && e->lean_e_list.p &&
+                 ix.n_u == ix.n_full && ix.n_full > 0 && ix.dirty_ans.p && ix.W > 1 && ix.v_span > 0 && ix.v_span <= 32 && e->fin_partials.p &&
                  prm->cs < (1ull << 32) && e->ig.vq_log2 == 6 && !test_env("BK_NO_LEAN_FINALIZE") && !test_env("BK_NO_FUSE") && !test_env("BK_NO_N_DIRECT");
     if (e->fuse_ok)
         for (MatePlane& p : e->mate) { BK_HIP(p.fuse_touch.alloc(((size_t)ix.n_full + (size_t)ix.v_span + 63) / 64 * 12 + 16)); BK_HIP(hipMemset(p.fuse_touch.p, 0, p.fuse_touch.n * sizeof(unsigned int))); }
@@ -366,7 +365,7 @@
         if (test_env("BK_L2_STATS")[0] == '2')
             for (int b = 0; b < n_wg; b++) fprintf(stderr, "[bk]   wg %d: %.1f %.1f %.1f %.1f\n", b, (clk[4 * b] - t0) * 0.01, (clk[4 * b + 1] - t0) * 0.01, (clk[4 * b + 2] - t0) * 0.01, (clk[4 * b + 3] - t0) * 0.01);
     }
-    fprintf(stderr, "[bk] finalize: %u + %u k-mers deferred to the general kernel\n", nd[0], nd[1]);
+    fprintf(stderr, "[bk] finalize: %u + %u k-mers deferred (items the regional finalize settles in place, or the general kernel's list)\n", nd[0], nd[1]);
     if (e->gather_mode) {
         unsigned int ah[2] = {0u, 0u};
         BK_HIP(hipMemcpy(ah, e->n_alias_hits.p, sizeof ah, hipMemcpyDeviceToHost));
@@ -600,7 +599,8 @@
     }
     a.sel = c.two_pass ? &e->sel_out.p->file_id : nullptr; a.sel_file = -1;
     const bool ride = c.clean_dense && !c.two_pass && e->fin_partials.p && pl.used;
-    a.no_lean = test_env("BK_NO_LEAN_FINALIZE") != nullptr; a.lean_e_list = e->lean_e_list.p; a.lean_n_list = e->lean_n_list.p;
+    a.no_lean = test_env("BK_NO_LEAN_FINALIZE") != nullptr; a.lean_list_cap = bk::kLeanListCap;
+    if (const char* lc = test_env("BK_LEAN_LIST_CAP")) a.lean_list_cap = (uint32_t)std::max(1, std::min((int)bk::kLeanListCap, atoi(lc)));
     a.zero_e = ride ? pl.counters.p : nullptr; a.zero_e_n = ride ? (size_t)std::min<uint64_t>(ix.v_off, ix.plane_len) : 0;
     return a;
 }
diff --git a/bronko_amd/csrc/bk_engine.h b/bronko_amd/csrc/bk_engine.h
--- a/bronko_amd/csrc/bk_engine.h
+++ b/bronko_amd/csrc/bk_engine.h
@@ -439,7 +439,6 @@
     DevBuf<unsigned int> ov;
     DevBuf<unsigned long long> ov_n;
     uint32_t ov_par = 0;
-    DevBuf<unsigned int> lean_e_list, lean_n_list;
     bool fuse_ok = false;
     struct PendingItems { bool on = false; int mate = 0; bk::BinArgs b{}; } pending;
     DevBuf<unsigned int> n_bits, n_any;
diff --git a/bronko_amd/csrc/bk_finalize_common.h b/bronko_amd/csrc/bk_finalize_common.h
--- a/bronko_amd/csrc/bk_finalize_common.h
+++ b/bronko_amd/csrc/bk_finalize_common.h
@@ -6,6 +6,18 @@
 #include "bk_scan_common.h"
 
 namespace bk {
+
+__device__ __forceinline__ int probe_table(const TableSlot* __restrict__ sub, uint32_t log2s, uint64_t key) {
+    const uint32_t smask = (1u << log2s) - 1u;
+    uint32_t h = hash_key(key, log2s);
+    for (;;) {
+        const uint4 e = *reinterpret_cast<const uint4*>(sub + h);
+        const uint64_t kk = (uint64_t)e.x | ((uint64_t)e.y << 32);
+        if (kk == key) return (int)e.z;
+        if (kk == kEmptyKey) return -1;
+        h = (h + 1) & smask;
+    }
+}
 
 __device__ __forceinline__ void vote(const FinalizeArgs& a, const DevEntry& e, uint64_t c, uint32_t isrc, int k, unsigned long long v) {
     if (a.mode == 1 || (a.mode == 2 && (int)e.file != a.sel_file)) return;
diff --git a/bronko_amd/csrc/bk_finalize_lean.hip b/bronko_amd/csrc/bk_finalize_lean.hip
--- a/bronko_amd/csrc/bk_finalize_lean.hip
+++ b/bronko_amd/csrc/bk_finalize_lean.hip
@@ -12,11 +12,18 @@
 constexpr uint32_t kLeanWin = 256;
 constexpr uint32_t kLeanMaxSpan = 32;
 constexpr uint32_t kLeanTouchWords = kLeanVq * kVRowsPerPos / 32;
-constexpr size_t kLeanStaticLds = (2u * 8u * kLeanWin + 5u + kLeanTouchWords + 1u) * sizeof(unsigned int);
+constexpr size_t kLeanStaticLds = (2u * 8u * kLeanWin + 6u + kLeanTouchWords + 1u + 4u * kLeanListCap) * sizeof(unsigned int);
 constexpr size_t lean_dynamic_lds(uint32_t v_span) { return (size_t)kLeanVq * kVRowsPerPos * ((size_t)v_span + 1u) * sizeof(unsigned int); }
 static_assert(kLeanStaticLds + 64u + lean_dynamic_lds(kLeanMaxSpan) <= 80u * 1024u, "two finalize_vbin workgroups no longer fit one CU's LDS");
 
-__device__ __forceinline__ void lean_vote(unsigned int* cnt, unsigned int* mxv, uint32_t span, uint32_t p0, const FinalizeArgs& a, uint32_t cell,
+typedef const __attribute__((address_space(4))) FinalizeArgs* LeanColdArgs;
+__device__ __forceinline__ LeanColdArgs lean_cold_args() {
+    LeanColdArgs p = (LeanColdArgs)__builtin_amdgcn_kernarg_segment_ptr();
+    asm volatile("" : "+s"(p));
+    return p;
+}
+template <typename Args>
+__device__ __forceinline__ void lean_vote(unsigned int* cnt, unsigned int* mxv, uint32_t span, uint32_t p0, const Args& a, uint32_t cell,
                                           uint32_t idx, bool canonical, uint64_t c, uint32_t isrc, int k, uint32_t v) {
     uint32_t bit_idx;
     bool forward;
@@ -29,8 +36,8 @@
         __hip_atomic_fetch_max(mxv + at, v, __ATOMIC_RELAXED, __HIP_MEMORY_SCOPE_WORKGROUP);
     } else {
         const size_t pc = (size_t)cell * 4 + bit_idx;
-        atomicAdd(a.pileup + (forward ? 2 : 3) * a.plane + pc, 1ull);
-        atomicMax(a.pileup + (forward ? 0 : 1) * a.plane + pc, (unsigned long long)v);
+        atomicAdd(a->pileup + (forward ? 2 : 3) * a->plane + pc, 1ull);
+        atomicMax(a->pileup + (forward ? 0 : 1) * a->plane + pc, (unsigned long long)v);
     }
 }
 __device__ __forceinline__ void lean_flush(const unsigned int* cnt, const unsigned int* mxv, uint32_t span, uint32_t p0, const FinalizeArgs& a) {
@@ -44,10 +51,43 @@
     }
 }
 
+__device__ __forceinline__ void lean_settle(unsigned int* cnt, unsigned int* mxv, uint32_t* lstats, uint32_t p0, uint64_t c, uint32_t meta, uint32_t v) {
+    const LeanColdArgs a = lean_cold_args();
+    const auto& ix = a->ix;
+    const int k = ix.k;
+    const uint32_t lane = threadIdx.x & 63u, isrc = meta & 1u;
+    int s = -1;
+    if (lane < (uint32_t)ix.W) {
+        if (meta & 2u) {
+            s = (int)ix.slot_of[(size_t)(meta >> 2) * (uint32_t)ix.W + lane];
+        } else {
+            const int sh = 2 * (k - 1 - (ix.wstart + (int)lane));
+            s = probe_table(ix.table + ((size_t)lane << ix.log2s), ix.log2s, c & ~(3ull << sh));
+        }
+    }
+    unsigned int hits = 0;
+    for (unsigned long long bm = __ballot(s >= 0); bm; bm &= bm - 1ull) {
+        const int sb = __shfl(s, __builtin_ctzll(bm));
+        const uint32_t off = ix.ent_off[sb], len = ix.ent_len[sb];
+        for (uint32_t q = lane; q < len; q += 64u) {
+            const DevEntry e = ix.entries[off + q];
+            hits += 1u;
+            lean_vote(cnt, mxv, kLeanWin, p0, a, e.cell, e.idx, e.canonical != 0, c, isrc, k, v);
+        }
+    }
+#pragma unroll
+    for (int off = 32; off; off >>= 1) hits += (unsigned int)__shfl_xor((int)hits, off);
+    if (lane == 0 && hits) {
+        if (hits == (unsigned int)ix.W) { atomicAdd(&lstats[0], 1u); atomicAdd(&lstats[2], 1u); }
+        else atomicAdd(&lstats[1], 1u);
+    }
+}
+
 template <bool FUSED>
 __global__ __launch_bounds__(kLeanVBlock) __attribute__((amdgpu_waves_per_eu(8, 8))) void finalize_vbin_kernel(FinalizeArgs a) {
     __shared__ unsigned int cnt[8 * kLeanWin], mxv[8 * kLeanWin];
-    __shared__ uint32_t lstats[3 + 2];
+    __shared__ uint32_t lstats[3 + 2 + 1];
+    __shared__ uint4 wlist[kLeanListCap];
     __shared__ unsigned int tmask[kLeanTouchWords + 1];
     extern __shared__ __attribute__((aligned(16))) unsigned int acc[];
     const IndexView& ix = a.ix;
@@ -58,7 +98,7 @@
     const uint32_t id_lo = min(q0 >= span - 1u ? q0 - (span - 1u) : 0u, ix.n_full - 1u);
     const uint32_t p0 = ix.id_rec[id_lo].cell;
     for (uint32_t i = threadIdx.x; i < 8u * kLeanWin; i += kLeanVBlock) { cnt[i] = 0u; mxv[i] = 0u; }
-    if (threadIdx.x < 5) lstats[threadIdx.x] = 0u;
+    if (threadIdx.x < 6) lstats[threadIdx.x] = 0u;
     if constexpr (FUSED) {
         const uint32_t n_eb = a.f_ig.n_ebins, n_bins = n_eb + a.f_ig.n_vbins, bin = n_eb + blockIdx.x, cap = a.f_ig.cap_v, G = a.f_ig.grid_max;
         const uint32_t upb = cap / 8u;
@@ -127,6 +167,28 @@
     const uint32_t grp = lane64 / lpr, oo = lane64 - grp * lpr;
     const bool lane_on = grp < gpw;
     unsigned int kept = 0, distinct = 0, variant = 0;
+#ifdef BK_TESTING
+    const uint32_t list_cap = lean_cold_args()->lean_list_cap;
+#else
+    constexpr uint32_t list_cap = kLeanListCap;
+#endif
+    auto list_items = [&](bool has, uint64_t c, uint32_t meta, uint32_t v) __attribute__((always_inline)) {
+        const unsigned long long dm = __ballot(has);
+        if (!dm) return;
+        const int lead = __builtin_ctzll(dm);
+        unsigned int base = 0;
+        if (lane64 == (uint32_t)lead) {
+            base = __hip_atomic_fetch_add(&lstats[5], (unsigned int)__popcll(dm), __ATOMIC_RELAXED, __HIP_MEMORY_SCOPE_WORKGROUP);
+            atomicAdd(lean_cold_args()->n_deferred, (unsigned int)__popcll(dm));
+        }
+        base = (unsigned int)__shfl((int)base, lead);
+        const unsigned int slot = base + (unsigned int)__popcll(dm & ((1ull << lane64) - 1ull));
+        if (has && slot < list_cap) wlist[slot] = make_uint4((uint32_t)c, (uint32_t)(c >> 32), meta, v);
+        for (unsigned long long om = __ballot(has && slot >= list_cap); om; om &= om - 1ull) {
+            const int l = __builtin_ctzll(om);
+            lean_settle(cnt, mxv, lstats, p0, __shfl(c, l), (uint32_t)__shfl((int)meta, l), (uint32_t)__shfl((int)v, l));
+        }
+    };
     for (uint32_t g0 = 0; g0 < kLeanVq * kVRowsPerPos; g0 += (kLeanVBlock / 64) * gpw) {
         const uint32_t g = g0 + wave * gpw + grp;
         const uint32_t q = q0 + g / kVRowsPerPos, r6 = g % kVRowsPerPos;
@@ -186,21 +248,9 @@
             }
             if (!plain) { defer = true; act = false; }
         }
-        {
-            const unsigned long long dm = __ballot(defer);
-            if (dm) {
-                unsigned int base = 0;
-                if (lane64 == (uint32_t)__builtin_ctzll(dm)) base = atomicAdd(a.n_deferred, (unsigned int)__popcll(dm));
-                base = (unsigned int)__shfl((int)base, __builtin_ctzll(dm));
-                if (defer) {
-                    const unsigned int slot = base + (unsigned int)__popcll(dm & ((1ull << lane64) - 1ull));
-                    a.deferred[slot] = (uint32_t)at;
-                    if (a.deferred_n) a.deferred_n[slot] = n;
-                }
-            }
-        }
-        if (act) lean_vote(cnt, mxv, kLeanWin, p0, a, idr.z + (uint32_t)j, (uint32_t)j, rcid != 0u, c, isrc, k, v);
+        if (act) lean_vote(cnt, mxv, kLeanWin, p0, &a, idr.z + (uint32_t)j, (uint32_t)j, rcid != 0u, c, isrc, k, v);
         variant += act ? 1u : 0u;
+        list_items(defer, c, isrc, v);
     }
 #pragma unroll
     for (int off = 32; off; off >>= 1) variant += (unsigned int)__shfl_xor((int)variant, off);
@@ -209,13 +259,17 @@
         const uint32_t W = (uint32_t)ix.W;
         const uint32_t sub = threadIdx.x & 15u, id = q0 + (threadIdx.x >> 4);
         unsigned int perfect = 0;
+        unsigned long long n0 = 0ull, n1 = 0ull;
+        uint64_t km = 0ull;
+        bool listed = false;
         if (id < ix.n_full) {
             const uint4 idr = *reinterpret_cast<const uint4*>(ix.id_rec + id);
-            const unsigned long long n0 = a.counters[2 * (size_t)id], n1 = a.counters[2 * (size_t)id + 1];
+            n0 = a.counters[2 * (size_t)id]; n1 = a.counters[2 * (size_t)id + 1];
+            if (unsigned long long* const ze = lean_cold_args()->zero_e; ze && sub < 2u && (sub ? n1 : n0)) ze[2 * (size_t)id + sub] = 0ull;
+            km = (uint64_t)idr.x | ((uint64_t)idr.y << 32);
             if (!(idr.w & kIdSimple)) {
-                if (sub == 0u && (n0 | n1)) a.lean_e_list[atomicAdd(a.lean_n_list + 2, 1u)] = id;
+                listed = sub == 0u && (n0 | n1) != 0ull;
             } else {
-                const uint64_t km = (uint64_t)idr.x | ((uint64_t)idr.y << 32);
                 const uint32_t rcid = (idr.w >> 1) & 1u;
 #pragma unroll
                 for (uint32_t isrc = 0; isrc < 2u; ++isrc) {
@@ -226,22 +280,38 @@
                     const uint32_t v = (uint32_t)(n > a.cs ? a.cs : n);
                     for (uint32_t t = sub; t < W; t += 16u) {
                         const uint32_t j = (uint32_t)ix.wstart + t;
-                        lean_vote(cnt, mxv, kLeanWin, p0, a, idr.z + j, j, rcid != 0u, km, isrc, k, v);
+                        lean_vote(cnt, mxv, kLeanWin, p0, &a, idr.z + j, j, rcid != 0u, km, isrc, k, v);
                     }
                 }
             }
         }
+        if (__ballot(listed)) {
+#pragma unroll 1
+            for (uint32_t isrc = 0; isrc < 2u; ++isrc) {
+                const unsigned long long n = isrc ? n1 : n0;
+                bool item = listed && n != 0ull;
+                if (item) { distinct += 1; if (n < a.ci || n > a.cx) item = false; else kept += 1; }
+                list_items(item, km, isrc | 2u | (id << 2), (uint32_t)(n > a.cs ? a.cs : n));
+            }
+        }
 #pragma unroll
         for (int off = 32; off; off >>= 1) perfect += (unsigned int)__shfl_xor((int)perfect, off);
         if (lane64 == 0 && perfect) { atomicAdd(&lstats[0], perfect); atomicAdd(&lstats[2], perfect); }
     }
     __syncthreads();
+    if (const uint32_t n_list = min(lstats[5], list_cap)) {
+        for (uint32_t i = wave; i < n_list; i += kLeanVBlock / 64) {
+            const uint4 it = wlist[i];
+            lean_settle(cnt, mxv, lstats, p0, (uint64_t)it.x | ((uint64_t)it.y << 32), it.z, it.w);
+        }
+        __syncthreads();
+    }
     lean_flush(cnt, mxv, kLeanWin, p0, a);
     finalize_epilogue(a, lstats, kept, distinct, lstats + 3, (int)blockIdx.x);
 }
 
 bool finalize_lean_ok(const FinalizeArgs& a) {
-    return !a.no_lean && a.lean_e_list && a.lean_n_list && !a.ix.slot_files && a.mode == 0 && !a.v_list && !a.p_list && !a.e_list && !a.ktab_keys && a.ix.n_prows == 0 && a.ix.n_u == a.ix.n_full &&
+    return !a.no_lean && !a.ix.slot_files && a.mode == 0 && !a.v_list && !a.p_list && !a.e_list && !a.ktab_keys && a.ix.n_prows == 0 && a.ix.n_u == a.ix.n_full &&
            a.ix.n_full > 0 && a.ix.n_files == 1 && a.ix.dirty_ans && a.ix.W > 1 && a.ix.v_span > 0 && a.ix.v_span <= (int)kLeanMaxSpan && a.partials && a.cs < (1ull << 32) &&
            a.elem_lo == 0 && a.elem_hi >= a.ix.v_off + v_plane_len(a.ix.n_full, a.ix.v_span, 0);
 }
diff --git a/bronko_amd/csrc/bk_kernels.h b/bronko_amd/csrc/bk_kernels.h
--- a/bronko_amd/csrc/bk_kernels.h
+++ b/bronko_amd/csrc/bk_kernels.h
@@ -20,6 +20,7 @@
 constexpr uint32_t kEBinLog2 = 7;
 constexpr uint32_t kERunMax = 255;
 constexpr uint32_t kEBinSpan = (1u << kEBinLog2) + kERunMax;
+constexpr uint32_t kLeanListCap = 256;
 constexpr uint32_t kItemGCap = 256;
 
 struct ScanArgs {
@@ -123,11 +124,8 @@
     int mode;
     const int* sel;
     int sel_file;
-    unsigned int* lean_e_list;
-    unsigned int* lean_n_list;
     int no_lean;
-    const unsigned int* tail_e_list;
-    const unsigned int* tail_n_list;
+    uint32_t lean_list_cap;
     unsigned long long* zero_e;
     size_t zero_e_n;
     int gather;
diff --git a/bronko_amd/csrc/bk_kernels.hip b/bronko_amd/csrc/bk_kernels.hip
--- a/bronko_amd/csrc/bk_kernels.hip
+++ b/bronko_amd/csrc/bk_kernels.hip
@@ -14,18 +14,6 @@
 
 namespace bk {
 
-
-__device__ __forceinline__ int probe_table(const TableSlot* __restrict__ sub, uint32_t log2s, uint64_t key) {
-    const uint32_t smask = (1u << log2s) - 1u;
-    uint32_t h = hash_key(key, log2s);
-    for (;;) {
-        const uint4 e = *reinterpret_cast<const uint4*>(sub + h);
-        const uint64_t kk = (uint64_t)e.x | ((uint64_t)e.y << 32);
-        if (kk == key) return (int)e.z;
-        if (kk == kEmptyKey) return -1;
-        h = (h + 1) & smask;
-    }
-}
 
 __device__ __forceinline__ int single_diff_pos(uint64_t a, uint64_t b, int k) {
     const uint64_t x = a ^ b;
@@ -1847,7 +1835,6 @@
     __shared__ unsigned long long wave_sums[4];
     const int n3 = a.ix.n_files * 3, cols = n3 + 2;
     for (size_t i = (size_t)blockIdx.x * 256 + threadIdx.x; i < zero_n; i += (size_t)gridDim.x * 256) zero_p[i] = 0ull;
-    if (a.lean_n_list && blockIdx.x == 0 && threadIdx.x < 8) a.lean_n_list[threadIdx.x] = 0u;
     const int col = blockIdx.x;
     unsigned long long s = 0;
     for (int r = threadIdx.x; r < n_rows; r += 256) s += a.partials[(size_t)r * cols + col];
@@ -2553,7 +2540,6 @@
 
     const int k = ix.k;
     const size_t S = (size_t)1 << ix.log2s;
-    const uint64_t n_e = e_plane_len(ix.n_u);
     const uint64_t n_items = *a.n_deferred;
 
     if (a.mode == 2) {
@@ -2585,39 +2571,19 @@
         }
         return;
     }
-    const uint64_t n_tail = (a.tail_e_list && a.mode == 0) ? 2ull * a.tail_n_list[2] : 0ull;
-    unsigned int tail_kept = 0, tail_distinct = 0;
     auto wave_item = [&](uint64_t item) {
         {
-            uint64_t ci, c;
+            uint64_t c;
             unsigned long long v;
             uint32_t isrc, p_, t_;
-            if (item < n_items) {
-                ci = n_e + a.deferred[item];
-                v_kmer_of_counter(ix, a.deferred_n ? nullptr : a.counters + ix.v_off, ci - n_e, p_, t_, c, isrc, v);
-                if (a.deferred_n) v = a.deferred_n[item];
-            } else {
-                const uint64_t e = item - n_items;
-                const uint32_t id = a.tail_e_list[e >> 1];
-                isrc = (uint32_t)e & 1u;
-                ci = 2ull * id + isrc;
-                v = a.counters[ci];
-                const uint4 idr = *reinterpret_cast<const uint4*>(ix.id_rec + id);
-                c = (uint64_t)idr.x | ((uint64_t)idr.y << 32);
-                if (lane == 0) tail_distinct += v != 0;
-                if (v == 0 || v < a.ci || v > a.cx) return;
-                if (lane == 0) tail_kept += 1;
-            }
+            v_kmer_of_counter(ix, a.deferred_n ? nullptr : a.counters + ix.v_off, a.deferred[item], p_, t_, c, isrc, v);
+            if (a.deferred_n) v = a.deferred_n[item];
             v = v > a.cs ? a.cs : v;
 
             int s = -1;
             if (lane < ix.W) {
-                if (ci < n_e) {
-                    s = (int)ix.slot_of[(size_t)(ci >> 1) * ix.W + lane];
-                } else {
-                    const int sh = 2 * (k - 1 - (ix.wstart + lane));
-                    s = probe_table(ix.table + (size_t)lane * S, ix.log2s, c & ~(3ull << sh));
-                }
+                const int sh = 2 * (k - 1 - (ix.wstart + lane));
+                s = probe_table(ix.table + (size_t)lane * S, ix.log2s, c & ~(3ull << sh));
             }
             if (a.mode == 1) note_alias(s, c, isrc, v);
             for (unsigned long long bm = __ballot(s >= 0); bm; bm &= bm - 1ull) {
@@ -2686,11 +2652,11 @@
             for (unsigned long long gm = __ballot(on && generic); gm; gm &= gm - 1ull) wave_item(item0 + (uint64_t)__builtin_ctzll(gm));
         }
     } else
-    for (uint64_t item = blockIdx.x; item < n_items + n_tail; item += gridDim.x) wave_item(item);
+    for (uint64_t item = blockIdx.x; item < n_items; item += gridDim.x) wave_item(item);
     __syncthreads();
     if (lane == 0) { ntouched[0] = 0; ntouched[1] = 0; }
     __syncthreads();
-    if (do_stats) finalize_epilogue(a, lstats, tail_kept, tail_distinct, ntouched, a.row_general + (int)blockIdx.x);
+    if (do_stats) finalize_epilogue(a, lstats, 0u, 0u, ntouched, a.row_general + (int)blockIdx.x);
 }
 
 __global__ __launch_bounds__(256) void compact_touched_kernel(unsigned int* bm, uint64_t n_bits, unsigned int* list, unsigned int* n_out,
@@ -2773,7 +2739,7 @@
     return (unsigned)std::min<size_t>(a.ix.n_files >= 8 ? kFinGeneralBlocks : kFinGeneralBlocks / 32, 256 * std::max<size_t>(1, (160u * 1024u) / finalize_lds_bytes(a.ix.n_files)));
 }
 bool finalize_runs_by_region(const FinalizeArgs& a) {
-    return finalize_lean_ok(a) && (uint64_t)(a.ix.n_full + (uint32_t)a.ix.v_span) / 64 + (uint64_t)a.ix.total_cells / 256 + 2 + 64 + finalize_general_blocks(a) <= finalize_partial_rows();
+    return finalize_lean_ok(a) && (uint64_t)(a.ix.n_full + (uint32_t)a.ix.v_span) / 64 + 1 <= finalize_partial_rows();
 }
 void launch_finalize(const FinalizeArgs& a0, hipStream_t stream) {
     if (a0.ix.W <= 0) return;
@@ -2800,13 +2766,12 @@
         if (a.alias_hits) launch_alias_votes(a, stream);
         return;
     }
-    unsigned b_v = b_var, b_e = 0;
-    const bool lean = finalize_runs_by_region(a);
-    if (lean) {
-        b_v = launch_finalize_lean_variant(a, stream);
-        a.tail_e_list = a.lean_e_list; a.tail_n_list = a.lean_n_list;
-        b_e = 0;
-    } else {
+    if (finalize_runs_by_region(a)) {
+        const unsigned b_lean = launch_finalize_lean_variant(a, stream);
+        hipLaunchKernelGGL(finalize_reduce_kernel, dim3((unsigned)(a.ix.n_files * 3 + 2)), dim3(256), 0, stream, a, (int)b_lean, (unsigned long long*)nullptr, (size_t)0);
+        return;
+    }
+    const unsigned b_v = b_var;
     if (a.ix.slot_files) hipLaunchKernelGGL(finalize_variant_kernel<true>, dim3(b_var), dim3(256), lds_votes, stream, a);
     else hipLaunchKernelGGL(finalize_variant_kernel<false>, dim3(b_var), dim3(256), lds_votes, stream, a);
     const uint64_t n_work = e_plane_len(a.ix.n_u) * (uint64_t)a.ix.W;
@@ -2817,8 +2782,7 @@
     else if (a.mode == 0 && a.e_list && a.file_cell_lo && a.ix.id_own_files && a.ix.cell_file && a.ix.estat_files && a.ix.id_rest_off && a.ix.total_cells)
         hipLaunchKernelGGL(finalize_exact_own_kernel, dim3((a.ix.total_cells + kOwnCells - 1) / kOwnCells), dim3(256), 0, stream, a);
     hipLaunchKernelGGL(finalize_exact_kernel, dim3(b_ex), dim3(256), lds_votes, stream, a);
-    b_e = b_ex;
-    }
+    const unsigned b_e = b_ex;
     a.row_general = (int)(b_v + b_e);
     hipLaunchKernelGGL(finalize_general_kernel, dim3(b_gen), dim3(64), lds, stream, a);
     if (a.partials && a.mode < 2) {
```

Result: faster. 10.38 billion, median of 6 (+2.9%).
